# llsurreal919/Reduce-Complexity-for-intra-coding-of-VVC

Hardware: AMD Instinct MI355X
Metric: CTUs/sec (All-Intra, QP32) (higher is better)
Workload: dtype int16/int32 samples+coefficients, fp64 RD cost

## Files before the change

### include/vvcx.h

```cpp
#ifndef VVCX_H
#define VVCX_H
#include <stdint.h>
#ifdef __cplusplus
extern "C" {
#endif

typedef enum {
  VVCX_OK = 0, VVCX_ERR_ARG = -1, VVCX_ERR_UNSUPPORTED = -2, VVCX_ERR_DEVICE = -3, VVCX_ERR_STATE = -4, VVCX_ERR_NO_ENCODING = -5
} vvcx_status;

enum {
  VVCX_TOOL_MRL = 1 << 0, VVCX_TOOL_MIP = 1 << 1, VVCX_TOOL_ISP = 1 << 2, VVCX_TOOL_LFNST = 1 << 3, VVCX_TOOL_MTS = 1 << 4,
  VVCX_TOOL_TS = 1 << 5, VVCX_TOOL_DEPQUANT = 1 << 6, VVCX_TOOL_RDOQ = 1 << 7, VVCX_TOOL_CCLM = 1 << 8,
  VVCX_TOOL_JCCR = 1 << 9, VVCX_TOOL_LMCS = 1 << 10, VVCX_TOOL_CU_REUSE = 1 << 11,
  VVCX_TOOL_FAST = 1 << 12,
  VVCX_TOOL_WPP = 1 << 13
};

typedef struct {
  int32_t pic_w, pic_h;
  int32_t bit_depth;
  int32_t ctu_size;
  int32_t min_qt[2];
  int32_t max_bt_depth[2];
// ... 67 lines not shown
int  vvcx_create(const vvcx_cfg *cfg, vvcx_handle **h);
void vvcx_destroy(vvcx_handle *h);
int  vvcx_set_slice(vvcx_handle *h, const vvcx_slice *s);
typedef struct {
  int32_t qp;
  int32_t bit_depth;
  int32_t n_pts;
  int32_t qp_in[8], qp_out[8];
  int32_t cb_qp_offset, cr_qp_offset;
  int32_t gop_size;
  int32_t dep_quant;
} vvcx_slice_cfg;
int  vvcx_chroma_qp_table(int bit_depth, int n_pts, const int32_t *qp_in, const int32_t *qp_out, int32_t *table);
int  vvcx_derive_slice(const vvcx_slice_cfg *cfg, vvcx_slice *out);

int  vvcx_set_forest(vvcx_handle *h, int n_trees, int n_nodes, int n_classes, const int32_t *root, const int32_t *feature, const double *threshold,
                     const int32_t *left, const int32_t *right, const double *value, const int32_t *classes);
int  vvcx_bind_frames(vvcx_handle *h, const vvcx_frame *frames, int n);
int  vvcx_compress_ctus(vvcx_handle *h, const vvcx_ctu_task *tasks, int n, vvcx_ctu_result *out, void *hip_stream);
int  vvcx_submit_ctus(vvcx_handle *h, const vvcx_ctu_task *tasks, int n, void *hip_stream);
int  vvcx_poll_ctus(vvcx_handle *h);
int  vvcx_wait_ctus(vvcx_handle *h, vvcx_ctu_result *out, int n);
int  vvcx_compress_bound_frames(vvcx_handle *h, vvcx_ctu_result *out , void *hip_stream);
int  vvcx_get_cus(vvcx_handle *h, int frame, vvcx_cu *cus, int max_cus, int *n_cus);
int  vvcx_get_tus(vvcx_handle *h, int frame, vvcx_tu *tus, int max_tus, int *n_tus);
int  vvcx_get_levels(vvcx_handle *h, int frame, int comp, int16_t *plane, int stride);
int  vvcx_lmcs_inverse_reco(vvcx_handle *h, void *hip_stream);
int  vvcx_lmcs_analyze(const void *const org[3], const int stride[3], int pic_w, int pic_h, int bit_depth, int slice_qp, int update_ctrl, vvcx_slice *slice);
int  vvcx_lmcs_analyze_device(const void *const org[3], const int stride[3], int pic_w, int pic_h, int bit_depth, int slice_qp, int update_ctrl, vvcx_slice *slice);
int  vvcx_lmcs_tables(vvcx_handle *h, int16_t *fwd, int16_t *inv, int32_t pivot[17], int32_t chroma_scale[16]);
int  vvcx_deblock_bound_frames(vvcx_handle *h, int beta_offset_div2, int tc_offset_div2, void *hip_stream);
float vvcx_last_deblock_ms(const vvcx_handle *h);
typedef struct vvcx_sao_param { int8_t mode, type, band, offset[4]; } vvcx_sao_param;
int   vvcx_sao_bound_frames(vvcx_handle *h, const vvcx_sao_param *prm, int lf_across_tiles, int log2_offset_scale, void *hip_stream);
float vvcx_last_sao_ms(const vvcx_handle *h);
int   vvcx_sao_statistics_bound_frames(vvcx_handle *h, int lf_across_tiles, int64_t *stats, void *hip_stream);
float vvcx_last_sao_stats_ms(const vvcx_handle *h);
int   vvcx_sao_decide(int pic_w, int pic_h, int bit_depth, int tile_cols, int tile_rows, int slice_qp, const double *lambda, int log2_offset_scale,
                      const int64_t *stats, vvcx_sao_param *prm);
int   vvcx_sao_picture(int pic_w, int pic_h, int bit_depth, int tile_cols, int tile_rows, const vvcx_sao_param *prm, int lf_across_tiles, int log2_offset_scale,
                       uint16_t *y, uint16_t *cb, uint16_t *cr, int device);
typedef struct vvcx_alf_aps {
  int32_t num_luma_filters; uint8_t class_to_filter[25]; uint8_t nonlinear_luma; int16_t luma_coeff[25][12]; uint8_t luma_clip_idx[25][12];
  int32_t num_chroma_alt; uint8_t nonlinear_chroma[8]; int16_t chroma_coeff[8][6]; uint8_t chroma_clip_idx[8][6];
} vvcx_alf_aps;
typedef struct vvcx_alf_slice { int32_t n_luma_aps, luma_aps[8], chroma_aps; } vvcx_alf_slice;
typedef struct vvcx_alf_ctu { uint8_t flag[3]; int8_t set; uint8_t alt[2]; } vvcx_alf_ctu;
int   vvcx_alf_bound_frames(vvcx_handle *h, const vvcx_alf_aps *aps, int n_aps, const vvcx_alf_slice *slices, const vvcx_alf_ctu *ctus, void *hip_stream);
float vvcx_last_alf_ms(const vvcx_handle *h);
int   vvcx_alf_picture(int pic_w, int pic_h, int bit_depth, const vvcx_alf_aps *aps, int n_aps, const vvcx_alf_slice *slice, const vvcx_alf_ctu *ctus,
                       uint16_t *y, uint16_t *cb, uint16_t *cr, uint8_t *classes, int device);
int   vvcx_alf_statistics_picture(int pic_w, int pic_h, int bit_depth, int n_bins, const uint16_t *const org[3], const uint16_t *const rec[3],
                                  int64_t *luma, int64_t *chroma, int device);
int   vvcx_alf_statistics_bound_frames(vvcx_handle *h, int frame_first, int n, int n_bins, int64_t *luma, int64_t *chroma, void *hip_stream);
float vvcx_last_alf_stats_ms(const vvcx_handle *h);
int   vvcx_alf_decide(int pic_w, int pic_h, int bit_depth, int chroma, int n_bins, const int64_t *luma, const int64_t *chroma_stats,
                      const double lambda[3], int max_luma_filters, vvcx_alf_aps *aps, vvcx_alf_slice *slice, vvcx_alf_ctu *ctus);
int  vvcx_deblock_cu_table(int pic_w, int pic_h, int bit_depth, int qp, int qp_cb, int qp_cr, int beta_offset_div2, int tc_offset_div2,
                           const int32_t *rows, int n_rows, uint16_t *y, uint16_t *cb, uint16_t *cr, int device);
int  vvcx_get_payload(vvcx_handle *h, int frame, int tile, uint8_t *buf, int cap, int *nbytes);
int  vvcx_enable_training_dump(vvcx_handle *h, int cap_rows);
int  vvcx_get_training_rows(vvcx_handle *h, int32_t *rows, int max_rows, int *n_rows);
int  vvcx_get_substream_sizes(vvcx_handle *h, int frame, int tile, int *sizes, int max_sizes, int *n_sizes);
float vvcx_last_kernel_ms(const vvcx_handle *h);
int  vvcx_get_counters(vvcx_handle *h, uint64_t out[4]);
int  vvcx_get_profile(vvcx_handle *h, uint64_t out[48]);
const char *vvcx_last_error(void);
int  vvcx_ctus_per_frame(const vvcx_handle *h);
int  vvcx_resident_streams(const vvcx_handle *h);


int  vvcx_distortion_batch(const int16_t *a, const int16_t *b, int w, int h, int n, uint64_t *out, int device);
typedef struct { int32_t comp, x, y, w, h, mode, mrl; } vvcx_pred_case;
int  vvcx_intra_pred_batch(vvcx_handle *h, const void *const reco[3], const uint8_t *const coded[2], const vvcx_pred_case *cases, int n, int16_t *pred);
int  vvcx_ctx_init(int qp, uint16_t s0[386], uint16_t s1[386]);
int  vvcx_cabac_code_bins(uint16_t *s0, uint16_t *s1, int ctx, const uint8_t *bins, int nbins, uint64_t *frac_bits, int device);
int  vvcx_rd_cost_batch(double lambda, const uint64_t *frac_bits, const uint64_t *dist, int n, double *cost, int device);
int  vvcx_transform_quant_batch(const int16_t *org, const int16_t *pred, int w, int h, int bit_depth, int qp, int n,
                                int16_t *lev, int16_t *rec, uint64_t *sse, uint8_t *cbf, int device);
int  vvcx_depquant_batch(const int16_t *org, const int16_t *pred, int w, int h, int bit_depth, int qp, int comp, int mts_idx, int cbf_cb, double lambda,
                         const uint16_t *s0, const uint16_t *s1, int n, int16_t *lev, int16_t *rec, uint64_t *sse, uint8_t *cbf, int device);
int  vvcx_lfnst_depquant_batch(const int16_t *org, const int16_t *pred, int w, int h, int bit_depth, int qp, int comp, int lfnst_idx, int intra_dir, int cbf_cb, double lambda,
                               const uint16_t *s0, const uint16_t *s1, int n, int16_t *lev, int16_t *rec, uint64_t *sse, uint8_t *cbf, int device);
int  vvcx_transform_skip_batch(const int16_t *resi, int w, int h, int bit_depth, int qp, double lambda, const uint16_t *s0, const uint16_t *s1, int n,
                               int16_t *lev, int16_t *resi_out, int32_t *abs_sum, uint8_t *keep, uint64_t *frac_bits, int device);
int  vvcx_isp_tu_batch(const int16_t *org, const int16_t *pred, int tw, int th, int bit_depth, int qp, double lambda, int prev_cbf, int cbf_inferred,
                       const uint16_t *s0, const uint16_t *s1, int n, int16_t *lev, int16_t *rec, uint64_t *sse, uint8_t *cbf, int device);
int  vvcx_scan_order(int w, int h, uint16_t *idx, int device);
int  vvcx_mip_pred_batch(const int32_t *cases, int n, const int16_t *refs, int n_refs, int16_t *pred, int n_pred, int device);
int  vvcx_forest_predict_batch(vvcx_handle *h, const int32_t *rows, int n, int32_t *out);

#ifdef __cplusplus
}
#endif
#endif
```

### reduce-complexity-for-intra-coding-of-vvc_amd/csrc/vvcx_api.hip

```cpp
#include <hip/hip_runtime.h>
#include <stdint.h>
#include <stdio.h>
#include <stdarg.h>
#include <stdlib.h>
#include <string.h>
#include <math.h>
#include <limits>
#include <algorithm>
#include <vector>
#include "vvcx.h"
#include "vvcx_dev.h"
#include "vvcx_host.h"
#include "vvcx_tables.h"

extern "C" __global__ void vvcx_compress_kernel_u8(VxParams p);
extern "C" __global__ void vvcx_compress_kernel_u16(VxParams p);
extern "C" __global__ void vvcx_compress_wpp_kernel_u8(VxParams p);
extern "C" __global__ void vvcx_compress_wpp_kernel_u16(VxParams p);
extern "C" __global__ void vvcx_leaf_dist_kernel(const int16_t *a, const int16_t *b, int w, int h, int16_t *scr, unsigned long long *out);
extern "C" __global__ void vvcx_leaf_pred_kernel_u8(VxParams p, const VxLeafPred *cases, int16_t *out, const int *out_off);
extern "C" __global__ void vvcx_leaf_pred_kernel_u16(VxParams p, const VxLeafPred *cases, int16_t *out, const int *out_off);
extern "C" __global__ void vvcx_leaf_cabac_kernel(uint16_t *io, int ctx, const uint8_t *bins, int nbins, unsigned long long *bits);
extern "C" __global__ void vvcx_leaf_rdcost_kernel(VxParams p, const unsigned long long *bits, const unsigned long long *dist, int n, double *cost);
extern "C" __global__ void vvcx_leaf_scan_kernel(int w, int h, uint16_t *idx);
extern "C" __global__ void vvcx_leaf_forest_kernel(VxParams p, const int32_t *rows, int n, int32_t *out);
struct VxMipCase { int32_t w, h, mode, bit_depth, ref_off, pred_off; };
extern "C" __global__ void vvcx_leaf_mip_kernel(const VxMipCase *cases, const int16_t *refs, int16_t *preds);
extern "C" __global__ void vvcx_sao_copy_kernel_u8(VxSaoParams p);
extern "C" __global__ void vvcx_sao_copy_kernel_u16(VxSaoParams p);
extern "C" __global__ void vvcx_sao_kernel_u8(VxSaoParams p);
extern "C" __global__ void vvcx_sao_kernel_u16(VxSaoParams p);
extern "C" __global__ void vvcx_sao_stats_kernel_u8(VxSaoStatParams p);
extern "C" __global__ void vvcx_sao_stats_kernel_u16(VxSaoStatParams p);
extern "C" __global__ void vvcx_alf_copy_kernel_u8(VxAlfParams p);
extern "C" __global__ void vvcx_alf_copy_kernel_u16(VxAlfParams p);
extern "C" __global__ void vvcx_alf_kernel_u8(VxAlfParams p);
extern "C" __global__ void vvcx_alf_kernel_u16(VxAlfParams p);
extern "C" __global__ void vvcx_alf_stats_b1_kernel_u8(VxAlfStatParams p);
extern "C" __global__ void vvcx_alf_stats_b4_kernel_u8(VxAlfStatParams p);
extern "C" __global__ void vvcx_alf_stats_b1_kernel_u16(VxAlfStatParams p);
extern "C" __global__ void vvcx_alf_stats_b4_kernel_u16(VxAlfStatParams p);
extern "C" __global__ void vvcx_deblock_edges_kernel(VxDeblockParams p);
extern "C" __global__ void vvcx_deblock_kernel_u8(VxDeblockParams p);
extern "C" __global__ void vvcx_deblock_kernel_u16(VxDeblockParams p);
extern "C" __global__ void vvcx_jccr_sign_kernel_u8(VxFrameDev *frames, int wc, int hc);
extern "C" __global__ void vvcx_jccr_sign_kernel_u16(VxFrameDev *frames, int wc, int hc);
extern "C" __global__ void vvcx_leaf_dq_kernel(VxParams p, const uint16_t *ctx, const int16_t *org, int16_t *rec, int16_t *lev, int32_t *tmp, int w, int h, int qp, int comp, int mts, int cbf_cb, unsigned long long *out, int lf, int lfdir);
extern "C" __global__ void vvcx_leaf_ts_kernel(VxParams p, const uint16_t *ctx, const int16_t *resi, int16_t *lev, int16_t *resi_out, int32_t *tmp, int w, int h, int qp, int *out, unsigned long long *bits);
extern "C" __global__ void vvcx_lmcs_map_kernel_u8(const uint8_t *src, uint8_t *dst, int w, int h, int stride, const int16_t *lut);
extern "C" __global__ void vvcx_lmcs_map_kernel_u16(const uint16_t *src, uint16_t *dst, int w, int h, int stride, const int16_t *lut);
extern "C" __global__ void vvcx_leaf_isp_kernel(VxParams p, const uint16_t *ctx, const int16_t *org, int16_t *rec, int16_t *lev, int32_t *tmp, int w, int h, int qp, int cbf_ctx, unsigned long long *out);
extern "C" __global__ void vvcx_ctu_activity_kernel_u8(const VxFrameDev *frames, int pic_w, int pic_h, int ctus_w, unsigned *out);
extern "C" __global__ void vvcx_ctu_activity_kernel_u16(const VxFrameDev *frames, int pic_w, int pic_h, int ctus_w, unsigned *out);
extern "C" __global__ void vvcx_leaf_trq_kernel(const int16_t *org, int16_t *rec, int16_t *lev, int32_t *tmp, int w, int h, int bd, int qp, unsigned long long *out);

static thread_local char g_err[512];
extern "C" const char *vvcx_last_error(void) { return g_err; }
extern "C" int vvcx_fail_msg_(int code, const char *msg) { snprintf(g_err, sizeof g_err, "%s", msg); return code; }
static int fail(int code, const char *fmt, ...)
{
  va_list ap; va_start(ap, fmt); vsnprintf(g_err, sizeof g_err, fmt, ap); va_end(ap);
  return code;
}

struct vvcx_handle {
  vvcx_cfg cfg; vvcx_slice sl; bool have_slice;
  int ctus_w, ctus_h, uw, uh, ntiles;
  std::vector<int> ctu_tile;
  std::vector<std::vector<int>> tile_ctus;
  int n_frames;
  std::vector<VxFrameDev> frames_h;
  int nsub;
  std::vector<int> ctu_sub, sub_tile, sub_above, tile_sub0, tile_nsub;
  std::vector<std::vector<int>> sub_ctus;
  DevBuf<int32_t> train_rows_d; DevBuf<uint32_t> train_n_d; int train_cap;
  DevBuf<int32_t> wpp_sched_d; int wpp_rr;
  DevBuf<int32_t> wpp_progress_d; DevBuf<uint16_t> wpp_sync_d;
  std::vector<int> next_idx;
  DevBuf<VxFrameDev> frames_d; DevBuf<int16_t> lev_d; DevBuf<VxUnit> units_d; DevBuf<uint16_t> stream_ctx_d;
  DevBuf<uint8_t> scratch_d;
  DevBuf<VxStreamDesc> streams_d; DevBuf<int32_t> task_ctu_d; DevBuf<VxCtuRes> results_d;
  DevBuf<unsigned long long> counters_d;
  DevBuf<uint8_t> payload_d; DevBuf<uint64_t> payload_off_d; DevBuf<uint32_t> payload_cap_d; DevBuf<uint8_t> arith_d; std::vector<uint64_t> payload_off; std::vector<uint32_t> payload_cap;
  DevBuf<VxForestNode> f_node_d; DevBuf<double> f_value_d; DevBuf<int32_t> f_root_d; int f_ntrees, f_nclasses; int32_t f_classes[8];
  DevBuf<VxDqConst> dq_d;
  bool lmcs_on, lmcs_inverted; int16_t lmcs_fwd[1024], lmcs_inv[1024]; int32_t lmcs_pivot[17], lmcs_cadj[16];
  DevBuf<int16_t> lmcs_lut_d; DevBuf<uint8_t> lmcs_org_d;
  std::vector<uint32_t> activity;
  hipEvent_t ev0, ev1; float last_ms, last_deblock_ms, last_sao_ms;
  DevBuf<uint8_t> sao_tmp_d; DevBuf<VxSaoEntry> sao_tab_d; DevBuf<uint8_t> sao_tile_d;
  DevBuf<uint8_t> db_edges_d;
  DevBuf<long long> sao_stat_d; float last_sao_stats_ms;
  DevBuf<VxAlfFrame> alf_tab_d; DevBuf<VxAlfCtu> alf_ctu_d; float last_alf_ms;
  DevBuf<long long> alf_stat_luma_d, alf_stat_chroma_d; float last_alf_stats_ms;
  bool pending; hipStream_t pend_stream; int pend_n; VxCtuRes *pend_res; int pend_cap;
  std::vector<VxStreamDesc> pend_sd; std::vector<int32_t> pend_task_ctu; std::vector<int> pend_src, pend_next; VxDqConst pend_dq[17 * 96];
  size_t lev_plane[3], lev_frame, units_plane, units_frame;
};

#define VVCX_PAYLOAD_BYTES_PER_CTU 32768u
static const uint32_t kBuiltTools = VVCX_TOOL_ISP | VVCX_TOOL_MRL | VVCX_TOOL_MIP | VVCX_TOOL_LFNST | VVCX_TOOL_MTS | VVCX_TOOL_JCCR | VVCX_TOOL_DEPQUANT | VVCX_TOOL_CU_REUSE | VVCX_TOOL_CCLM | VVCX_TOOL_FAST |
                                    VVCX_TOOL_TS | VVCX_TOOL_RDOQ | VVCX_TOOL_LMCS | VVCX_TOOL_WPP;

static VxDqConst dq_consts_of(int lsum, int bit_depth, int qp, double lambda)
{
  VxDqConst c; memset(&c, 0, sizeof c);
  const int sq = lsum & 1, qpDQ = qp + 1, per = qpDQ / 6, rem = qpDQ - 6 * per;
  const int nomShift = 15 - bit_depth - (lsum >> 1), trShift = nomShift + (sq ? -1 : 0);
  const int qshift = 14 - 1 + per + trShift;
  const int64_t qscale = VX_QUANT_SCALES[sq * 6 + rem];
  const int invShift = 6 + 1 - per - trShift;
  int qIdxBD = 32 + invShift - 6 - 1; if (qIdxBD > 16) qIdxBD = 16;
  const int nomDShift = 15 - 2 * nomShift + qshift + (sq ? 1 : 0);
  const double qScale2 = (double) (qscale * qscale);
  const double nomDistFactor = nomDShift < 0 ? 1.0 / ((double) ((int64_t) 1 << (-nomDShift)) * qScale2 * lambda) : (double) ((int64_t) 1 << nomDShift) / (qScale2 * lambda);
  const int64_t pow2dfShift = (int64_t) (nomDistFactor * qScale2) + 1;
  int dfShift = (pow2dfShift & (pow2dfShift - 1)) ? 1 : 0;
  for (uint64_t x = (uint64_t) pow2dfShift; x > 1; x >>= 1) dfShift++;
  const int dshift = 62 + qshift - 2 * 15 - dfShift;
  c.qshift = qshift; c.qadd = -(((int64_t) 3 << qshift) >> 1); c.qscale = qscale; c.max_qidx = (1 << (qIdxBD - 1)) - 4;
  c.thres = (int32_t) ((int64_t) 4 << qshift);
  c.dshift = dshift; c.dadd = ((int64_t) 1 << dshift) >> 1;
  c.dstep = (int64_t) (nomDistFactor * (double) ((int64_t) 1 << (dshift + qshift)) + .5);
  c.dorg = (int64_t) (nomDistFactor * (double) ((int64_t) 1 << (dshift + 1)) + .5);
  return c;
}

#define NOT_PENDING(h) do { if ((h) && (h)->pending) return fail(VVCX_ERR_STATE, "a submitted launch is outstanding: call vvcx_wait_ctus first"); } while (0)

// ... 1605 lines not shown
  HIPCHK(hipGetLastError());
  HIPCHK(hipMemcpy(pred, dp.p, (size_t) po * 2, hipMemcpyDeviceToHost));
  return VVCX_OK;
}

extern "C" int vvcx_forest_predict_batch(vvcx_handle *h, const int32_t *rows, int n, int32_t *out)
{
  NOT_PENDING(h);
  if (!h || !rows || !out || n < 0) return fail(VVCX_ERR_ARG, "bad argument");
  if (!h->f_ntrees) return fail(VVCX_ERR_STATE, "vvcx_set_forest first");
  if (n == 0) return VVCX_OK;
  ON_DEVICE(h->cfg.device);
  DevBuf<int32_t> dr, dout; HIPCHK(dr.alloc((size_t) n * 26)); HIPCHK(dout.alloc((size_t) n));
  HIPCHK(hipMemcpy(dr.p, rows, (size_t) n * 26 * 4, hipMemcpyHostToDevice));
  VxParams p; memset(&p, 0, sizeof p);
  p.f_node = h->f_node_d.p; p.f_value = h->f_value_d.p; p.f_root = h->f_root_d.p; p.f_ntrees = h->f_ntrees; p.f_nclasses = h->f_nclasses;
  for (int c = 0; c < 8; c++) p.f_classes[c] = h->f_classes[c];
  hipLaunchKernelGGL(vvcx_leaf_forest_kernel, dim3((unsigned) ((n + VXD_NT - 1) / VXD_NT)), dim3(VXD_NT), 0, 0, p, dr.p, n, dout.p);
  HIPCHK(hipGetLastError());
  HIPCHK(hipMemcpy(out, dout.p, (size_t) n * 4, hipMemcpyDeviceToHost));
  return VVCX_OK;
}

extern "C" int vvcx_transform_quant_batch(const int16_t *org, const int16_t *pred, int w, int h, int bit_depth, int qp, int n,
                                          int16_t *lev, int16_t *rec, uint64_t *sse, uint8_t *cbf, int device)
{
  if (!org || !pred || !lev || !rec || !sse || !cbf || n < 0 || !pow2_block(w, h) || (bit_depth != 8 && bit_depth != 10) || qp < 0 || qp > 75) return fail(VVCX_ERR_ARG, "bad argument");
  if (n == 0) return VVCX_OK;
  ON_DEVICE(device);
  const size_t bytes = (size_t) n * w * h * 2;
  DevBuf<int16_t> dorg, drec, dlev; DevBuf<int32_t> dtmp; DevBuf<unsigned long long> dout;
  HIPCHK(dorg.alloc(bytes / 2)); HIPCHK(drec.alloc(bytes / 2)); HIPCHK(dlev.alloc(bytes / 2)); HIPCHK(dtmp.alloc((size_t) n * 2048)); HIPCHK(dout.alloc((size_t) n * 2));
  HIPCHK(hipMemcpy(dorg.p, org, bytes, hipMemcpyHostToDevice)); HIPCHK(hipMemcpy(drec.p, pred, bytes, hipMemcpyHostToDevice));
  hipLaunchKernelGGL(vvcx_leaf_trq_kernel, dim3((unsigned) n), dim3(VXD_NT), 0, 0, dorg.p, drec.p, dlev.p, dtmp.p, w, h, bit_depth, qp,
                     dout.p);
  HIPCHK(hipGetLastError());
  std::vector<unsigned long long> o((size_t) n * 2);
  HIPCHK(hipMemcpy(lev, dlev.p, bytes, hipMemcpyDeviceToHost)); HIPCHK(hipMemcpy(rec, drec.p, bytes, hipMemcpyDeviceToHost));
  HIPCHK(hipMemcpy(o.data(), dout.p, (size_t) n * 16, hipMemcpyDeviceToHost));
  for (int i = 0; i < n; i++) { sse[i] = o[(size_t) i * 2]; cbf[i] = (uint8_t) o[(size_t) i * 2 + 1]; }
  return VVCX_OK;
}

static int depquant_batch_impl(const int16_t *org, const int16_t *pred, int w, int h, int bit_depth, int qp, int comp, int mts_idx, int cbf_cb, double lambda,
                               const uint16_t *s0, const uint16_t *s1, int n, int16_t *lev, int16_t *rec, uint64_t *sse, uint8_t *cbf, int device, int lfnst_idx, int intra_dir)
{
  if (!org || !pred || !lev || !rec || !sse || !cbf || !s0 || !s1 || n < 0 || !pow2_block(w, h) || (bit_depth != 8 && bit_depth != 10) || qp < 0 || qp > 75 || comp < 0 || comp > 2 ||
      !(lambda > 0.0) || (mts_idx != 0 && (mts_idx < 2 || mts_idx > 5 || comp != 0 || w > 32 || h > 32 || w < 4 || h < 4))) return fail(VVCX_ERR_ARG, "bad argument");
  if (n == 0) return VVCX_OK;
  ON_DEVICE(device);
  const size_t bytes = (size_t) n * w * h * 2;
  DevBuf<int16_t> dorg, drec, dlev; DevBuf<int32_t> dtmp; DevBuf<unsigned long long> dout; DevBuf<uint16_t> dctx; DevBuf<VxDqConst> dtab; DevBuf<uint8_t> dscr;
  HIPCHK(dorg.alloc(bytes / 2)); HIPCHK(drec.alloc(bytes / 2)); HIPCHK(dlev.alloc(bytes / 2)); HIPCHK(dtmp.alloc((size_t) n * 2048)); HIPCHK(dout.alloc((size_t) n * 2));
  HIPCHK(dctx.alloc(2 * VXD_NUM_CTX)); HIPCHK(dtab.alloc(48)); HIPCHK(dscr.alloc((size_t) n * VXD_OFF_CACHE));
  HIPCHK(hipMemcpy(dorg.p, org, bytes, hipMemcpyHostToDevice)); HIPCHK(hipMemcpy(drec.p, pred, bytes, hipMemcpyHostToDevice));
  { uint16_t kept[2 * VXD_NUM_CTX]; ctx_from_reference_order(s0, s1, kept); HIPCHK(hipMemcpy(dctx.p, kept, sizeof kept, hipMemcpyHostToDevice)); }
  VxDqConst tab[48]; memset(tab, 0, sizeof tab);
  for (int lsum = 2; lsum <= 12; lsum++) tab[comp * 16 + lsum] = dq_consts_of(lsum, bit_depth, qp, lambda);
  HIPCHK(hipMemcpy(dtab.p, tab, sizeof tab, hipMemcpyHostToDevice));
  VxParams p; memset(&p, 0, sizeof p);
  p.bit_depth = bit_depth; p.tools = VVCX_TOOL_DEPQUANT | VVCX_TOOL_MTS | (lfnst_idx ? VVCX_TOOL_LFNST : 0); p.dq_consts = dtab.p; p.scratch = dscr.p; p.scratch_per_stream = VXD_OFF_CACHE;
  hipLaunchKernelGGL(vvcx_leaf_dq_kernel, dim3((unsigned) n), dim3(VXD_NT), 0, 0, p, dctx.p, dorg.p, drec.p, dlev.p, dtmp.p,
                     w, h, qp, comp, mts_idx, cbf_cb, dout.p, (w >= 4 && h >= 4) ? lfnst_idx : 0, intra_dir);
  HIPCHK(hipGetLastError());
  std::vector<unsigned long long> o((size_t) n * 2);
  HIPCHK(hipMemcpy(lev, dlev.p, bytes, hipMemcpyDeviceToHost)); HIPCHK(hipMemcpy(rec, drec.p, bytes, hipMemcpyDeviceToHost));
  HIPCHK(hipMemcpy(o.data(), dout.p, (size_t) n * 16, hipMemcpyDeviceToHost));
  for (int i = 0; i < n; i++) { sse[i] = o[(size_t) i * 2]; cbf[i] = (uint8_t) o[(size_t) i * 2 + 1]; }
  return VVCX_OK;
}

extern "C" int vvcx_depquant_batch(const int16_t *org, const int16_t *pred, int w, int h, int bit_depth, int qp, int comp, int mts_idx, int cbf_cb, double lambda,
                                   const uint16_t *s0, const uint16_t *s1, int n, int16_t *lev, int16_t *rec, uint64_t *sse, uint8_t *cbf, int device)
{
  return depquant_batch_impl(org, pred, w, h, bit_depth, qp, comp, mts_idx, cbf_cb, lambda, s0, s1, n, lev, rec, sse, cbf, device, 0, 0);
}
extern "C" int vvcx_lfnst_depquant_batch(const int16_t *org, const int16_t *pred, int w, int h, int bit_depth, int qp, int comp, int lfnst_idx, int intra_dir, int cbf_cb, double lambda,
                                         const uint16_t *s0, const uint16_t *s1, int n, int16_t *lev, int16_t *rec, uint64_t *sse, uint8_t *cbf, int device)
{
  if (lfnst_idx < 0 || lfnst_idx > 2 || intra_dir < 0 || intra_dir > 66) return fail(VVCX_ERR_ARG, "bad argument");
  return depquant_batch_impl(org, pred, w, h, bit_depth, qp, comp, 0, cbf_cb, lambda, s0, s1, n, lev, rec, sse, cbf, device, lfnst_idx, intra_dir);
}

extern "C" int vvcx_isp_tu_batch(const int16_t *org, const int16_t *pred, int tw, int th, int bit_depth, int qp, double lambda, int prev_cbf, int cbf_inferred,
                                 const uint16_t *s0, const uint16_t *s1, int n, int16_t *lev, int16_t *rec, uint64_t *sse, uint8_t *cbf, int device)
{
  const bool shape = tw >= 1 && th >= 1 && tw <= 64 && th <= 64 && !(tw & (tw - 1)) && !(th & (th - 1)) && tw * th >= 16;
  if (!org || !pred || !lev || !rec || !sse || !cbf || !s0 || !s1 || n < 0 || !shape || (bit_depth != 8 && bit_depth != 10) || qp < 0 || qp > 75 || !(lambda > 0.0)) return fail(VVCX_ERR_ARG, "bad argument");
  if (n == 0) return VVCX_OK;
  ON_DEVICE(device);
  const size_t bytes = (size_t) n * tw * th * 2;
  DevBuf<int16_t> dorg, drec, dlev; DevBuf<int32_t> dtmp; DevBuf<unsigned long long> dout; DevBuf<uint16_t> dctx; DevBuf<VxDqConst> dtab; DevBuf<uint8_t> dscr;
  HIPCHK(dorg.alloc(bytes / 2)); HIPCHK(drec.alloc(bytes / 2)); HIPCHK(dlev.alloc(bytes / 2)); HIPCHK(dtmp.alloc((size_t) n * 2048)); HIPCHK(dout.alloc((size_t) n * 2));
  HIPCHK(dctx.alloc(2 * VXD_NUM_CTX)); HIPCHK(dtab.alloc(96)); HIPCHK(dscr.alloc((size_t) n * VXD_OFF_CACHE));
  HIPCHK(hipMemcpy(dorg.p, org, bytes, hipMemcpyHostToDevice)); HIPCHK(hipMemcpy(drec.p, pred, bytes, hipMemcpyHostToDevice));
  { uint16_t kept[2 * VXD_NUM_CTX]; ctx_from_reference_order(s0, s1, kept); HIPCHK(hipMemcpy(dctx.p, kept, sizeof kept, hipMemcpyHostToDevice)); }
  VxDqConst tab[96]; memset(tab, 0, sizeof tab);
  for (int lsum = 2; lsum <= 12; lsum++) tab[lsum] = dq_consts_of(lsum, bit_depth, qp, lambda);
  HIPCHK(hipMemcpy(dtab.p, tab, sizeof tab, hipMemcpyHostToDevice));
  VxParams p; memset(&p, 0, sizeof p);
  p.bit_depth = bit_depth; p.tools = VVCX_TOOL_DEPQUANT | VVCX_TOOL_MTS | VVCX_TOOL_LFNST | VVCX_TOOL_ISP; p.dq_consts = dtab.p; p.scratch = dscr.p; p.scratch_per_stream = VXD_OFF_CACHE;
  p.lambda = lambda;
  hipLaunchKernelGGL(vvcx_leaf_isp_kernel, dim3((unsigned) n), dim3(VXD_NT), 0, 0, p, dctx.p, dorg.p, drec.p, dlev.p, dtmp.p,
                     tw, th, qp, cbf_inferred ? -1 : (int) VX_CTX_QtCbf[0] + 2 + (prev_cbf ? 1 : 0), dout.p);
  HIPCHK(hipGetLastError());
  std::vector<unsigned long long> o((size_t) n * 2);
  HIPCHK(hipMemcpy(lev, dlev.p, bytes, hipMemcpyDeviceToHost)); HIPCHK(hipMemcpy(rec, drec.p, bytes, hipMemcpyDeviceToHost));
  HIPCHK(hipMemcpy(o.data(), dout.p, (size_t) n * 16, hipMemcpyDeviceToHost));
  for (int i = 0; i < n; i++) { sse[i] = o[(size_t) i * 2]; cbf[i] = (uint8_t) o[(size_t) i * 2 + 1]; }
  return VVCX_OK;
}

extern "C" int vvcx_transform_skip_batch(const int16_t *resi, int w, int h, int bit_depth, int qp, double lambda, const uint16_t *s0, const uint16_t *s1, int n,
                                         int16_t *lev, int16_t *resi_out, int32_t *abs_sum, uint8_t *keep, uint64_t *frac_bits, int device)
{
  if (!resi || !lev || !resi_out || !abs_sum || !keep || !frac_bits || !s0 || !s1 || n < 0 || !pow2_block(w, h) || w < 4 || h < 4 || w > 32 || h > 32 || (bit_depth != 8 && bit_depth != 10) ||
      qp < 0 || qp > 75 || !(lambda > 0.0)) return fail(VVCX_ERR_ARG, "bad argument");
  if (n == 0) return VVCX_OK;
  ON_DEVICE(device);
  const size_t bytes = (size_t) n * w * h * 2;
  DevBuf<int16_t> dres, dout, dlev; DevBuf<int32_t> dtmp; DevBuf<int> do2; DevBuf<unsigned long long> dbits; DevBuf<uint16_t> dctx;
  HIPCHK(dres.alloc(bytes / 2)); HIPCHK(dout.alloc(bytes / 2)); HIPCHK(dlev.alloc(bytes / 2)); HIPCHK(dtmp.alloc((size_t) n * 2048)); HIPCHK(do2.alloc((size_t) n * 2)); HIPCHK(dbits.alloc((size_t) n));
  HIPCHK(dctx.alloc(2 * VXD_NUM_CTX));
  HIPCHK(hipMemcpy(dres.p, resi, bytes, hipMemcpyHostToDevice)); HIPCHK(hipMemset(dout.p, 0, bytes));
  { uint16_t kept[2 * VXD_NUM_CTX]; ctx_from_reference_order(s0, s1, kept); HIPCHK(hipMemcpy(dctx.p, kept, sizeof kept, hipMemcpyHostToDevice)); }
  VxParams p; memset(&p, 0, sizeof p);
  p.bit_depth = bit_depth; p.tools = VVCX_TOOL_DEPQUANT | VVCX_TOOL_LFNST | VVCX_TOOL_TS; p.lambda = lambda;
  hipLaunchKernelGGL(vvcx_leaf_ts_kernel, dim3((unsigned) n), dim3(VXD_NT), 0, 0, p, dctx.p, dres.p, dlev.p, dout.p, dtmp.p, w, h, qp,
                     do2.p, dbits.p);
  HIPCHK(hipGetLastError());
  std::vector<int> o((size_t) n * 2);
  HIPCHK(hipMemcpy(lev, dlev.p, bytes, hipMemcpyDeviceToHost)); HIPCHK(hipMemcpy(resi_out, dout.p, bytes, hipMemcpyDeviceToHost));
  HIPCHK(hipMemcpy(o.data(), do2.p, (size_t) n * 8, hipMemcpyDeviceToHost)); HIPCHK(hipMemcpy(frac_bits, dbits.p, (size_t) n * 8, hipMemcpyDeviceToHost));
  for (int i = 0; i < n; i++) { abs_sum[i] = o[(size_t) i * 2]; keep[i] = (uint8_t) o[(size_t) i * 2 + 1]; }
  return VVCX_OK;
}

static int payload_of_tile(vvcx_handle *h, int frame, int tile, uint8_t *buf, int cap, int *nbytes, int *sizes, int max_sizes, int *n_sizes)
{
  if (!h || frame < 0 || frame >= h->n_frames || tile < 0 || tile >= h->ntiles) return fail(VVCX_ERR_ARG, "bad argument");
  if (!h->payload_d.p) return fail(VVCX_ERR_STATE, "handle was created without emit_payload");
  ON_DEVICE(h->cfg.device);
  const int sub0 = h->tile_sub0[(size_t) tile], ns = h->tile_nsub[(size_t) tile];
  if (n_sizes) *n_sizes = ns;
  if (sizes && max_sizes < ns) return fail(VVCX_ERR_ARG, "room for %d sub-stream sizes, the tile has %d", max_sizes, ns);
  size_t total = 0;
  for (int k = 0; k < ns; k++) {
    const size_t s = (size_t) frame * h->nsub + (size_t) (sub0 + k);
    if (h->next_idx[s] != (int) h->sub_ctus[(size_t) (sub0 + k)].size()) return fail(VVCX_ERR_STATE, "tile %d of frame %d is not completely coded yet", tile, frame);
    uint32_t st[8];
    HIPCHK(hipMemcpy(st, (const uint8_t *) h->arith_d.p + s * 32, 32, hipMemcpyDeviceToHost));
    const uint32_t n = st[7];
    if (n > h->payload_cap[s]) return fail(VVCX_ERR_STATE, "payload of tile %d exceeds the %u bytes reserved", tile, h->payload_cap[s]);
    if (sizes) sizes[k] = (int) n;
    if (buf && total + n <= (size_t) cap) HIPCHK(hipMemcpy(buf + total, h->payload_d.p + h->payload_off[s], n, hipMemcpyDeviceToHost));
    total += n;
  }
  if (nbytes) *nbytes = (int) total;
  if (buf && total > (size_t) cap) return fail(VVCX_ERR_ARG, "buffer too small: %zu bytes needed", total);
  return VVCX_OK;
}
extern "C" int vvcx_enable_training_dump(vvcx_handle *h, int cap_rows)
{
  NOT_PENDING(h);
  if (!h || cap_rows < 0) return fail(VVCX_ERR_ARG, "bad argument");
  if (cap_rows > 0 && (h->cfg.tools & VVCX_TOOL_WPP)) return fail(VVCX_ERR_UNSUPPORTED, "the training dump is not available on a WPP handle");
// ... 37 lines not shown
```

### reduce-complexity-for-intra-coding-of-vvc_amd/csrc/vvcx_depquant_dev.h

```cpp
#pragma once
#ifndef VXD_SERIAL_PRIO
#define VXD_SERIAL_PRIO 0
#endif

struct U4 { unsigned a, b, c, d; };
struct U8 { unsigned a, b, c, d, e, f, g, h; };
struct DqS { long long cost; int pk, rem; unsigned long long anc; U4 lev; };
#define DQ_NUMSIG(p) ((p) & 31)
#define DQ_HIST(p) ((((p) >> 5) & 7) - 1)
#define DQ_RPAR(p) (((p) >> 8) & 3)
#define DQ_RZERO(p) (((p) >> 10) & 63)
#define DQ_SBBC(p) ((((p) >> 16) & 3) - 1)
#define DQ_SIGI(p) (((p) >> 18) & 15)
#define DQ_GTXI(p) (((p) >> 22) & 31)
__device__ inline int dq_put(int p, int sh, int nbits, int v) { const int m = ((1 << nbits) - 1) << sh; return (p & ~m) | ((v << sh) & m); }

#ifndef VX_GLOBAL
#ifdef VX_EMU
#define VX_GLOBAL
#else
#define VX_GLOBAL __attribute__((address_space(1)))
#endif
#endif
#ifndef VX_REG_BARRIER
#define VX_REG_BARRIER(x) asm volatile("" : "+v"(x))
#endif
__device__ inline unsigned dq_get_b(const U4 &v, int i)
{
  unsigned a = v.a, b = v.b, c = v.c, d = v.d;
  VX_REG_BARRIER(a); VX_REG_BARRIER(b); VX_REG_BARRIER(c); VX_REG_BARRIER(d);
  const unsigned w = i < 8 ? (i < 4 ? a : b) : (i < 12 ? c : d);
  return (w >> ((i & 3) << 3)) & 255u;
}
__device__ inline void dq_set_b(U4 &v, int i, unsigned x)
{
  const unsigned sh = (unsigned) (i & 3) << 3, m = ~(255u << sh), y = x << sh; const int wi = i >> 2;
  v.a = wi == 0 ? (v.a & m) | y : v.a; v.b = wi == 1 ? (v.b & m) | y : v.b; v.c = wi == 2 ? (v.c & m) | y : v.c; v.d = wi == 3 ? (v.d & m) | y : v.d;
}
__device__ inline unsigned dq_get_h(const U8 &v, int i)
{
  const int wi = i >> 1;
  unsigned a = v.a, b = v.b, c = v.c, d = v.d, e = v.e, f = v.f, g = v.g, h = v.h;
  VX_REG_BARRIER(a); VX_REG_BARRIER(b); VX_REG_BARRIER(c); VX_REG_BARRIER(d); VX_REG_BARRIER(e); VX_REG_BARRIER(f); VX_REG_BARRIER(g); VX_REG_BARRIER(h);
  const unsigned w = wi < 4 ? (wi < 2 ? (wi == 0 ? a : b) : (wi == 2 ? c : d)) : (wi < 6 ? (wi == 4 ? e : f) : (wi == 6 ? g : h));
  return (w >> ((i & 1) << 4)) & 0xffffu;
}
__device__ inline void dq_set_h(U8 &v, int i, unsigned x)
{
  const unsigned sh = (unsigned) (i & 1) << 4, m = ~(0xffffu << sh), y = x << sh; const int wi = i >> 1;
  v.a = wi == 0 ? (v.a & m) | y : v.a; v.b = wi == 1 ? (v.b & m) | y : v.b; v.c = wi == 2 ? (v.c & m) | y : v.c; v.d = wi == 3 ? (v.d & m) | y : v.d;
  v.e = wi == 4 ? (v.e & m) | y : v.e; v.f = wi == 5 ? (v.f & m) | y : v.f; v.g = wi == 6 ? (v.g & m) | y : v.g; v.h = wi == 7 ? (v.h & m) | y : v.h;
}
__device__ inline U4 dq_shfl_u4(const U4 &v, int src) { U4 r; r.a = (unsigned) __shfl((int) v.a, src); r.b = (unsigned) __shfl((int) v.b, src); r.c = (unsigned) __shfl((int) v.c, src); r.d = (unsigned) __shfl((int) v.d, src); return r; }
__device__ inline U8 dq_shfl_u8(const U8 &v, int src)
{
  U8 r; r.a = (unsigned) __shfl((int) v.a, src); r.b = (unsigned) __shfl((int) v.b, src); r.c = (unsigned) __shfl((int) v.c, src); r.d = (unsigned) __shfl((int) v.d, src);
  r.e = (unsigned) __shfl((int) v.e, src); r.f = (unsigned) __shfl((int) v.f, src); r.g = (unsigned) __shfl((int) v.g, src); r.h = (unsigned) __shfl((int) v.h, src);
  return r;
}
template <int CTRL> __device__ inline long long dq_quad_i64(long long v)
{
  const int lo = __builtin_amdgcn_update_dpp(0, (int) v, CTRL, 0xF, 0xF, true), hi = __builtin_amdgcn_update_dpp(0, (int) (v >> 32), CTRL, 0xF, 0xF, true);
  return (long long) (((unsigned long long) (unsigned) hi << 32) | (unsigned) lo);
}
__device__ inline int dq_parent(int v, bool fromA)
{
  const int a = __builtin_amdgcn_update_dpp(0, v, 0xD8, 0xF, 0xF, true), b = __builtin_amdgcn_update_dpp(0, v, 0x8D, 0xF, 0xF, true);
  return fromA ? a : b;
}
__device__ inline long long dq_shfl_i64(long long v, int src)
{
  const int lo = __shfl((int) v, src), hi = __shfl((int) (v >> 32), src);
  return (long long) (((unsigned long long) (unsigned) hi << 32) | (unsigned) lo);
}
__device__ inline long long dq_uni_ll(long long v)
{
  const int lo = __builtin_amdgcn_readfirstlane((int) v), hi = __builtin_amdgcn_readfirstlane((int) (v >> 32));
  return (long long) (((unsigned long long) (unsigned) hi << 32) | (unsigned) lo);
}
__device__ inline int dq_fb(int ci, int ctx, int bin) { const Ctx &c = L.ctxs[ci]; return (int) BIN_FRAC(((unsigned) c.s0[ctx] + (unsigned) c.s1[ctx]) >> 8, bin); }
__device__ inline int dq_rice_bits(int par, unsigned v) { return rem_abs_len(v, (unsigned) par) << 15; }

struct DqRate { int ci, g1Base, g2Base, parBase, sbbBase; };
__device__ inline long long dq_lev_bits(const DqRate &R, int gtx_i, int rice_par, int lev)
{
  if (lev == 0) return 0;
  if (lev == 1) return dq_fb(R.ci, R.g1Base + gtx_i, 0) + (1 << 15);
  long long b = (long long) dq_fb(R.ci, R.g1Base + gtx_i, 1) + (1 << 15) + dq_fb(R.ci, R.parBase + gtx_i, lev & 1) + dq_fb(R.ci, R.g2Base + gtx_i, lev >= 4);
  if (lev >= 4) { const unsigned v = (unsigned) (lev - 4) >> 1; b += dq_rice_bits(rice_par, v < 32 ? v : 31); }
  return b;
}
__device__ inline int dq_qidx0(const VxDqConst &q, long long scaledOrg)
{
  const int v = (int) ((scaledOrg + q.qadd) >> q.qshift);
  return imax(1, imin(q.max_qidx, v));
}
__device__ inline long long dq_dd(const VxDqConst &q, long long scaledOrg, int qIdx0, int step)
{
  const long long scaledAdd = (long long) qIdx0 * q.dstep - scaledOrg * q.dorg + (long long) step * q.dstep;
  return (scaledAdd * (qIdx0 + step) + q.dadd) >> q.dshift;
}
__device__ inline int dq_sig_off(int ch, int diag) { return ch ? (diag < 2 ? 4 : 0) : (diag < 2 ? 8 : diag < 5 ? 4 : 0); }
__device__ inline int dq_gtx_off(int ch, int diag) { return ch ? (diag < 1 ? 6 : 1) : (diag < 1 ? 16 : diag < 3 ? 11 : diag < 10 ? 6 : 1); }

#define DQ_TAB_BYTES (4 * DQ_TAB_INTS)
#ifdef VVCX_STAMP_DQ
#define DQ_T(n_) const long long n_ = clock64()
#define DQ_U(n_) n_ = clock64()
#else
#define DQ_T(n_)
#define DQ_U(n_)
#endif
__device__ inline void dq_fill_tables(int *tab, int ci, int ch, int t, int nt)
{
  const int ngtx = ch ? 11 : 21, nsig = ch ? 8 : 12;
  const int g1Base = VX_CTX_GtxFlag[2 + ch], g2Base = VX_CTX_GtxFlag[ch], parBase = VX_CTX_ParFlag[ch], sbbBase = VX_CTX_SigCoeffGroup[ch];
  int *levTab = tab, *sigTab = tab + 21 * 6, *sbbTab = sigTab + 3 * 12 * 2;
  for (int e = t; e < ngtx * 6; e += nt) {
    const int g = e / 6, j = e - g * 6;
    levTab[e] = j == 0 ? 0 : j == 1 ? dq_fb(ci, g1Base + g, 0) + (1 << 15) : dq_fb(ci, g1Base + g, 1) + (1 << 15) + dq_fb(ci, parBase + g, j & 1) + dq_fb(ci, g2Base + g, j >= 4);
  }
  for (int e = t; e < 3 * nsig * 2; e += nt) { const int st = e / (nsig * 2), r = e - st * nsig * 2; sigTab[st * 24 + r] = dq_fb(ci, VX_CTX_SigFlag[ch + 2 * st] + (r >> 1), r & 1); }
  if (t < 4) sbbTab[t] = dq_fb(ci, sbbBase + (t >> 1), t & 1);
}
__device__ inline void dq_build_tables(int ch) { dq_fill_tables(L.dq_tab, CI_CUR, ch, (int) VTX, NT); __syncthreads(); }
template <int TAB>
__device__ __noinline__ void wave_depquant_batch(int n_items, int16_t *cf_base, int cf_stride, uint8_t *nodes, int node_stride, int wk_wave, int abs0,
                                                 int ci0, int ci_step, int cbf_ctx0, unsigned cbf_mask, int w, int h, int comp, int zo, int lfnst, int lane, int qidx = -1)
{
  n_items = uni(n_items); w = uni(w); h = uni(h); comp = uni(comp); zo = uni(zo); lfnst = uni(lfnst); ci0 = uni(ci0); ci_step = uni(ci_step); cbf_ctx0 = uni(cbf_ctx0);
  cf_base = uni_p(cf_base); nodes = uni_p(nodes); cf_stride = uni(cf_stride); node_stride = uni(node_stride); abs0 = uni(abs0); cbf_mask = (unsigned) uni((int) cbf_mask); qidx = uni(qidx);
  uint8_t *wk = (uint8_t *) &L.wm[uni(wk_wave)];
  const int ch = comp ? 1 : 0, lw = ilog2i(w), lh = ilog2i(h);
  const int qrow = uni(qidx) < 0 ? comp : uni(qidx);
  VxDqConst q;
  { const VxDqConst &qv = L.par.dq_consts[(qrow ? uni(L.lmcs_tab) * 96 : 0) + qrow * 16 + lw + lh];
    q.qshift = uni(qv.qshift); q.max_qidx = uni(qv.max_qidx); q.thres = uni(qv.thres); q.dshift = uni(qv.dshift);
    q.qadd = dq_uni_ll(qv.qadd); q.qscale = dq_uni_ll(qv.qscale); q.dadd = dq_uni_ll(qv.dadd); q.dstep = dq_uni_ll(qv.dstep); q.dorg = dq_uni_ll(qv.dorg); }
  const ScanGeo geo = scan_geo(w, h);
  const int lcw = geo.lcw, lch = geo.lch, lcg = geo.lcg, gs = 1 << lcg, total = geo.nscan;
  const int nzw = imin(32, w), nzh = imin(32, h), wsbb = geo.wg, hsbb = geo.hg;
  const uint8_t *cg_inv = L.t.cg_inv + cg_tab_off(lcw, lch);
  const uint8_t *grp_inv = L.t.grp_inv + 15 * (wsbb - 1) + wsbb * (hsbb - 1);
  int effW = w, effH = h, zeroOut = 0;
  if (zo && comp == 0) { effH = h == 32 ? 16 : h; effW = w == 32 ? 16 : w; zeroOut = effH < h || effW < w; }
  const int item = lane >> 2, k = lane & 3, qbase = lane & ~3;
  const bool valid = item < n_items;
  DQ_T(t0);
  const int it0 = valid ? item : 0;
  int16_t *cf = cf_base + it0 * cf_stride;
  uint8_t *nd = nodes + (size_t) it0 * node_stride;
  int *lastb = (int *) wk + it0 * 20;
  uint16_t *trel = (uint16_t *) (wk + n_items * 80) + it0 * total;
  uint16_t *tmrows = (uint16_t *) (wk + n_items * (80 + 2 * total)) + it0 * 80;
  const int node_room = node_stride ? node_stride : VXD_DQ_WAVE;
  VX_CHECK((total >> lcg) * 64 <= node_room);
  if (valid) for (int e = k; e < 80; e += 4) tmrows[e] = 0;
  const int ci = ci0 + it0 * ci_step;
  const int cbf_ctx = cbf_ctx0 < 0 ? -1 : cbf_ctx0 + (int) ((cbf_mask >> it0) & 1u);
  int start = total - 1;
  if (lfnst > 0 && w >= 4 && h >= 4) start = ((w == 4 && h == 4) || (w == 8 && h == 8)) ? 7 : 15;
  int first = -1, top = -1;
  {
    const int thr = q.thres / (int) (4 * q.qscale);
    for (int i = 0; i < n_items; i++) {
      const int16_t *c = cf_base + i * cf_stride;
      int found = -1;
      for (int t = start | 63; t >= 63 && found < 0; t -= 64) {
        const int sp = t - lane;
        bool hit = false;
        if (sp <= start) {
          const int blk = scan_blk(geo, sp), x = blk & (w - 1), y = blk >> lw;
          hit = !(zeroOut && (x >= effW || y >= effH)) && iabs((int) c[blk]) > thr;
        }
        const unsigned long long m = __ballot(hit);
        if (m) found = t - (__ffsll(m) - 1);
      }
      found = uni(found);
      if (item == i) first = found;
      top = imax(top, found);
    }
  }
  DQ_T(t1);
  if (top < 0) {
    for (int i = 0; i < n_items; i++) { int16_t *c = cf_base + i * cf_stride; for (int sp = lane; sp < total; sp += 64) c[scan_blk(geo, sp)] = 0; }
    if (lane < n_items) L.dq_abs[abs0 + lane] = 0;
    wave_sync();
    return;
  }
  DqRate R; R.ci = ci; R.g1Base = VX_CTX_GtxFlag[2 + ch]; R.g2Base = VX_CTX_GtxFlag[ch]; R.parBase = VX_CTX_ParFlag[ch]; R.sbbBase = VX_CTX_SigCoeffGroup[ch];
  const int sigSet = VX_CTX_SigFlag[ch + 2 * imax(k - 1, 0)];
  int *tabBase = TAB == 2 ? L.dq_tab : (int *) (wk + n_items * (240 + 2 * total));
  if (TAB == 1) dq_fill_tables(tabBase, ci, ch, lane, 64);
  const int *levTab = tabBase, *sigTab = tabBase + 21 * 6, *sbbTab = sigTab + 3 * 12 * 2; const uint8_t *riceTab = L.t.rice_len;
  const int *mySig = sigTab + imax(k - 1, 0) * 24;
  auto levBits = [&](int gtx_i, int rpar, int lev) -> int {
    if (!TAB) return (int) dq_lev_bits(R, gtx_i, rpar, lev);
    const int b = levTab[gtx_i * 6 + (lev < 4 ? lev : 4 + (lev & 1))];
    const int rb = (int) riceTab[rpar * 32 + imin(31, imax(0, lev - 4) >> 1)] << 15;
    return lev >= 4 ? b + rb : b;
  };
  auto riceBits = [&](int rpar, unsigned v) -> int { return TAB ? (int) riceTab[rpar * 32 + (int) v] << 15 : dq_rice_bits(rpar, v); };
  auto sbbBits = [&](int sbbc, int bin) -> int { return TAB ? sbbTab[sbbc * 2 + bin] : dq_fb(ci, R.sbbBase + sbbc, bin); };
  if (valid) {
    const int cbfDelta = cbf_ctx >= 0 ? dq_fb(ci, cbf_ctx, 1) - dq_fb(ci, cbf_ctx, 0) : 0;
    for (int e = k; e < 20; e += 4) {
      const int xy = e >= 10, id = xy ? e - 10 : e;
      const int size = xy ? h : w, l2 = ilog2i(size);
      const int base = (xy ? VX_CTX_LastY : VX_CTX_LastX)[ch];
      const int sh = comp == 0 ? (l2 + 1) >> 2 : imin(2, size >> 3), lo = comp == 0 ? L.t.last_prefix[l2] : 0;
      const int maxId = L.t.group_idx[imin(32, size) - 1];
      if (id <= maxId) {
        unsigned sum = 0;
        for (int j = 0; j < id; j++) sum += (unsigned) dq_fb(ci, base + lo + (j >> sh), 1);
        unsigned b = sum + (id > 3 ? (unsigned) ((id - 2) >> 1) << 15 : 0u) + (unsigned) (xy ? cbfDelta : 0);
        if (id < maxId) b += (unsigned) dq_fb(ci, base + lo + (id >> sh), 0);
        lastb[e] = (int) b;
      }
    }
  }
  wave_sync();
  DQ_T(t2);
  const int regFull = (imin(32, effW) * imin(32, effH) * 28) >> 4;
  struct DqK { long long cost; int pk, rem; unsigned long long anc; };
  DqS cur, prv; DqK skp;
  {
    DqS s0; s0.cost = 0x7fffffffffffffffll >> 1; s0.rem = 4; s0.anc = 0;
    s0.pk = dq_put(0, 5, 3, 0);
    s0.lev = U4{ 0, 0, 0, 0 };
    cur = s0; prv = s0; skp.cost = s0.cost; skp.pk = s0.pk; skp.rem = s0.rem; skp.anc = 0;
  }
  long long decCost = 0x7fffffffffffffffll >> 2;
  if (valid) for (int sp = k; sp <= first; sp += 4) trel[sp] = (uint16_t) cf[scan_blk(geo, sp)];
  wave_sync();
  unsigned eosW = 0;
  if (lane < gs) {
    const int off = cg_tab_off(lcw, lch);
    const int xy = L.t.cg_scan[off + lane], gx = xy & 15, gy = xy >> 4;
#pragma unroll
    for (int n = 0; n < 5; n++) {
      const int xx = gx + (n == 0 ? 1 : n == 1 ? 2 : n == 2 ? 1 : 0), yy = gy + (n == 2 ? 1 : n == 3 ? 1 : n == 4 ? 2 : 0);
      const int ox = (xx >> lcw) != 0, oy = (yy >> lch) != 0;
      if (ox || oy) eosW |= (unsigned) ((ox ? (oy ? 3 : 1) : 2) | ((int) cg_inv[((yy & ((1 << lch) - 1)) << lcw) | (xx & ((1 << lcw) - 1))] << 2)) << (6 * n);
    }
  }
  int cnext = 0;
#ifdef VVCX_STAMP_DQ
  long long sA = 0, sB = 0, sC = 0, sE = 0, u1 = 0, u2 = 0, u3 = 0;
#endif
  __builtin_amdgcn_s_setprio(VXD_SERIAL_PRIO);
  for (int top64 = top; top64 >= 0; top64 -= 64) {
  int pgA = 0, pgB = 0, pgC = 0;
  {
    const int sp = top64 - lane;
    if (sp >= 0) {
      const int blk = scan_blk(geo, sp), x = blk & (w - 1), y = blk >> lw, inside = sp & (gs - 1);
      int spt = 0;
      if (inside == gs - 1 && sp > gs && sp < total - 1) spt = 1; else if (inside == 0 && sp > 0 && sp < total - gs) spt = 2;
      pgA = blk | (inside << 12) | (spt << 16) | ((zeroOut && (x >= effW || y >= effH)) ? 1 << 18 : 0) | ((int) L.t.group_idx[x] << 19) | ((int) L.t.group_idx[y] << 23);
      if (sp > 0) {
        const int nb = scan_blk(geo, sp - 1), xn = nb & (w - 1), yn = nb >> lw, diag = xn + yn;
        int cnt = 0;
#pragma unroll
        for (int n = 0; n < 5; n++) {
          const int xx = xn + (n == 0 ? 1 : n == 1 ? 2 : n == 2 ? 1 : 0), yy = yn + (n == 2 ? 1 : n == 3 ? 1 : n == 4 ? 2 : 0);
          if (xx < nzw && yy < nzh && (xx >> lcw) == (xn >> lcw) && (yy >> lch) == (yn >> lch)) { pgC |= (int) cg_inv[((yy & ((1 << lch) - 1)) << lcw) | (xx & ((1 << lcw) - 1))] << (4 * cnt); cnt++; }
        }
        pgB = ((sp - 1) & (gs - 1)) | (dq_sig_off(ch, diag) << 4) | (dq_gtx_off(ch, diag) << 8) | (cnt << 13) | (nb << 16);
      }
    }
  }
  if (top64 == top) cnext = (valid && top <= first) ? (int) (int16_t) trel[top] : 0;
  const int nchunk = imin(64, top64 + 1);
  for (int it = 0; it < nchunk; it++) {
    const int sp = top64 - it;
    DQ_T(u0); DQ_U(u1);
    const int gA = __builtin_amdgcn_readlane(pgA, it), gB = __builtin_amdgcn_readlane(pgB, it), nbl = __builtin_amdgcn_readlane(pgC, it);
    const int inside = (gA >> 12) & 15, eos = inside == 0, spt = (gA >> 16) & 3, zeroed = (gA >> 18) & 1;
    const int nin = gB & 15, sigOffN = (gB >> 4) & 15, gtxOffN = (gB >> 8) & 31, nbCnt = (gB >> 13) & 7;
    const bool act = valid && sp <= first;
    const int absC = iabs(cnext);
    if (valid && sp > 0 && sp - 1 <= first) cnext = (int) (int16_t) trel[sp - 1];
    { const DqS t = prv; prv = cur; cur = t; }
    long long dc = 0x7fffffffffffffffll >> 2; int dsrc = 0, dnz = 0, dlev = -1;
    if (zeroed) {
      if (spt == 2) { dc = skp.cost + (DQ_SBBC(skp.pk) >= 0 ? sbbBits(DQ_SBBC(skp.pk), 0) : 0); dsrc = 4; dlev = 0; }
    } else {
      const long long scaledOrg = (long long) absC * q.qscale;
      const int qIdx0 = dq_qidx0(q, scaledOrg);
#define DQ_STEP(i_) (((i_) - qIdx0) & 3)
#define DQ_LEV(st_) ((qIdx0 + (st_) + 1) >> 1)
      const int stA = DQ_STEP(k < 2 ? 0 : 3), stB = DQ_STEP(k < 2 ? 2 : 1);
      const int levA = DQ_LEV(stA), levB = DQ_LEV(stB);
      const long long ddMine = dq_dd(q, scaledOrg, qIdx0, DQ_STEP(k));
      const long long ddA = dq_quad_i64<0xF0>(ddMine), ddB = dq_quad_i64<0x5A>(ddMine);
      long long cA = prv.cost + ddA, cB = prv.cost + ddB, cZ = prv.cost;
      {
        const int ppk = prv.pk, rpar = DQ_RPAR(ppk);
        if (prv.rem >= 4) {
          cA += levBits(DQ_GTXI(ppk), rpar, levA); cB += levBits(DQ_GTXI(ppk), rpar, levB);
          int s0b, s1b;
          if (TAB) { const long long sb2 = *(const long long *) (mySig + 2 * DQ_SIGI(ppk)); s0b = (int) sb2; s1b = (int) (sb2 >> 32); }
          else { s0b = dq_fb(ci, sigSet + DQ_SIGI(ppk), 0); s1b = dq_fb(ci, sigSet + DQ_SIGI(ppk), 1); }
          if (spt == 0) { cA += s1b; cB += s1b; cZ += s0b; }
          else if (spt == 1) { const int sb = DQ_SBBC(ppk) >= 0 ? sbbBits(DQ_SBBC(ppk), 1) : 0; cA += sb + s1b; cB += sb + s1b; cZ += sb + s0b; }
          else if (DQ_NUMSIG(ppk)) { cA += s1b; cB += s1b; cZ += s0b; }
          else cZ = 0x7fffffffffffffffll;
        } else {
          const int rz = DQ_RZERO(ppk);
          cA += (1 << 15) + riceBits(rpar, (unsigned) (levA <= rz ? levA - 1 : (levA < 32 ? levA : 31)));
          cB += (1 << 15) + riceBits(rpar, (unsigned) (levB <= rz ? levB - 1 : (levB < 32 ? levB : 31)));
          cZ += riceBits(rpar, (unsigned) imin(31, rz));
        }
      }
      DQ_U(u1);
      const long long azA = dq_quad_i64<0xD8>(cA), azZ = dq_quad_i64<0xD8>(cZ), bB = dq_quad_i64<0x8D>(cB);
      const int tLevA = DQ_LEV(DQ_STEP((k & 1) ? 3 : 0)), tLevB = DQ_LEV(DQ_STEP((k & 1) ? 1 : 2));
      {
        long long m = azA; int msrc = 2, mnz = 1, mlev = tLevA;
        if (azZ < m) { m = azZ; mnz = 0; mlev = 0; }
        const bool bWins = k < 2 ? bB < m : bB <= m;
// ... 6 lines not shown
      }
      if (!(k & 1)) {
        const int stS = DQ_STEP(k), levS = DQ_LEV(stS);
        const long long c = ddMine + (long long) (lastb[(gA >> 19) & 15] + lastb[10 + ((gA >> 23) & 15)]) + levBits(0, 0, levS);
        if (c < dc) { dc = c; dsrc = 1; dnz = 1; dlev = levS; }
      }
#undef DQ_STEP
#undef DQ_LEV
    }
    {
      int e = ((dsrc << 1) | dnz) << (4 * k);
      e = seg_sum<4>(e);
      VX_CHECK(sp >= 0 && sp < total);
      if (k == 0 && act) trel[sp] = (uint16_t) e;
    }
    if (act) decCost = dc;
    DQ_U(u2);
    if (sp == 0) break;
    if (eos || !zeroed) {
      struct { int pk, rem; unsigned long long anc; U4 lev; } P;
      {
        const bool fromA = dsrc == 2;
#define DQ_PARENT(x_) dq_parent((int) (x_), fromA)
        P.pk = DQ_PARENT(prv.pk); P.rem = DQ_PARENT(prv.rem);
        P.anc = (unsigned long long) (unsigned) DQ_PARENT((unsigned) prv.anc) | ((unsigned long long) (unsigned) DQ_PARENT((unsigned) (prv.anc >> 32)) << 32);
        P.lev.a = (unsigned) DQ_PARENT(prv.lev.a); P.lev.b = (unsigned) DQ_PARENT(prv.lev.b); P.lev.c = (unsigned) DQ_PARENT(prv.lev.c); P.lev.d = (unsigned) DQ_PARENT(prv.lev.d);
#undef DQ_PARENT
      }
      const bool alive = act && dsrc != 0, fromPrev = dsrc == 2 || dsrc == 3;
      if (act) cur.cost = dc;
      if (!eos) {
        if (alive) {
          int pk = cur.pk;
          {
            const int lowNew = fromPrev ? ((P.pk & ((7 << 5) | (3 << 16))) | ((P.pk + (dlev != 0)) & 31)) : 1;
            pk = (pk & (fromPrev ? ~(0xFF | (3 << 16)) : ~0xFF)) | lowNew;
            int rem = fromPrev ? P.rem - 1 : regFull;
            rem -= rem >= 4 ? (dlev < 2 ? dlev : 3) : 0;
            cur.rem = rem; cur.anc = fromPrev ? P.anc : 0ull;
            cur.lev.a = fromPrev ? P.lev.a : 0u; cur.lev.b = fromPrev ? P.lev.b : 0u; cur.lev.c = fromPrev ? P.lev.c : 0u; cur.lev.d = fromPrev ? P.lev.d : 0u;
          }
          dq_set_b(cur.lev, inside, (unsigned) imin(255, dlev));
          const int trow = fromPrev ? ((P.pk >> 27) & 7) : 4;
          VX_CHECK(trow <= 4 && nin < 16);
          pk = (pk & ~(7 << 27)) | (trow << 27);
          const int t = (int) tmrows[trow * 16 + nin];
          int sumAbs = t >> 8, sumAbs1 = (t >> 3) & 31, sumNum = t & 7;
          {
            typedef unsigned dq_v4u __attribute__((vector_size(16)));
            const dq_v4u cl = { cur.lev.a, cur.lev.b, cur.lev.c, cur.lev.d };
#pragma unroll
            for (int n = 0; n < 5; n++) if (n < nbCnt) {
              const int bi = (nbl >> (4 * n)) & 15;
              const int a = (int) ((cl[bi >> 2] >> ((bi & 3) << 3)) & 255u);
              sumAbs += a; sumAbs1 += imin(4 + (a & 1), a); sumNum += a != 0;
            }
          }
          if (cur.rem >= 4) {
            pk = (pk & ~((3 << 8) | (0x1FF << 18))) | (((sumAbs >= 27) + (sumAbs >= 34) + (sumAbs >= 48)) << 8) | ((sigOffN + imin((sumAbs1 + 1) >> 1, 3)) << 18)
                 | ((gtxOffN + imin(sumAbs1 - sumNum, 4)) << 22);
          } else {
            sumAbs = imin(31, sumAbs);
            pk = dq_put(pk, 8, 2, L.t.gorice_pars[sumAbs]); pk = dq_put(pk, 10, 6, L.t.gorice_pos0[imax(0, k - 1) * 32 + sumAbs]);
          }
          cur.pk = pk;
        }
      } else {
        const int g = sp >> lcg;
        int pk = cur.pk; int numSig, pRem; unsigned long long pAnc; U4 lv = { 0, 0, 0, 0 };
        if (dsrc == 4) { numSig = 0; pRem = skp.rem; pAnc = skp.anc; }
        else if (fromPrev) { numSig = DQ_NUMSIG(P.pk) + (dlev != 0); pRem = P.rem; pAnc = P.anc; lv = P.lev; }
        else { numSig = 1; pRem = regFull; pAnc = 0; }
        dq_set_b(lv, 0, (unsigned) imin(255, imax(dlev, 0)));
        const unsigned long long anc = (pAnc << 4) | (unsigned long long) (unsigned) (k + 1) | ((numSig != 0) ? 8ull : 0ull);
        VX_CHECK(g >= 1 && (g * 4 + k) * 16 + 16 <= node_room);
        if (alive) { VX_GLOBAL uint32_t *hl = (VX_GLOBAL uint32_t *) (nd + (size_t) (g * 4 + k) * 16); hl[0] = lv.a; hl[1] = lv.b; hl[2] = lv.c; hl[3] = lv.d; }
        wave_sync();
        const unsigned ng = geo.grp[g - 1]; const int nsx = (int) (ng & 15), nsy = (int) (ng >> 4);
        const int gR = nsx < wsbb - 1 ? grp_inv[nsy * wsbb + nsx + 1] : -1, gB = nsy < hsbb - 1 ? grp_inv[(nsy + 1) * wsbb + nsx] : -1;
        const int gD = (gR >= 0 && gB >= 0) ? grp_inv[(nsy + 1) * wsbb + nsx + 1] : -1;
        const unsigned fR = gR >= 0 ? (unsigned) (anc >> (4 * (gR - g))) & 15u : 0u, fB = gB >= 0 ? (unsigned) (anc >> (4 * (gB - g))) & 15u : 0u;
        const unsigned fD = gD >= 0 ? (unsigned) (anc >> (4 * (gD - g))) & 15u : 0u;
        const int sigN = ((fR & 8u) || (fB & 8u)) ? 1 : 0;
        typedef unsigned dq_v16u __attribute__((vector_size(64)));
        dq_v16u nv = { 0, 0, 0, 0, 0, 0, 0, 0, 0, 0, 0, 0, 0, 0, 0, 0 };
        if (alive) {
          VX_CHECK(!(fR & 7u) || (gR >= g && gR - g < 16 && (gR * 4 + (int) (fR & 7u) - 1) * 16 + 16 <= node_room));
          VX_CHECK(!(fB & 7u) || (gB >= g && gB - g < 16 && (gB * 4 + (int) (fB & 7u) - 1) * 16 + 16 <= node_room));
          VX_CHECK(!(fD & 7u) || (gD >= g && gD - g < 16 && (gD * 4 + (int) (fD & 7u) - 1) * 16 + 16 <= node_room));
          if (fR & 7u) { const VX_GLOBAL uint32_t *p_ = (const VX_GLOBAL uint32_t *) (nd + (size_t) (gR * 4 + (int) (fR & 7u) - 1) * 16); nv[4] = p_[0]; nv[5] = p_[1]; nv[6] = p_[2]; nv[7] = p_[3]; }
          if (fB & 7u) { const VX_GLOBAL uint32_t *p_ = (const VX_GLOBAL uint32_t *) (nd + (size_t) (gB * 4 + (int) (fB & 7u) - 1) * 16); nv[8] = p_[0]; nv[9] = p_[1]; nv[10] = p_[2]; nv[11] = p_[3]; }
          if (fD & 7u) { const VX_GLOBAL uint32_t *p_ = (const VX_GLOBAL uint32_t *) (nd + (size_t) (gD * 4 + (int) (fD & 7u) - 1) * 16); nv[12] = p_[0]; nv[13] = p_[1]; nv[14] = p_[2]; nv[15] = p_[3]; }
        }
        for (int id = 0; id < gs; id++) {
          const unsigned wrd = (unsigned) __builtin_amdgcn_readlane((int) eosW, id);
          int sumAbs = 0, sumAbs1 = 0, sumNum = 0;
#pragma unroll
          for (int n = 0; n < 5; n++) {
            const unsigned f = (wrd >> (6 * n)) & 63u;
            if (f & 3u) {
              const int a = (int) ((nv[(f & 3u) * 4 + (f >> 4)] >> (((f >> 2) & 3u) << 3)) & 255u);
              sumAbs += a; sumAbs1 += imin(4 + (a & 1), a); sumNum += a != 0;
            }
          }
          if (alive) tmrows[k * 16 + id] = (uint16_t) (sumNum + (sumAbs1 << 3) + (imin(127, sumAbs) << 8));
        }
        if (alive) {
          pk = dq_put(pk, 0, 5, 0); pk = dq_put(pk, 8, 2, 0); pk = dq_put(pk, 5, 3, k + 1); pk = dq_put(pk, 16, 2, sigN + 1);
          cur.rem = pRem; cur.anc = anc;
          cur.lev = U4{ 0, 0, 0, 0 };
          pk = dq_put(pk, 27, 3, k);
          const int t = (int) tmrows[k * 16 + nin];
          const int sumAbs1 = (t >> 3) & 31, sumNum = t & 7;
          pk = dq_put(pk, 18, 4, sigOffN + imin((sumAbs1 + 1) >> 1, 3)); pk = dq_put(pk, 22, 5, gtxOffN + imin(sumAbs1 - sumNum, 4));
          cur.pk = pk;
        }
      }
    }
    DQ_U(u3);
#ifdef VVCX_STAMP_DQ
    sA += u1 - u0; sB += u2 - u1; sC += u3 - u2; if (eos) sE += u3 - u2;
#endif
    if (spt == 1) { const DqK t = skp; skp.cost = prv.cost; skp.pk = prv.pk; skp.rem = prv.rem; skp.anc = prv.anc; prv.cost = t.cost; prv.pk = t.pk; prv.rem = t.rem; prv.anc = t.anc; }
  }
  }
  __builtin_amdgcn_s_setprio(0);
  DQ_T(t3);
  int prev = -2; long long minCost = 0;
#pragma unroll
  for (int s = 0; s < 4; s++) { const long long c = dq_shfl_i64(decCost, qbase + s); if (c < minCost) { prev = s; minCost = c; } }
  int nPath = 0;
  if (k == 0 && valid) {
    int sp = 0, absSum = 0;
    if (first < 0) prev = -2;
    while (prev >= 0) {
      VX_CHECK(sp >= 0 && sp <= first && prev < 4);
      const int e = (trel[sp] >> (4 * prev)) & 15, src = e >> 1;
      int lev = 0;
      if (e & 1) {
        const long long scaledOrg = (long long) iabs((int) cf[scan_blk(geo, sp)]) * q.qscale;
        const int i = src == 1 ? prev : src == 2 ? ((prev & 1) ? 3 : 0) : ((prev & 1) ? 1 : 2);
        const int qIdx0 = dq_qidx0(q, scaledOrg);
        lev = (qIdx0 + ((i - qIdx0) & 3) + 1) >> 1;
      }
      trel[sp] = (uint16_t) lev; absSum += lev;
      if (src == 4) { for (int j = 1; j < gs; j++) trel[sp + j] = 0; sp += gs; }
      else { prev = src == 1 ? -1 : src == 2 ? ((prev & 1) ? (prev == 1 ? 2 : 3) : (prev == 0 ? 0 : 1)) : src == 3 ? ((prev & 1) ? (prev == 1 ? 3 : 2) : (prev == 0 ? 1 : 0)) : -2; sp++; }
    }
    nPath = sp;
    L.dq_abs[abs0 + item] = absSum;
  }
  nPath = __shfl(nPath, qbase);
  wave_sync();
  DQ_T(t4);
  for (int i = 0; i < n_items; i++) {
    const int np = __builtin_amdgcn_readlane(nPath, i * 4);
    int16_t *c_ = cf_base + i * cf_stride; const uint16_t *tr = (const uint16_t *) (wk + n_items * 80) + i * total;
    for (int sp = lane; sp < total; sp += 64) {
      const int blk = scan_blk(geo, sp), c = c_[blk];
      const int lv = sp < np ? (int) tr[sp] : 0;
      c_[blk] = (int16_t) (c < 0 ? -lv : lv);
    }
  }
  wave_sync();
#ifdef VVCX_STAMP_DQ
  { const long long t5 = clock64(); int fs = valid && k == 0 ? first + 1 : 0; for (int o = 32; o; o >>= 1) fs += __shfl_xor(fs, o);
    if (lane == 0) { const long long v[14] = { t1 - t0, t2 - t1, t3 - t2, t4 - t3, t5 - t4, 1, top + 1, n_items, fs, total, sA, sB, sC, sE };
      for (int i = 0; i < 14; i++) atomicAdd(&L.prof[16 + i], (unsigned long long) v[i]); } }
#endif
}

#ifndef VXD_DQ_TAB_MIN
#define VXD_DQ_TAB_MIN 16
#endif
template <bool SMALL>
__device__ inline int wave_depquant(int16_t *cf_g, int buf_off, uint8_t *scratch, int ci, int w, int h, int comp, int cbf_ctx, int zo, int lfnst, int lane, int qidx = -1)
{
  const int wave_ = uni(VTX >> 6);
  int16_t *cf = SMALL ? L.wm[wave_].slot + BUF + uni(buf_off) : cf_g;
  if (imin(32, w) * imin(32, h) >= VXD_DQ_TAB_MIN && 240 + 2 * imin(32, w) * imin(32, h) + DQ_TAB_BYTES <= (int) (sizeof(WaveScratch) + sizeof(int32_t) * BUF))
    wave_depquant_batch<1>(1, cf, 0, scratch + VXD_OFF_DQ + (size_t) wave_ * VXD_DQ_WAVE, 0, wave_, DQ_ABS_SINGLE + wave_, ci, 0, cbf_ctx, 0u, w, h, comp, zo, lfnst, lane, qidx);
  else
    wave_depquant_batch<0>(1, cf, 0, scratch + VXD_OFF_DQ + (size_t) wave_ * VXD_DQ_WAVE, 0, wave_, DQ_ABS_SINGLE + wave_, ci, 0, cbf_ctx, 0u, w, h, comp, zo, lfnst, lane, qidx);
  return uni(L.dq_abs[DQ_ABS_SINGLE + wave_]);
}

__device__ inline void wave_dequant_dq(const int16_t *lev, int16_t *deq, int w, int h, int zw, int zh, int bd, int qp, int lane)
{
  const ScanGeo geo = scan_geo(w, h);
  const int lw = ilog2i(w), lh = ilog2i(h), lzw = ilog2i(zw), total = geo.nscan;
  int last = -1;
  for (int top = (total - 1) | 63; top >= 63 && last < 0; top -= 64) {
    const int sp = top - lane;
    const unsigned long long m = __ballot(sp < total && lev[scan_blk(geo, sp)] != 0);
    if (m) last = top - (__ffsll(m) - 1);
  }
  last = uni(last);
  for (int i = lane; i < zw * zh; i += 64) deq[i] = 0;
  wave_sync();
  if (last < 0) return;
  const int sq = (lw + lh) & 1, qpDQ = qp + 1, per = qpDQ / 6, rem = qpDQ - 6 * per;
  const int trShift = 15 - bd - ((lw + lh) >> 1) - sq;
  const int shift = 6 + 1 - per - trShift;
  int invQ = L.t.iqscale[sq * 6 + rem];
  if (shift < 0) invQ <<= -shift;
  const int sh = shift < 0 ? 0 : shift, add = shift < 0 ? 0 : ((1 << shift) >> 1);
  int x0 = 0, y0 = 0;
  const unsigned long long below = lane == 0 ? 0ull : (~0ull >> (64 - lane));
  const unsigned long long EVEN = 0x5555555555555555ull, ODD = 0xAAAAAAAAAAAAAAAAull;
  for (int t0 = 0; t0 <= last; t0 += 64) {
    const int sp = last - t0 - lane;
    int lv = 0, blk = 0;
    if (sp >= 0) { blk = scan_blk(geo, sp); lv = lev[blk]; }
    const unsigned long long P = __ballot(lv & 1);
    const int odd = lane & 1;
    const int xs = (odd ? y0 : x0) ^ (__popcll(P & below & (odd ? EVEN : ODD)) & 1);
    if (lv) {
      const int qIdx = (lv << 1) + (lv > 0 ? -xs : xs);
      const long long v = ((long long) qIdx * (long long) invQ + add) >> sh;
      deq[((blk >> lw) << lzw) + (blk & (w - 1))] = (int16_t) (v < -32768 ? -32768 : v > 32767 ? 32767 : v);
    }
    x0 ^= __popcll(P & ODD) & 1; y0 ^= __popcll(P & EVEN) & 1;
  }
  wave_sync();
}
```

### reduce-complexity-for-intra-coding-of-vvc_amd/csrc/vvcx_dev.h

```cpp
#pragma once
#include <stdint.h>

#ifndef VXD_NW
#define VXD_NW 4
#endif
#define VXD_NT (VXD_NW * 64)
#ifndef VXD_BUF
#define VXD_BUF 256
#endif
#ifndef VXD_WPE
#define VXD_WPE 5
#endif
#define VXD_MAXD 12
#define VXD_NUM_CTX 291

struct VxUnit {
  uint64_t ss;
  int16_t  x, y;
  uint8_t  lw, lh;
  uint8_t  qt, mt, bt, depth;
  uint8_t  dir, mrl, cbf, mts;
  uint16_t tag;
};

// ... 39 lines not shown
  int32_t             ntiles, nsub;
  uint8_t            *payload;
  const uint64_t     *payload_off;
  const uint32_t     *payload_cap;
  void               *arith_state;
  const VxForestNode *f_node;
  const double       *f_value;
  const int32_t      *f_root;
  int32_t             f_ntrees, f_nclasses;
  int32_t             f_classes[8];
  const VxDqConst    *dq_consts;
  int32_t             lmcs_on, lmcs_cadj_on, lmcs_min_bin, lmcs_max_bin;
  int32_t             lmcs_pivot[17], lmcs_cadj[16];
  int32_t             n_streams;
  int32_t             train_cap;
  int32_t            *train_rows;
  uint32_t           *train_n;
  int32_t            *wpp_progress;
  uint16_t           *wpp_sync;
  int32_t            *wpp_sched;
  int32_t             wpp_rr, pad_wpp;
};

struct VxDeblockParams {
  const VxFrameDev *frames;
  int32_t uw, uh, bit_depth, chroma;
  int32_t qp, qp_c[2];
  int32_t beta_off2, tc_off2, dir;
  uint8_t *edges;
};

struct VxSaoEntry { int8_t type, band; int16_t off[4]; int16_t pad_; };
struct VxSaoParams {
  const VxFrameDev *frames;
  const VxSaoEntry *table;
  const uint8_t *tile_of_ctu;
  void *tmp;
  uint64_t tmp_frame, tmp_comp[3];
  int32_t pic_w, pic_h, ctus_w, ctus_h, bit_depth, chroma, lf_across_tiles, pad_;
};

struct VxSaoStatParams {
  const VxFrameDev *frames;
  const uint8_t *tile_of_ctu;
  long long *out;
  int32_t pic_w, pic_h, ctus_w, ctus_h, bit_depth, chroma, lf_across_tiles, pad_;
};

struct VxAlfCtu { uint8_t flag[3]; int8_t set; uint8_t alt[2]; };
struct VxAlfFrame { int16_t luma_coeff[8][25][12], luma_clip[8][25][12], chroma_coeff[8][6], chroma_clip[8][6]; int32_t n_sets, n_alt; };
struct VxAlfParams {
  const VxFrameDev *frames;
  const VxAlfFrame *tabs;
  const VxAlfCtu *ctus;
  void *tmp;
  uint64_t tmp_frame, tmp_comp[3];
  uint8_t *classes;
  int32_t pic_w, pic_h, ctus_w, ctus_h, bit_depth, chroma;
};

struct VxAlfStatParams {
  const VxFrameDev *frames;
  long long *luma;
  long long *chroma;
  int32_t frame_first, pic_w, pic_h, ctus_w, ctus_h, bit_depth;
  int32_t clip[2][4];
};

#define VXD_STORE_REC   (128 * 128 * 2)
#define VXD_STORE_UNITS (32 * 32 * (int) sizeof(VxUnit))
#define VXD_STORE_LEVEL (2 * VXD_STORE_REC + VXD_STORE_UNITS)
#define VXD_CTXSNAP     (2 * VXD_NUM_CTX * 2)
#define VXD_OFF_STORE   0
#define VXD_OFF_CTX     (VXD_OFF_STORE + VXD_MAXD * VXD_STORE_LEVEL)
#define VXD_OFF_SLOTS   ((VXD_OFF_CTX + (VXD_MAXD + VXD_NW + 1) * 2 * VXD_CTXSNAP + 255) & ~255)
#define VXD_SLOT_ELEMS  (2 * 4096)
#define VXD_OFF_TMP     (VXD_OFF_SLOTS + VXD_NW * 2 * VXD_SLOT_ELEMS * 2)
struct VxCacheEnt { uint64_t ss; uint8_t kind , dir, mrl, cbf, depth, mts; uint16_t gen ; };
#define VXD_CACHE_ENTRIES (32 * 32 * 5 * 5)
#define VXD_CACHE_DIM   1152
#define VXD_OFF_ORG     (VXD_OFF_TMP + VXD_NW * 2048 * 4)
#define VXD_OFF_LM      (VXD_OFF_ORG + 4096 * 2)
#define VXD_DQ_WAVE     8192
#define VXD_OFF_DQ      ((VXD_OFF_LM + (1024 + 128) * 2 + 255) & ~255)
#define VXD_POOL_ELEMS      32768
#define VXD_POOL_NODE_BYTES (128 * 1024)
#define VXD_POOL_ITEMS      64
struct VxRbItem { double cost; uint64_t dist, bits; int32_t cbf, sum0, test, wave; };
#define VXD_OFF_POOL    ((VXD_OFF_DQ + VXD_NW * VXD_DQ_WAVE + 255) & ~255)
#define VXD_OFF_POOL_COEF  (VXD_OFF_POOL + VXD_POOL_ELEMS * 2)
#define VXD_OFF_POOL_NODES (VXD_OFF_POOL_COEF + VXD_POOL_ELEMS * 2)
#define VXD_OFF_POOL_REC   (VXD_OFF_POOL_NODES + VXD_POOL_NODE_BYTES)
#define VXD_ISP_WAVE    14336
#define VXD_OFF_ISP     ((VXD_OFF_POOL_REC + 2 * VXD_POOL_ITEMS * (int) sizeof(VxRbItem) + 255) & ~255)
#define VXD_OFF_ISP_BEST (VXD_OFF_ISP + VXD_NW * VXD_ISP_WAVE * 2)
#define VXD_OFF_JCCR    ((VXD_OFF_ISP_BEST + 2 * 4096 * 2 + 255) & ~255)
#define VXD_JCCR_WAVE   (6 * 1024 * 2)
#define VXD_OFF_CACHE   ((VXD_OFF_JCCR + VXD_NW * VXD_JCCR_WAVE + 255) & ~255)
#define VXD_OFF_CACHE_LEV (VXD_OFF_CACHE + VXD_CACHE_ENTRIES * (int) sizeof(VxCacheEnt))
#define VXD_OFF_META    (VXD_OFF_CACHE_LEV + VXD_CACHE_DIM * VXD_CACHE_DIM * 2)
#define VXD_SCRATCH_BYTES (VXD_OFF_META + 256)
```

### reduce-complexity-for-intra-coding-of-vvc_amd/csrc/vvcx_kernel.hip

```cpp
#include <hip/hip_runtime.h>
#include <stdint.h>
#define VX_QUAL static __device__ const
#include "vvcx_tables.h"
#include "vvcx_dev.h"
#include "vvcx_mip_dev.h"

#define NT VXD_NT
#if (VXD_NW & (VXD_NW - 1)) == 0
#define VTX ((threadIdx.x + ((((unsigned) blockIdx.x * 0x9E3779B1u) >> 30) << 6)) & (unsigned) (VXD_NT - 1))
#else
__device__ inline unsigned vtx_rotated()
{
  const unsigned t = threadIdx.x + ((((unsigned) blockIdx.x * 0x9E3779B1u) >> 24) % VXD_NW << 6);
  return t >= VXD_NT ? t - VXD_NT : t;
}
#define VTX (vtx_rotated())
#endif
#define NW VXD_NW
#define MAXD VXD_MAXD
#define BUF VXD_BUF
#define NCTX VXD_NUM_CTX
static_assert(VXD_NUM_CTX == VX_NUM_CTX, "vvcx_dev.h and the generated tables disagree on the number of context models");
#define MAX_DOUBLE 1.7e+308
#ifndef VVCX_STAMP
// ... 15 lines not shown
#define TOOL_LFNST (1u << 3)
#define MIPF 0x80
#define TOOL_MTS (1u << 4)
#define TOOL_TS (1u << 5)
#define TOOL_DEPQUANT (1u << 6)
#define TOOL_CCLM (1u << 8)
#define TOOL_JCCR (1u << 9)
#define TOOL_FAST (1u << 12)
#define TOOL_WPP (1u << 13)
enum { LM_CHROMA = 67, MDLM_L = 68, MDLM_T = 69 };
enum { PLANAR = 0, DC = 1, HOR = 18, DIA = 34, VER = 50, VDIA = 66, DM_CHROMA = 70 };
enum { OP_NONE, OP_DONE, OP_LUMA_PREP, OP_STAGE_A, OP_STAGE_B, OP_CHROMA_RD, OP_SAVE_INTRA, OP_SAVE_PIC, OP_RESTORE_PIC,
       OP_CLEAR_UNITS, OP_CTX_COPY, OP_REUSE, OP_FAST, OP_ISP, OP_ISP_END, OP_ISP_PARK };
enum { PH_ENTER, PH_FAST_DONE, PH_RUN, PH_A1_DONE, PH_A2_DONE, PH_B_DONE, PH_INTRA_SAVED, PH_CHILD, PH_CHILD_RET, PH_SPLIT_SAVED, PH_ADVANCE, PH_EXIT, PH_EXIT2, PH_A3_DONE, PH_PASS, PH_NEXT_PASS, PH_ISP };
enum { CTX_CUR = 0, CTX_START = 1, CTX_BEST = 2, CTX_WAVE = 3 };

struct Ctx { uint16_t s0[NCTX], s1[NCTX]; };
struct Cab { int ci; uint64_t bits; };

struct Sum {
  double cost; uint64_t dist, bits;
  int16_t n_cu, f_bt, f_cbf, f_w, f_h, l_bt, l_w, l_h, max_qt, valid;
};

struct Frame {
  int16_t x, y, w, h;
  uint8_t depth, qt, bt, mt, impl_bt, last_split, part_idx, phase;
  uint8_t impl_checked, impl_split, nmodes, did_h, did_v, did_q, do_th, do_tv;
  uint8_t qt_before_bt, max_qt_sub, has_best, cur_mode, cur_split, child, nparts, first;
  uint8_t modes[8];
  uint8_t nb_ok, nbL_lh, nbL_qt, nbA_lw, nbA_qt;
  uint8_t can_mask, ctx_spl, ctx_qt, ctx_hv;
  uint8_t reusing, r_dir, r_mrl, r_cbf, r_mts;
  uint8_t ctx_dirty;
  int16_t px[4], py[4], pw[4], ph[4];
  uint64_t ss;
  double max_cost;
  Sum best, temp;
};

struct Cand { uint8_t mode, mrl; };
struct IspRes { unsigned long long d[4], fb[4]; uint8_t cbf, nrun, mode, split, used, pad_[3]; };
struct Arith { uint32_t low, range, buffered_byte; int32_t bits_left, num_buffered; uint32_t bit_acc; int32_t bit_n; uint32_t n; };

struct CtlState {
  Cand rdList[24]; double rdCost[24]; int rdSize, numRd;
  uint8_t checked[67];
  int n_a2;
  int8_t lfOn, grp, lf, mts, startLf, endLf, skipOther, bestMts, bestLf, considerMts, mtsUsage, testMip, lfSaved, bestValid0;
  uint8_t grpCheck[4], bestSel[4], idxOf[16];
  double dct2Cost, grpBest[4], modeCost[16], bestCost0;
  int lfNum, lfSize, mtsNum; Cand lfList[16], mtsList[16];
  int8_t ispHave, ispPark, ispReqMode, ispReqSplit;
  int8_t testIsp, ispSlot, ispPrev, ispNT, ispBestMode, ispBestSplit, ispNOrig, ispNList, ispRegN, ispHadN, skipMts2, ispBreak, ispStop[2], ispNumTotal[2], ispCandIdx[2], ispNTested[2];
  uint8_t ispTMode[16], ispTInfo[16], ispList[28], ispReg[16], ispHad[24], ispWinMode, ispWinSplit, ispWinTucbf;
  double ispTCost[16], ispBestRd, ispCurBest, noIspCost;
  unsigned long long ispWinDist, ispWinBits;
  alignas(4) int8_t ispPartsOf[2][68]; int8_t ispFirst[2][2];
  uint8_t inv0[16], rdSrc[24];
};

#define BIN_FRAC(st_, bin_) L.t.bin_frac[(unsigned) (st_) ^ ((0u - (unsigned) (bin_)) & 255u)]
struct Tables {
  uint32_t bin_frac[256];
  int32_t  qscale[12], iqscale[12];
  int16_t  ang[32], inv_ang[32];
  int8_t   gauss[128], cubic[128];
  uint8_t  last_prefix[8], mode_shift[8];
  uint8_t  ctx_rate[NCTX + 2], gorice_pars[32], gorice_pos0[96], rice_len[128], group_idx[64], mode_num[36], intra_thr[8];
  uint8_t  cg_scan[84], grp_scan[228];
  uint8_t  cg_inv[84], grp_inv[228];
};

#define DQ_ABS_SINGLE 64
#define RC_LIST 320
#define DQ_TAB_INTS (21 * 6 + 3 * 12 * 2 + 4)
struct WaveRc { uint16_t binbuf[RC_LIST]; uint8_t binsort[RC_LIST + 8]; };
struct alignas(16) WaveScratch { WaveRc rc; };
struct WaveMem {
  WaveScratch ws;
  alignas(16) int32_t tmp[BUF];
  alignas(16) int16_t slot[2 * BUF];
};
#define CI_CUR 0
#define CI_W(w) (1 + (w))
struct Lds {
  Tables t;
  Ctx ctxs[1 + NW];
  alignas(16) int16_t org[BUF];
  alignas(16) WaveMem wm[NW];
  int acc[NW][4][2];
  int16_t refs[4][2][140];
  uint8_t flags[72]; int8_t src_unit[72];
  int cache_gen, cur_stream;
  int dq_abs[DQ_ABS_SINGLE + NW];
  Frame fr[MAXD];
  int op, op_a, op_b, op_c, op_d, op_ch;
  int pre_copy_d;
  int nx, ny, nw, nh, nd;
  Cand cand[64]; union { double cand_cost[64]; IspRes isp_res[NW]; }; int n_cand;
  union { uint2 cand_ipa[64]; int dq_tab[DQ_TAB_INTS]; };
  Cand rd[16]; double rd_cost[16]; uint64_t rd_dist[16]; uint64_t rd_bits[16]; uint8_t rd_cbf[16]; uint8_t rd_mts[16]; int mts_evals[NW]; int n_rd;
  int do_save;
  int wave_best[NW], wave_slot[NW];
  uint8_t rd_wave[16];
  uint8_t rb_pairs[VXD_POOL_ITEMS]; int rb_nb;
  CtlState S; VxUnit cu;
  unsigned mpm[6], mpm_sorted[6]; int mpm_n;
  int16_t mip_n, mip_ctx;
  int16_t isp_ok, isp_pad_;
  int8_t ps_lfnst, ps_mts, ps_grp, isp_wait; int rc_last[NW]; uint8_t rd_lfl[16];
  int8_t spec_n, spec_kind; uint8_t rd_src[16]; int spec_abs[16];
  double isp_limit;
  unsigned long long isp_dist;
  uint8_t isp_nb, isp_park, isp_split, isp_tucbf, isp_win, isp_pad2_[3];
  int lmcs_cadj, lmcs_tab;
  int dc_val[4];
  int cur_tile, frame, ctu_x, ctu_y, tree_ch;
  int d;
  int win_idx, win_wave;
  unsigned long long cu_bits;
  unsigned long long cnt[4];
  VxParams par; VxFrameDev fdv;
  alignas(16) int16_t lm_in[BUF / 2]; union { struct { int16_t lm_top[64], lm_left[64]; }; int ts_tab[36]; }; int lm_info[4], lm_ok, lm_nsatd; int lm_par[2][3][3]; int64_t lm_cost[8];
  int16_t fa_nb[5][4]; int fa_n, fa_res, fa_row, fa_feat[27];
  int wpp_ok, wpp_pos;
  int train_row[MAXD];
  Arith aw; uint8_t *aw_out; uint32_t aw_cap; int colm;
  unsigned long long prof[VVCX_STAMP ? 48 : 1];
};

__shared__ Lds L;
#define PROF(i) L.prof[VVCX_STAMP ? (i) : 0]
#ifdef VVCX_STAMP_ISP
#define ISP_T(n_) long long n_ = clock64()
#define ISP_ADD(slot_, a_, b_) do { if (VTX == 0) PROF(slot_) += (unsigned long long) ((b_) - (a_)); } while (0)
#define ISP_ADD0(slot_, a_, b_) do { PROF(slot_) += (unsigned long long) ((b_) - (a_)); } while (0)
#else
#define ISP_T(n_)
#define ISP_ADD(slot_, a_, b_)
#define ISP_ADD0(slot_, a_, b_)
#endif
#ifndef VX_POISON_LDS
#define VX_POISON_LDS(obj) ((void) 0)
#endif
#ifndef VX_CHECK
#define VX_CHECK(c) ((void) 0)
#endif

__device__ inline int ilog2i(int v) { return 31 - __clz(v); }
__device__ inline int imin(int a, int b) { return a < b ? a : b; }
__device__ inline int imax(int a, int b) { return a > b ? a : b; }
__device__ inline int iabs(int a) { return a < 0 ? -a : a; }
__device__ inline int pow2_log(int d) { return (d & (d - 1)) == 0 ? 31 - __clz(d) : -1; }
__device__ inline int fast_div(int i, int d, int ld) { return ld >= 0 ? i >> ld : i / d; }
__device__ inline int uni(int v) { return __builtin_amdgcn_readfirstlane(v); }
template <typename T> __device__ inline T *uni_p(T *p)
{
  union { T *p; int i[2]; } u; u.p = p;
  u.i[0] = __builtin_amdgcn_readfirstlane(u.i[0]); u.i[1] = __builtin_amdgcn_readfirstlane(u.i[1]);
  return u.p;
}
template <typename T> __device__ inline T *as_lds(T *p) { return (T *) ((char *) &L + (int) ((const char *) p - (const char *) &L)); }
__device__ inline double uni_d(double v)
{
  union { double d; int i[2]; } u; u.d = v;
// ... 1874 lines not shown
  for (int c = wave; c < n_rd; c += NW) {
    const int mode = uni(L.rd[c].mode), mrl = uni(L.rd[c].mrl);
    int16_t *rec = SMALL ? L.wm[wave].slot : slot_rec(scratch, P, wave, cur), *lev = SMALL ? L.wm[wave].slot + BUF : slot_lev(scratch, P, wave, cur);
    if (lane == 0) L.rd_cost[c] = MAX_DOUBLE;
    const int mip = mrl & MIPF;
    Ipa ip; init_pred_params(w, h, 1, mip ? 0 : mode, mip ? 0 : mrl, ip);
    const int set = luma_set(mip ? 0 : mrl, ip.ref_filter);
    const int16_t *top = L.refs[set][0], *left = L.refs[set][1];
    const int dcv = L.dc_val[luma_set(mip ? 0 : mrl, 0)];
    const long long tb0 = STAMP();
    if (mip) wave_pred_mip(rec, w, h, mode, bd, wave, lane);
    else for (int i = lane; i < P; i += 64) { const int py = i >> ilog2i(w), px = i & (w - 1); rec[i] = (int16_t) pred_sample(top, left, w, h, px, py, ip, mode, 1, bd, dcv); }
    wave_sync();
    const long long tb1 = STAMP();
    const int mtsOk = MTS && mts_allowed(p, w, h);
    unsigned test = 1; int sum0 = 0;
    double mbest = MAX_DOUBLE; int cbfDCT2 = 1;
    for (int k = 0; k < (MTS && mtsOk ? 5 : 1); k++) {
    if (!cbfDCT2) break;
    if (!((test >> k) & 1)) continue;
    const int mts = k ? k + 1 : 0;
    if (k) {
      rec = SMALL ? L.wm[wave].slot : slot_rec(scratch, P, wave, cur); lev = SMALL ? L.wm[wave].slot + BUF : slot_lev(scratch, P, wave, cur);
      if (mip) wave_pred_mip(rec, w, h, mode, bd, wave, lane);
      else for (int i = lane; i < P; i += 64) { const int py = i >> ilog2i(w), px = i & (w - 1); rec[i] = (int16_t) pred_sample(top, left, w, h, px, py, ip, mode, 1, bd, dcv); }
      wave_sync();
    }
    if (MTS && k == 1) {
      int sums[5]; sums[0] = sum0;
      for (int q = 1; q < 5; q++) sums[q] = wave_fwd_sumabs<SMALL>(org_tile(scratch, P), rec, wave_tmp(scratch, imin(w, 32) * h, wave), w, h, bd, q + 1, lane);
      const int ls = imax(ilog2i(w), ilog2i(h)) - 2;
      const double fac = ls == 0 ? 1.2 : ls <= 2 ? 1.3 : ls == 3 ? 1.4 : 1.5;
      const double thr = fac * (double) sums[0], thrTS = (double) sums[0];
      int numTests = 0; test = 0;
      for (int q = 0; q < 5; q++) { const int t = (double) sums[q] <= (q == 1 ? thrTS : thr) && numTests <= 3; test |= (unsigned) t << q; numTests += t; }
      test = uni((int) test);
      if (!((test >> 1) & 1)) continue;
    }
    unsigned long long sse; int cbf;
    if (k == 0 && !(MTS && mtsOk)) wave_code_block<SMALL>(org_tile(scratch, P), 0, 0, rec, lev, wave_tmp(scratch, imin(w, 32) * h, wave), w, h, bd, p.qp_tr, lane, sse, cbf);
    else if (k == 0) wave_code_block<SMALL, true>(org_tile(scratch, P), 0, 0, rec, lev, wave_tmp(scratch, imin(w, 32) * h, wave), w, h, bd, p.qp_tr, lane, sse, cbf, -1, &sum0);
    else wave_code_block_mts<SMALL>(org_tile(scratch, P), rec, lev, wave_tmp(scratch, imin(w, 32) * h, wave), w, h, bd, p.qp_tr, mts, lane, sse, cbf);
    if (k) nmts++;
    if (k == 0) { cbfDCT2 = uni(cbf); if (MTS && mtsOk) test = 0x1f; }
    if (k && !uni(cbf)) continue;
    const long long tb2 = STAMP();
    { uint32_t *d = (uint32_t *) &L.ctxs[CI_W(wave)]; const uint32_t *s = (const uint32_t *) &L.ctxs[CI_CUR]; for (int i = lane; i < NCTX; i += 64) d[i] = s[i]; }
    wave_sync();
    double cost = 0;
    Cab cb; cb.ci = CI_W(wave); cb.bits = 0;
    if (lane == 0) {
      enc_intra_luma_pred_mode(cb, L.ny, mode, mrl);
      enc_bin(cb, (unsigned) cbf, VX_CTX_QtCbf[0]);
      if (cbf && mtsOk) enc_mts_idx(cb, mts);
    }
    if (uni(cbf)) residual_coding_wave<SMALL>(cb, 0, lev, w, h, 0, lane, mts > 1);
    if (lane == 0) cost = rd_cost(p, cb.bits, sse);
    if (VVCX_STAMP && VTX == 0) { const long long tb3 = STAMP(); PROF(28) += (unsigned long long) (tb1 - tb0); PROF(29) += (unsigned long long) (tb2 - tb1); PROF(31) += (unsigned long long) (tb3 - tb2); }
    cost = lane0_d(cost);
    if (cost < mbest) {
      mbest = cost;
      if (lane == 0) { L.rd_cost[c] = cost; L.rd_dist[c] = sse; L.rd_bits[c] = cb.bits; L.rd_cbf[c] = (uint8_t) cbf; L.rd_mts[c] = (uint8_t) mts; L.rd_wave[c] = (uint8_t) wave; }
    }
    if (cost < wbest) {
      wbest = cost;
      if (lane == 0) { L.wave_best[wave] = c; L.wave_slot[wave] = SMALL ? 1 : cur; }
      if (SMALL) { int16_t *pr = slot_rec(scratch, P, wave, 1), *pl = slot_lev(scratch, P, wave, 1); for (int i = lane; i < P; i += 64) { pr[i] = rec[i]; pl[i] = lev[i]; } }
      else cur ^= 1;
      { uint32_t *d = (uint32_t *) ctx_ptr(scratch, CTX_START, MAXD + wave, 0); const uint32_t *s = (const uint32_t *) &L.ctxs[CI_W(wave)]; for (int i = lane; i < NCTX; i += 64) d[i] = s[i]; }
    }
    wave_sync();
    }
  }
  if (lane == 0) L.mts_evals[wave] = nmts;
}
template <bool SMALL> __device__ __noinline__ void stage_b_loop_dct2(uint8_t *scratch, int wave, int lane, int w, int h) { stage_b_loop<SMALL, false>(L.par, scratch, wave, lane, w, h); }
template <bool SMALL> __device__ __noinline__ void stage_b_loop_mts(const VxParams &p_, uint8_t *scratch, int wave, int lane, int w, int h) { stage_b_loop<SMALL, true>(L.par, scratch, wave, lane, w, h); (void) p_; }
template <bool SMALL>
__device__ void dq_trellis_phase(uint8_t *scratch, int n, int P, int total, int w, int h, int zo, int wave, int lane, int lfnst = 0, int item0 = 0, int abs0 = 0, int wave_shift = 0)
{
  int16_t *poolCoef = (int16_t *) (scratch + VXD_OFF_POOL_COEF) + (size_t) item0 * P; uint8_t *poolNodes = scratch + VXD_OFF_POOL_NODES + (size_t) item0 * 4 * total;
  const int ipw = imin(16, (int) sizeof(WaveMem) / (240 + 2 * total));
  for (int i0 = ((wave + NW - wave_shift) % NW) * ipw; i0 < n; i0 += NW * ipw)
    wave_depquant_batch<2>(imin(ipw, n - i0), poolCoef + (size_t) i0 * P, P, poolNodes + (size_t) i0 * 4 * total, 4 * total, wave, abs0 + i0,
                        CI_CUR, 0, VX_CTX_QtCbf[0], 0u, w, h, 0, zo, lfnst, lane);
}
template <bool SMALL>
__device__ __noinline__ void stage_b_rounds(uint8_t *scratch, int wave, int lane, int w, int h)
{
  scratch = uni_p(scratch); wave = uni(wave); w = uni(w); h = uni(h);
  const VxParams &p = L.par;
  const int P = w * h, bd = uni(p.bit_depth), total = imin(32, w) * imin(32, h);
  const int mtsOk = mts_allowed(p, w, h);
  const int lfOn = uni((int) (p.tools & TOOL_LFNST)) != 0, psLf = lfOn ? uni((int) L.ps_lfnst) : 0, psMts = lfOn ? uni((int) L.ps_mts) : 0, psGrp = uni((int) L.ps_grp);
  const int pruneOk = mtsOk && !lfOn;
  const int tsOn = lfOn && !psLf && !psMts && ts_allowed(p, w, h);
  int16_t *poolPred = (int16_t *) (scratch + VXD_OFF_POOL), *poolCoef = (int16_t *) (scratch + VXD_OFF_POOL_COEF);
  VxRbItem *recA = (VxRbItem *) (scratch + VXD_OFF_POOL_REC), *recB = recA + VXD_POOL_ITEMS;
  const int capItems = imin(VXD_POOL_ITEMS, imin(VXD_POOL_ELEMS / P, VXD_POOL_NODE_BYTES / (4 * total)));
  const int capCand = imin(16, pruneOk ? imax(1, capItems / 3) : capItems);
  const int n_rd = uni(L.n_rd);
  const int specGen = lfOn && !psLf && !psMts && mtsOk && 2 * n_rd <= capItems && n_rd <= 16;
  const int specGen2 = lfOn && psLf == 1 && !psMts && uni((int) L.S.endLf) >= 2 && 2 * n_rd <= capItems && n_rd <= 16;
  const int specKind = uni((int) L.spec_kind);
  const int specUse = lfOn && uni((int) L.spec_n) > 0 && ((psMts && psGrp == 0 && specKind == 1) || (psLf == 2 && !psMts && specKind == 2 && uni((int) L.spec_n) == n_rd));
  const int specN = uni((int) L.spec_n);
  const int tsEarly = tsOn && NW >= 4 && n_rd <= 16 && (48 + 16) * P <= VXD_POOL_ELEMS, tsAt = tsEarly ? 48 : 0;
  if (lane == 0) L.wave_best[wave] = -1;
  if (tsOn) ts_build_tables();
  dq_build_tables(0);
  double wbest = MAX_DOUBLE; int wkey = 1 << 30;
  int cur = 0, nmts = 0;
  const int16_t *org = org_tile(scratch, P);
  for (int c0 = 0; c0 < n_rd; c0 += capCand) {
    const int nA = imin(capCand, n_rd - c0);
    const long long q0 = STAMP();
    if (!specUse) for (int i = wave; i < nA; i += NW) {
      const int c = c0 + i, mode = uni(L.rd[c].mode), mrl = uni(L.rd[c].mrl), mip = mrl & MIPF;
      int16_t *rec = SMALL ? L.wm[wave].slot : slot_rec(scratch, P, wave, cur), *lev = SMALL ? L.wm[wave].slot + BUF : slot_lev(scratch, P, wave, cur);
      if (mip) wave_pred_mip(rec, w, h, mode, bd, wave, lane);
      else {
        Ipa ip; init_pred_params(w, h, 1, mode, mrl, ip);
        const int set = luma_set(mrl, ip.ref_filter), dcv = L.dc_val[luma_set(mrl, 0)];
        const int16_t *top = L.refs[set][0], *left = L.refs[set][1];
        for (int e = lane; e < P; e += 64) { const int py = e >> ilog2i(w), px = e & (w - 1); rec[e] = (int16_t) pred_sample(top, left, w, h, px, py, ip, mode, 1, bd, dcv); }
      }
      wave_sync();
      for (int e = lane; e < P; e += 64) poolPred[(size_t) i * P + e] = rec[e];
      unsigned long long sse; int cbf, sum0 = 0;
      const int mtsC = psMts ? pass_mts_idx(psGrp, mode) : 0;
      if (mtsC) wave_code_block_mts<SMALL>(org, rec, lev, wave_tmp(scratch, imin(w, 32) * h, wave), w, h, bd, p.qp_tr, mtsC, lane, sse, cbf, -2);
      else wave_code_block<SMALL, true>(org, 0, 0, rec, lev, wave_tmp(scratch, imin(w, 32) * h, wave), w, h, bd, p.qp_tr, lane, sse, cbf, -2, &sum0, 0, 0, 0, psLf, psLf ? lfnst_mode(mip ? PLANAR : mode, w, h) : 0);
      for (int e = lane; e < P; e += 64) poolCoef[(size_t) i * P + e] = lev[e];
      if (lane == 0) { recA[i].sum0 = sum0; recA[i].test = 0; recB[i].sum0 = sum0; }
      if (specGen) {
        wave_code_block_mts<SMALL>(org, rec, lev, wave_tmp(scratch, imin(w, 32) * h, wave), w, h, bd, p.qp_tr, 2, lane, sse, cbf, -2);
        for (int e = lane; e < P; e += 64) poolCoef[(size_t) (nA + i) * P + e] = lev[e];
      }
      if (specGen2) {
        wave_code_block<SMALL>(org, 0, 0, rec, lev, wave_tmp(scratch, imin(w, 32) * h, wave), w, h, bd, p.qp_tr, lane, sse, cbf, -2, nullptr, 0, 0, 0, 2, lfnst_mode(mip ? PLANAR : mode, w, h));
        for (int e = lane; e < P; e += 64) poolCoef[(size_t) (nA + i) * P + e] = lev[e];
      }
    }
    __threadfence_block();
    __syncthreads();
    const long long q1 = STAMP();
    if (!specUse) dq_trellis_phase<SMALL>(scratch, nA, P, total, w, h, psMts, wave, lane, psLf);
    if (specGen) dq_trellis_phase<SMALL>(scratch, nA, P, total, w, h, 1, wave, lane, 0, nA, 32, 1);
    if (specGen2) dq_trellis_phase<SMALL>(scratch, nA, P, total, w, h, 0, wave, lane, 2, nA, 32, 1);
    if (tsEarly && wave >= 2) {
      for (int i = wave - 2; i < nA; i += 2) {
        const int sa = wave_ts_fwd(org, poolPred + (size_t) i * P, poolCoef + (size_t) (48 + i) * P, w, h, bd, lane);
        if (lane == 0) L.rb_pairs[i] = (uint8_t) ((double) sa <= (double) recB[i].sum0);
      }
      __threadfence_block();
      wave_sync();
      int cnt = 0, mine = -1;
      for (int i = wave - 2; i < nA; i += 2) if (L.rb_pairs[i]) { if (cnt == lane) mine = i; cnt++; }
      if (mine >= 0) L.dq_abs[48 + mine] = ts_rdoq_lane(poolCoef + (size_t) (48 + mine) * P, w, h, bd, p.qp_tr);
    }
    __threadfence_block();
    __syncthreads();
    const long long q2 = STAMP();
    if (specGen || specGen2) { if ((int) VTX < nA) L.spec_abs[VTX] = L.dq_abs[32 + VTX]; if (VTX == 0) { L.spec_n = (int8_t) nA; L.spec_kind = (int8_t) (specGen ? 1 : 2); } }
    else if (VTX == 0) L.spec_n = 0;
    for (int i = wave; i < nA; i += NW) {
      const int c = c0 + i, mode = uni(L.rd[c].mode), mrl = uni(L.rd[c].mrl);
// ... 269 lines not shown
      if (lane == 0) {
        enc_intra_chroma_pred_mode(cb, cm, L.colm, L.lm_ok);
        enc_bin(cb, (unsigned) cbfs[0], VX_CTX_QtCbf[1]);
        enc_bin(cb, (unsigned) cbfs[1], VX_CTX_QtCbf[2] + cbfs[0]);
      }
      if (uni(cbfs[0])) residual_coding_wave<SMALL>(cb, 0, levb, w, h, 1, lane);
      if (uni(cbfs[1])) residual_coding_wave<SMALL>(cb, P, levb + P, w, h, 1, lane);
      if (lane == 0) {
        cost = rd_cost(p, cb.bits, dist);
        L.rd_cost[c] = cost; L.rd_dist[c] = dist; L.rd_cbf[c] = (uint8_t) ((cbfs[0] ? 2 : 0) | (cbfs[1] ? 4 : 0));
      }
    }
    cost = lane0_d(cost);
    if (cost < wbest) {
      wbest = cost;
      if (lane == 0) { L.wave_best[wave] = c; L.wave_slot[wave] = SMALL ? 1 : cur; }
      if (SMALL) { int16_t *pr = slot_rec(scratch, 2 * P, wave, 1), *pl = slot_lev(scratch, 2 * P, wave, 1); for (int i = lane; i < 2 * P; i += 64) { pr[i] = recb[i]; pl[i] = levb[i]; } }
      else cur ^= 1;
    }
    wave_sync();
  }
}
__device__ inline int ict_mode(int sign, int mask) { const int m = mask == 1 ? 3 : mask == 2 ? 1 : 2; return sign ? -m : m; }
__device__ inline int ict_fwd(int b, int r, int mode, long long &err)
{
  int v, eb, er;
  switch (mode) {
    case  1: v = (4 * b + 2 * r) / 5; eb = b - v; er = r - (v >> 1); break;
    case -1: v = (4 * b - 2 * r) / 5; eb = b - v; er = r - (-v >> 1); break;
    case  2: v = (b + r) / 2; eb = b - v; er = r - v; break;
    case -2: v = (b - r) / 2; eb = b - v; er = r + v; break;
    case  3: v = (4 * r + 2 * b) / 5; eb = b - (v >> 1); er = r - v; break;
    default: v = (4 * r - 2 * b) / 5; eb = b - (-v >> 1); er = r - v; break;
  }
  err += (long long) eb * eb + (long long) er * er;
  return v;
}
__device__ inline int ict_inv(int c, int mode, int k)
{
  const int am = mode < 0 ? -mode : mode, sc = mode < 0 ? -c : c;
  if (am == 3) return k == 1 ? c : (sc >> 1);
  return k == 0 ? c : (am == 1 ? (sc >> 1) : sc);
}
__device__ inline long long wave_sum_i64(long long v) { return (long long) wave_sum_u64((unsigned long long) v); }

template <bool SMALL>
__device__ __noinline__ void chroma_rd_rounds(uint8_t *scratch, int wave, int lane, int w, int h)
{
  scratch = uni_p(scratch); wave = uni(wave); w = uni(w); h = uni(h);
  const VxParams &p = L.par;
  const int P = w * h, bd = uni(p.bit_depth), total = imin(32, w) * imin(32, h);
  const int16_t *lmin = lm_in_buf(scratch, 2 * P);
  const int16_t *org = org_tile(scratch, 2 * P);
  int16_t *poolPred = (int16_t *) (scratch + VXD_OFF_POOL), *poolCoef = (int16_t *) (scratch + VXD_OFF_POOL_COEF); uint8_t *poolNodes = scratch + VXD_OFF_POOL_NODES;
  if (lane == 0) L.wave_best[wave] = -1;
  dq_build_tables(1);
  double wbest = MAX_DOUBLE;
  int cur = 0;
  const int n_rd = uni(L.n_rd);
  const int psLf = (uni((int) (p.tools & TOOL_LFNST)) && w >= 4 && h >= 4) ? uni((int) L.ps_lfnst) : 0;
  const int jccrOn = uni((int) (p.tools & TOOL_JCCR)) != 0;
  const int cadj = P > 4 ? uni(L.lmcs_cadj) : 0;
  int njoint = 0;
#define CHROMA_LFMODE(c_) (psLf ? lfnst_mode((uni((int) L.rd[c_].mode) >= LM_CHROMA && uni((int) L.rd[c_].mode) <= MDLM_T) ? uni(L.colm) : uni((int) L.rd[c_].mrl), w, h) : 0)
  for (int c = wave; c < n_rd; c += NW) {
    const int fm = uni(L.rd[c].mrl), lfm = CHROMA_LFMODE(c);
    int16_t *recb = SMALL ? L.wm[wave].slot : slot_rec(scratch, 2 * P, wave, cur), *levb = SMALL ? L.wm[wave].slot + BUF : slot_lev(scratch, 2 * P, wave, cur);
    for (int k = 0; k < 2; k++) {
      int16_t *rec = recb + k * P, *lev = levb + k * P;
      chroma_pred_wave(rec, lmin, k, fm, w, h, bd, lane);
      wave_sync();
      for (int e = lane; e < P; e += 64) poolPred[(size_t) (2 * c + k) * P + e] = rec[e];
      unsigned long long sse; int cbf;
      wave_code_block<SMALL>(org, k * P, k * P, rec, lev, wave_tmp(scratch, imin(w, 32) * h, wave), w, h, bd, p.qp_tr_c[k], lane, sse, cbf, -2, nullptr, k + 1, CI_CUR, 0, psLf, lfm, 0, -1, cadj);
      for (int e = lane; e < P; e += 64) poolCoef[(size_t) (2 * c + k) * P + e] = lev[e];
      wave_sync();
    }
  }
  __threadfence_block();
  __syncthreads();
  {
    const int ipw = imin(16, (int) sizeof(WaveMem) / (240 + 2 * total));
    for (int i0 = wave * ipw; i0 < n_rd; i0 += NW * ipw)
      wave_depquant_batch<2>(imin(ipw, n_rd - i0), poolCoef + (size_t) (2 * i0) * P, 2 * P, poolNodes + (size_t) (2 * i0) * 4 * total, 8 * total, wave, i0,
                          CI_CUR, 0, VX_CTX_QtCbf[1], 0u, w, h, 1, 0, psLf, lane);
  }
  __threadfence_block();
  __syncthreads();
  const bool crBatch = 4 * (240 + 2 * total) <= (int) (sizeof(WaveScratch) + sizeof(int32_t) * BUF);
  for (int c0 = 0; c0 < n_rd; c0 += NW) {
    const int c = c0 + wave; const bool have = c < n_rd;
    const int cm = have ? uni(L.rd[c].mode) : 0;
    const int lfm = have ? CHROMA_LFMODE(c) : 0;
    int16_t *recb = SMALL ? L.wm[wave].slot : slot_rec(scratch, 2 * P, wave, cur), *levb = SMALL ? L.wm[wave].slot + BUF : slot_lev(scratch, 2 * P, wave, cur);
    unsigned long long dist = 0; int cbfs[2] = { 0, 0 };
    double compCost = 0; int jccr = 0;
    if (have) {
      { uint32_t *d = (uint32_t *) &L.ctxs[CI_W(wave)]; const uint32_t *s_ = (const uint32_t *) &L.ctxs[CI_CUR]; for (int e = lane; e < NCTX; e += 64) d[e] = s_[e]; }
      for (int e = lane; e < P; e += 64) { recb[e] = poolPred[(size_t) (2 * c) * P + e]; levb[e] = poolCoef[(size_t) (2 * c) * P + e]; }
      wave_sync();
      cbfs[0] = uni(L.dq_abs[c]) > 0;
      unsigned long long sse; int cbf2;
      wave_code_block<SMALL>(org, 0, 0, recb, levb, wave_tmp(scratch, imin(w, 32) * h, wave), w, h, bd, p.qp_tr_c[0], lane, sse, cbf2, cbfs[0], nullptr, 1, CI_W(wave), 0, psLf, lfm, 0, -1, cadj);
      dist += (unsigned long long) (p.dist_weight[0] * (double) sse);
      { Cab cb; cb.ci = CI_W(wave); cb.bits = 0; if (lane == 0) enc_bin(cb, (unsigned) cbfs[0], VX_CTX_QtCbf[1]); if (cbfs[0]) residual_coding_wave<SMALL>(cb, 0, levb, w, h, 1, lane);
        double c0 = 0; if (lane == 0) c0 = rd_cost(p, cb.bits, dist); compCost = lane0_d(c0); }
      wave_sync();
      if (lane == 0) L.rb_pairs[wave] = (uint8_t) cbfs[0];
    }
    __threadfence_block();
    __syncthreads();
    {
      const int n4 = imin(NW, n_rd - c0);
      unsigned mask = 0; for (int i = 0; i < n4; i++) mask |= (unsigned) L.rb_pairs[i] << i;
      if (crBatch) { if (wave == 0) wave_depquant_batch<0>(n4, poolCoef + (size_t) (2 * c0 + 1) * P, 2 * P, poolNodes + (size_t) (2 * c0 + 1) * 4 * total, 8 * total, 0, c0,
                                                        CI_W(0), 1, VX_CTX_QtCbf[2], mask, w, h, 2, 0, psLf, lane); }
      else if (have) wave_depquant_batch<0>(1, poolCoef + (size_t) (2 * c + 1) * P, 0, poolNodes + (size_t) (2 * c + 1) * 4 * total, 0, wave, c,
                                         CI_W(wave), 0, VX_CTX_QtCbf[2], (unsigned) cbfs[0], w, h, 2, 0, psLf, lane);
    }
    __threadfence_block();
    __syncthreads();
    if (have) {
      int16_t *rec = recb + P, *lev = levb + P;
      for (int e = lane; e < P; e += 64) { rec[e] = poolPred[(size_t) (2 * c + 1) * P + e]; lev[e] = poolCoef[(size_t) (2 * c + 1) * P + e]; }
      wave_sync();
      cbfs[1] = uni(L.dq_abs[c]) > 0;
      unsigned long long sse; int cbf2;
      wave_code_block<SMALL>(org, P, P, rec, lev, wave_tmp(scratch, imin(w, 32) * h, wave), w, h, bd, p.qp_tr_c[1], lane, sse, cbf2, cbfs[1], nullptr, 2, CI_W(wave), cbfs[0], psLf, lfm, 0, -1, cadj);
      const unsigned long long distCr = (unsigned long long) (p.dist_weight[1] * (double) sse);
      dist += distCr;
      { Cab cb; cb.ci = CI_W(wave); cb.bits = 0;
        if (lane == 0) { enc_bin(cb, (unsigned) cbfs[1], VX_CTX_QtCbf[2] + cbfs[0]); if (jccrOn && (cbfs[0] | cbfs[1])) enc_bin(cb, 0u, VX_CTX_JointCbCrFlag + ((cbfs[0] ? 2 : 0) | (cbfs[1] ? 1 : 0)) - 1); }
        if (cbfs[1]) residual_coding_wave<SMALL>(cb, P, lev, w, h, 1, lane);
        double c1 = 0; if (lane == 0) c1 = compCost + rd_cost(p, cb.bits, distCr); compCost = lane0_d(c1); }
      wave_sync();
      if (jccrOn && (cbfs[0] | cbfs[1])) {
        int16_t *jb = (int16_t *) (scratch + VXD_OFF_JCCR + (size_t) wave * VXD_JCCR_WAVE);
        int16_t *jres = jb, *jout = jb + 1024, *jlev = jb + 2048, *brec = jb + 3072, *blev = jb + 5120;
        const int16_t *pCb = poolPred + (size_t) (2 * c) * P, *pCr = poolPred + (size_t) (2 * c + 1) * P;
        const int sign = uni(L.fdv.jccr_sign);
        long long d0 = 0, d1 = 0, e1 = 0, e2 = 0, e3 = 0;
        for (int e = lane; e < P; e += 64) {
          int b = org[e] - pCb[e], r = org[P + e] - pCr[e];
          if (cadj) { b = lmcs_scale_fwd(b, cadj, bd); r = lmcs_scale_fwd(r, cadj, bd); }
          d0 += (long long) b * b; d1 += (long long) r * r;
          ict_fwd(b, r, ict_mode(sign, 1), e1); ict_fwd(b, r, ict_mode(sign, 2), e2); ict_fwd(b, r, ict_mode(sign, 3), e3);
        }
        d0 = wave_sum_i64(d0); d1 = wave_sum_i64(d1); e1 = wave_sum_i64(e1); e2 = wave_sum_i64(e2); e3 = wave_sum_i64(e3);
        long long min1 = d0 < d1 ? d0 : d1, min2 = 0x7fffffffffffffffll; int m1 = 0, m2 = 0;
        for (int m = 1; m < 4; m++) {
          const long long pd = m == 1 ? e1 : m == 2 ? e2 : e3;
          if (pd < min1) { m2 = m1; min2 = min1; m1 = m; min1 = pd; } else if (pd < min2) { m2 = m; min2 = pd; }
        }
        int masks[2], nm = 0;
        if (m1) masks[nm++] = m1;
        if (m2 && ((min2 < (9 * min1) / 8) || (!m1 && min2 < (3 * min1) / 2))) masks[nm++] = m2;
        nm = uni(nm);
        unsigned long long bestJDist = 0;
        for (int q = 0; q < nm; q++) {
          const int mask = uni(masks[q]), mode = ict_mode(sign, mask), comp = (mask >> 1) ? 1 : 2;
          for (int e = lane; e < P; e += 64) {
            long long dm = 0; int b = org[e] - pCb[e], r = org[P + e] - pCr[e];
            if (cadj) { b = lmcs_scale_fwd(b, cadj, bd); r = lmcs_scale_fwd(r, cadj, bd); }
            jres[e] = (int16_t) ict_fwd(b, r, mode, dm); jout[e] = 0;
          }
          wave_sync();
          njoint++;
          unsigned long long sseJ; int cbfJ;
          wave_code_block<false>(jres, 0, 0, jout, jlev, wave_tmp(scratch, imin(w, 32) * h, wave), w, h, bd, mask == 3 ? p.qp_tr_j : p.qp_tr_c[comp - 1], lane, sseJ, cbfJ, -1, nullptr, comp, CI_CUR, 0, psLf, lfm, 1, 2 + mask);
          if (!cbfJ) continue;
          unsigned long long sCb = 0, sCr = 0;
          const int mx = (1 << bd) - 1;
          for (int e = lane; e < P; e += 64) {
            const int cj = jout[e];
            int rb = ict_inv(cj, mode, 0), rr = ict_inv(cj, mode, 1);
            if (cadj) { rb = lmcs_scale_inv((int) (int16_t) rb, cadj, bd); rr = lmcs_scale_inv((int) (int16_t) rr, cadj, bd); }
            int vb = pCb[e] + rb, vr = pCr[e] + rr;
            vb = vb < 0 ? 0 : vb > mx ? mx : vb; vr = vr < 0 ? 0 : vr > mx ? mx : vr;
            jres[e] = (int16_t) vb; jout[e] = (int16_t) vr;
            const int db = org[e] - vb, dr = org[P + e] - vr;
            sCb += (unsigned long long) (db * db); sCr += (unsigned long long) (dr * dr);
          }
          sCb = wave_sum_u64(sCb); sCr = wave_sum_u64(sCr);
          const unsigned long long dJ = (unsigned long long) (p.dist_weight[0] * (double) sCb) + (unsigned long long) (p.dist_weight[1] * (double) sCr);
          { uint32_t *d = (uint32_t *) &L.ctxs[CI_W(wave)]; const uint32_t *s_ = (const uint32_t *) &L.ctxs[CI_CUR]; for (int e = lane; e < NCTX; e += 64) d[e] = s_[e]; }
          wave_sync();
          Cab cb; cb.ci = CI_W(wave); cb.bits = 0;
          if (lane == 0) { enc_bin(cb, (unsigned) (mask >> 1), VX_CTX_QtCbf[1]); enc_bin(cb, (unsigned) (mask & 1), VX_CTX_QtCbf[2] + (mask >> 1)); enc_bin(cb, 1u, VX_CTX_JointCbCrFlag + mask - 1); }
          residual_coding_wave<false>(cb, 0, jlev, w, h, 1, lane);
          double cj = 0; if (lane == 0) cj = rd_cost(p, cb.bits, dJ);
          cj = lane0_d(cj);
          if (cj < compCost) {
            compCost = cj; jccr = mask; bestJDist = dJ;
            for (int e = lane; e < P; e += 64) { brec[e] = jres[e]; brec[P + e] = jout[e]; blev[e] = jlev[e]; }
          }
          wave_sync();
        }
        if (jccr) {
          dist = bestJDist; cbfs[0] = jccr >> 1; cbfs[1] = jccr & 1;
          for (int e = lane; e < P; e += 64) { recb[e] = brec[e]; recb[P + e] = brec[P + e]; levb[e] = (jccr >> 1) ? blev[e] : 0; levb[P + e] = (jccr >> 1) ? 0 : blev[e]; }
// ... 1488 lines not shown
        Frame &f = L.fr[0];
        f.x = (int16_t) ctu_x; f.y = (int16_t) ctu_y; f.w = 128; f.h = 128; f.depth = 0; f.qt = 0; f.bt = 0; f.mt = 0; f.impl_bt = 0;
        f.last_split = 0; f.part_idx = 0; f.impl_checked = 0; f.ss = 0; f.max_cost = MAX_DOUBLE; f.phase = PH_ENTER;
      }
      if (ch == 1) ctx_copy_all(&L.ctxs[CI_CUR], ctx_ptr(scratch, CTX_START, MAXD + NW, 0));
      __syncthreads();
      run_tree<T>(p, fd, scratch);
      if (tid == 0) { const Sum &b = L.fr[0].best; res.dist += b.dist; res.bits += b.bits; res.cost += b.cost; res.n_cu += b.n_cu; }
      __syncthreads();
    }
    ctx_copy_all(&L.ctxs[CI_CUR], ctx_ptr(scratch, CTX_START, MAXD + NW, 0));
    __syncthreads();
    if (tid == 0) {
      const long long t0 = STAMP();
      advance_ctx_ctu<T>(p, fd, sd.tile, ctu_x, ctu_y);
      if (p.payload) writer_end_of_ctu(sd.done_before + t + 1 == sd.tile_ctus, sd.sub == p.nsub - 1);
      if (VVCX_STAMP) PROF(12) += (unsigned long long) (STAMP() - t0);
      p.results[sd.first_task + t] = res;
    }
    __syncthreads();
    if (p.tools & TOOL_WPP) {
      if (sd.done_before + t == 0) ctx_copy_all((Ctx *) (p.wpp_sync + (size_t) sidx * 2 * NCTX), &L.ctxs[CI_CUR]);
      __threadfence();
      __syncthreads();
      if (tid == 0) { wpp_publish(p.wpp_progress + sidx, sd.done_before + t + 1); atomicAdd(p.wpp_sched + 2, 1); }
    }
  }
  ctx_copy_all(carry, &L.ctxs[CI_CUR]);
  if (tid == 0 && (p.tools & TOOL_CU_REUSE)) *(uint32_t *) (scratch + VXD_OFF_META) = (uint32_t) L.cache_gen;
  if (tid == 0 && p.payload) writer_suspend(p, sidx);
#ifdef VX_DBG_STREAM
  if (tid == 0) fprintf(stderr, "stream %d sub %d done_before %d tasks %d slot %d cnt %llu %llu %llu %llu gen %d\n", stream_idx, sd.sub, sd.done_before, sd.n_tasks, (int) blockIdx.x, L.cnt[0], L.cnt[1], L.cnt[2], L.cnt[3], L.cache_gen);
#endif
  if (tid == 0) { for (int i = 0; i < 4; i++) atomicAdd(&p.counters[i], L.cnt[i]); if (VVCX_STAMP) for (int i = 0; i < 48; i++) atomicAdd(&p.counters[4 + i], PROF(i)); }
  return pos0 + t;
}

extern "C" __global__ void __launch_bounds__(NT, VXD_WPE) vvcx_leaf_dist_kernel(const int16_t *a, const int16_t *b, int w, int h, int16_t *scr, unsigned long long *out)
{
  const int wave = uni(VTX >> 6), lane = VTX & 63, P = w * h;
  if (wave != 0) return;
  const int16_t *pa = a + (size_t) blockIdx.x * P, *pb = b + (size_t) blockIdx.x * P;
  unsigned long long sad, satd;
  wave_sad_satd<false>(pa, pb, scr + (size_t) blockIdx.x * P, w, h, lane, sad, satd);
  unsigned long long sse = 0;
  for (int i = lane; i < P; i += 64) { const int d = pa[i] - pb[i]; sse += (unsigned long long) (d * d); }
  sse = wave_sum_u64(sse);
  if (lane == 0) { out[blockIdx.x * 3 + 0] = sad; out[blockIdx.x * 3 + 1] = satd; out[blockIdx.x * 3 + 2] = sse; }
}
extern "C" __global__ void __launch_bounds__(NT, VXD_WPE) vvcx_leaf_trq_kernel(const int16_t *org, int16_t *rec, int16_t *lev, int32_t *tmp, int w, int h, int bd, int qp,
                                                                               unsigned long long *out)
{
  if (VTX == 0) L.par.tools = 0;
  load_tables();
  __syncthreads();
  const int wave = uni(VTX >> 6), lane = VTX & 63, P = w * h;
  if (wave != 0) return;
  unsigned long long sse; int cbf;
  wave_code_block<false>(org + (size_t) blockIdx.x * P, 0, 0, rec + (size_t) blockIdx.x * P, lev + (size_t) blockIdx.x * P, tmp + (size_t) blockIdx.x * 2048, w, h, bd, qp, lane, sse, cbf);
  if (lane == 0) { out[blockIdx.x * 2] = sse; out[blockIdx.x * 2 + 1] = (unsigned long long) cbf; }
}
extern "C" __global__ void __launch_bounds__(NT, VXD_WPE) vvcx_leaf_dq_kernel(VxParams p, const uint16_t *ctx, const int16_t *org, int16_t *rec, int16_t *lev, int32_t *tmp,
                                                                              int w, int h, int qp, int comp, int mts, int cbf_cb, unsigned long long *out, int lf, int lfdir)
{
  if (VTX == 0) { L.par = p; L.lmcs_tab = 0; }
  load_tables();
  for (int i = VTX; i < NCTX; i += NT) { L.ctxs[CI_CUR].s0[i] = ctx[i]; L.ctxs[CI_CUR].s1[i] = ctx[NCTX + i]; }
  __syncthreads();
  const int wave = uni(VTX >> 6), lane = VTX & 63, P = w * h, bd = uni(p.bit_depth);
  if (wave != 0) return;
  const size_t b = (size_t) blockIdx.x * P;
  unsigned long long sse; int cbf;
  if (P <= BUF) {
    for (int i = lane; i < P; i += 64) { L.org[i] = org[b + i]; L.wm[0].slot[i] = rec[b + i]; }
    wave_sync();
    if (mts > 1) wave_code_block_mts<true>(nullptr, nullptr, nullptr, nullptr, w, h, bd, qp, mts, lane, sse, cbf);
    else wave_code_block<true>(nullptr, 0, 0, nullptr, nullptr, nullptr, w, h, bd, qp, lane, sse, cbf, -1, nullptr, comp, CI_CUR, cbf_cb, lf, lf ? lfnst_mode(lfdir, w, h) : 0);
    wave_sync();
    for (int i = lane; i < P; i += 64) { rec[b + i] = L.wm[0].slot[i]; lev[b + i] = L.wm[0].slot[BUF + i]; }
  } else if (mts > 1) wave_code_block_mts<false>(org + b, rec + b, lev + b, tmp + (size_t) blockIdx.x * 2048, w, h, bd, qp, mts, lane, sse, cbf);
  else wave_code_block<false>(org + b, 0, 0, rec + b, lev + b, tmp + (size_t) blockIdx.x * 2048, w, h, bd, qp, lane, sse, cbf, -1, nullptr, comp, CI_CUR, cbf_cb, lf, lf ? lfnst_mode(lfdir, w, h) : 0);
  if (lane == 0) { out[blockIdx.x * 2] = sse; out[blockIdx.x * 2 + 1] = (unsigned long long) cbf; }
}
extern "C" __global__ void __launch_bounds__(NT, VXD_WPE) vvcx_leaf_ts_kernel(VxParams p, const uint16_t *ctx, const int16_t *resi, int16_t *lev, int16_t *resi_out, int32_t *tmp,
                                                                              int w, int h, int qp, int *out, unsigned long long *bits)
{
  if (VTX == 0) L.par = p;
  load_tables();
  for (int i = VTX; i < NCTX; i += NT) { L.ctxs[CI_CUR].s0[i] = ctx[i]; L.ctxs[CI_CUR].s1[i] = ctx[NCTX + i]; }
  __syncthreads();
  ts_build_tables();
  __syncthreads();
  const int wave = uni(VTX >> 6), lane = VTX & 63, P = w * h, bd = uni(p.bit_depth);
  if (wave != 0) return;
  const size_t b = (size_t) blockIdx.x * P;
  unsigned long long sse; int cbf, sum0 = 0;
  wave_code_block<false, true>(resi + b, 0, 0, resi_out + b, lev + b, tmp + (size_t) blockIdx.x * 2048, w, h, bd, qp, lane, sse, cbf, -2, &sum0);
  wave_sync();
  const int sa = wave_ts_fwd(resi + b, resi_out + b, lev + b, w, h, bd, lane);
  wave_sync();
  int a = 0;
  if (lane == 0) a = ts_rdoq_lane(lev + b, w, h, bd, qp);
  a = __builtin_amdgcn_readlane(a, 0);
  wave_sync();
  wave_ts_recon(resi + b, resi_out + b, lev + b, w, h, bd, qp, a > 0, lane, sse, 1);
  if (lane == 0) {
    Cab cb; cb.ci = CI_CUR; cb.bits = 0;
    if (a > 0) rc_ts_serial(cb, lev + b, w, h);
    out[blockIdx.x * 2] = a; out[blockIdx.x * 2 + 1] = sa <= sum0; bits[blockIdx.x] = cb.bits;
  }
}
extern "C" __global__ void __launch_bounds__(NT, VXD_WPE) vvcx_leaf_isp_kernel(VxParams p, const uint16_t *ctx, const int16_t *org, int16_t *rec, int16_t *lev, int32_t *tmp,
                                                                               int w, int h, int qp, int cbf_ctx, unsigned long long *out)
{
  if (VTX == 0) { L.par = p; L.lmcs_tab = 0; }
  load_tables();
  for (int i = VTX; i < NCTX; i += NT) { L.ctxs[CI_CUR].s0[i] = ctx[i]; L.ctxs[CI_CUR].s1[i] = ctx[NCTX + i]; }
  __syncthreads();
  const int wave = uni(VTX >> 6), lane = VTX & 63, P = w * h;
  if (wave != 0) return;
  const size_t b = (size_t) blockIdx.x * P;
  unsigned long long sse; int cbf;
  wave_code_block_isp<false>(org + b, rec + b, lev + b, w, tmp + (size_t) blockIdx.x * 2048, lev + b, p.scratch + (size_t) blockIdx.x * p.scratch_per_stream, w, h, p.bit_depth, qp, lane, sse, cbf, -1, CI_CUR, cbf_ctx);
  if (lane == 0) { out[blockIdx.x * 2] = sse; out[blockIdx.x * 2 + 1] = (unsigned long long) cbf; }
}
template <typename T>
__device__ void leaf_pred(const VxParams &p, const VxLeafPred *cases, int16_t *out, const int *out_off)
{
  const VxFrameDev &fd = p.frames[0];
  const VxLeafPred c = cases[blockIdx.x];
  if (VTX == 0) { L.par = p; L.fdv = p.frames[0]; }
  load_tables();
  if (VTX == 0) { L.cur_tile = 0; L.nx = c.x; L.ny = c.y; L.nw = c.w; L.nh = c.h; }
  __syncthreads();
  const int luma = c.comp == 0;
  int16_t *o = out + out_off[blockIdx.x];
  if (c.mode >= LM_CHROMA) {
    uint8_t *scratch = p.scratch + (size_t) blockIdx.x * p.scratch_per_stream;
    for (int k = 1; k <= 2; k++) build_refs<T>(p, fd, k, c.x, c.y, c.w, c.h, 0, 1);
    cclm_prepare<T>(p, fd, scratch, c.x, c.y, c.w, c.h);
    if ((VTX >> 6) == 0) chroma_pred_wave(o, lm_in_buf(scratch, 2 * c.w * c.h), c.comp - 1, c.mode, c.w, c.h, p.bit_depth, VTX & 63);
    return;
  }
  build_refs<T>(p, fd, c.comp, c.x, c.y, c.w, c.h, 0, luma ? 3 : 1);
  __syncthreads();
  if (VTX < 4) {
    const int s = VTX;
    if (luma ? s != 1 : s == c.comp - 1) L.dc_val[s] = dc_value(L.refs[s][0], L.refs[s][1], c.w, c.h, luma ? (s == 0 ? 0 : s == 2 ? 1 : 3) : 0);
  }
  __syncthreads();
  Ipa ip; init_pred_params(c.w, c.h, luma, c.mode, c.mrl, ip);
  const int set = luma ? luma_set(c.mrl, ip.ref_filter) : c.comp - 1;
  const int dcv = L.dc_val[luma ? luma_set(c.mrl, 0) : c.comp - 1];
  for (int i = VTX; i < c.w * c.h; i += NT) { const int py = i >> ilog2i(c.w), px = i & (c.w - 1); o[i] = (int16_t) pred_sample(L.refs[set][0], L.refs[set][1], c.w, c.h, px, py, ip, c.mode, luma, p.bit_depth, dcv); }
}
extern "C" __global__ void __launch_bounds__(NT, VXD_WPE) vvcx_leaf_pred_kernel_u8(VxParams p, const VxLeafPred *cases, int16_t *out, const int *out_off) { leaf_pred<uint8_t>(p, cases, out, out_off); }
extern "C" __global__ void __launch_bounds__(NT, VXD_WPE) vvcx_leaf_pred_kernel_u16(VxParams p, const VxLeafPred *cases, int16_t *out, const int *out_off) { leaf_pred<uint16_t>(p, cases, out, out_off); }
extern "C" __global__ void __launch_bounds__(NT, VXD_WPE) vvcx_leaf_cabac_kernel(uint16_t *io, int rate, const uint8_t *bins, int nbins, unsigned long long *bits)
{
  load_tables();
  __syncthreads();
  if (VTX == 0) {
    const int ctx = 0; L.t.ctx_rate[0] = (uint8_t) rate;
    L.ctxs[CI_CUR].s0[ctx] = io[0]; L.ctxs[CI_CUR].s1[ctx] = io[1];
    Cab cb; cb.ci = CI_CUR; cb.bits = 0;
    for (int i = 0; i < nbins; i++) enc_bin(cb, bins[i], ctx);
// ... 174 lines not shown
```

### reduce-complexity-for-intra-coding-of-vvc_amd/vvcx.py

```python
import ctypes as C
import os
import numpy as np

HERE = os.path.dirname(os.path.abspath(__file__))
DEFAULT_LIB = os.path.join(HERE, "libvvcx.so")
TOOL_MRL = 1
TOOL_LFNST = 1 << 3
TOOL_JCCR = 1 << 9
TOOL_MIP = 1 << 1
TOOL_MTS = 1 << 4
TOOL_DEPQUANT = 1 << 6
TOOL_CU_REUSE = 1 << 11
TOOL_CCLM = 1 << 8
TOOL_FAST = 1 << 12
TOOL_TS = 1 << 5
TOOL_RDOQ = 1 << 7
TOOL_ISP = 1 << 2
TOOL_LMCS = 1 << 10
TOOL_WPP = 1 << 13
TOOLS_DEFAULT = TOOL_MRL | TOOL_CU_REUSE


class VvcxError(RuntimeError):
    pass
# ... 465 lines not shown
        self._chk(self.L.vvcx_get_tus(self.h, frame, tus.ctypes.data, len(tus), C.byref(n)))
        return tus[:n.value].copy()

    def last_kernel_ms(self):
        return float(self.L.vvcx_last_kernel_ms(self.h))

    def profile(self):
        c = np.zeros(48, np.uint64)
        self._chk(self.L.vvcx_get_profile(self.h, c.ctypes.data))
        return c

    def counters(self):
        c = np.zeros(4, np.uint64)
        self._chk(self.L.vvcx_get_counters(self.h, c.ctypes.data))
        return c


PRED_CASE_DTYPE = np.dtype([("comp", "<i4"), ("x", "<i4"), ("y", "<i4"), ("w", "<i4"), ("h", "<i4"), ("mode", "<i4"), ("mrl", "<i4")])


def _chk(L, rc):
    if rc != 0:
        raise VvcxError("vvcx error %d: %s" % (rc, L.vvcx_last_error().decode()))


def distortion_batch(a, b, w, h, device=0, lib_path=None):
    L = load_library(lib_path)
    a = np.ascontiguousarray(a, np.int16).ravel(); b = np.ascontiguousarray(b, np.int16).ravel()
    n = a.size // (w * h)
    out = np.zeros((n, 3), np.uint64)
    _chk(L, L.vvcx_distortion_batch(a.ctypes.data, b.ctypes.data, w, h, n, out.ctypes.data, device))
    return out


def ctx_init(qp, lib_path=None):
    L = load_library(lib_path)
    s0 = np.zeros(386, np.uint16); s1 = np.zeros(386, np.uint16)
    _chk(L, L.vvcx_ctx_init(int(qp), s0.ctypes.data, s1.ctypes.data))
    return s0, s1


def cabac_code_bins(s0, s1, ctx, bins, device=0, lib_path=None):
    L = load_library(lib_path)
    a = np.array([s0], np.uint16); b = np.array([s1], np.uint16); bins = np.ascontiguousarray(bins, np.uint8); bits = np.zeros(1, np.uint64)
    _chk(L, L.vvcx_cabac_code_bins(a.ctypes.data, b.ctypes.data, int(ctx), bins.ctypes.data, len(bins), bits.ctypes.data, device))
    return int(bits[0]), int(a[0]), int(b[0])


def rd_cost_batch(lam, frac_bits, dist, device=0, lib_path=None):
    L = load_library(lib_path)
    fb = np.ascontiguousarray(frac_bits, np.uint64); d = np.ascontiguousarray(dist, np.uint64); out = np.zeros(len(fb), np.float64)
    _chk(L, L.vvcx_rd_cost_batch(float(lam), fb.ctypes.data, d.ctypes.data, len(fb), out.ctypes.data, device))
    return out


def scan_order(w, h, device=0, lib_path=None):
    L = load_library(lib_path)
    idx = np.zeros(min(w, 32) * min(h, 32), np.uint16)
    _chk(L, L.vvcx_scan_order(w, h, idx.ctypes.data, device))
    return idx


def transform_quant_batch(org, pred, w, h, bit_depth, qp, device=0, lib_path=None):
    L = load_library(lib_path)
    org = np.ascontiguousarray(org, np.int16).ravel(); pred = np.ascontiguousarray(pred, np.int16).ravel()
    n = org.size // (w * h)
    lev = np.zeros(org.size, np.int16); rec = np.zeros(org.size, np.int16); sse = np.zeros(n, np.uint64); cbf = np.zeros(n, np.uint8)
    _chk(L, L.vvcx_transform_quant_batch(org.ctypes.data, pred.ctypes.data, w, h, bit_depth, qp, n, lev.ctypes.data, rec.ctypes.data, sse.ctypes.data, cbf.ctypes.data, device))
    return lev.reshape(n, h, w), rec.reshape(n, h, w), sse, cbf


def depquant_batch(org, pred, w, h, bit_depth, qp, comp, mts_idx, cbf_cb, lam, s0, s1, device=0, lib_path=None):
    L = load_library(lib_path)
    org = np.ascontiguousarray(org, np.int16).ravel(); pred = np.ascontiguousarray(pred, np.int16).ravel()
    s0 = np.ascontiguousarray(s0, np.uint16); s1 = np.ascontiguousarray(s1, np.uint16)
    n = org.size // (w * h)
    lev = np.zeros(org.size, np.int16); rec = np.zeros(org.size, np.int16); sse = np.zeros(n, np.uint64); cbf = np.zeros(n, np.uint8)
    L.vvcx_depquant_batch.argtypes = [C.c_void_p, C.c_void_p] + [C.c_int] * 7 + [C.c_double, C.c_void_p, C.c_void_p, C.c_int] + [C.c_void_p] * 4 + [C.c_int]
    _chk(L, L.vvcx_depquant_batch(org.ctypes.data, pred.ctypes.data, w, h, bit_depth, qp, comp, mts_idx, cbf_cb, lam, s0.ctypes.data, s1.ctypes.data, n,
                                  lev.ctypes.data, rec.ctypes.data, sse.ctypes.data, cbf.ctypes.data, device))
    return lev.reshape(n, h, w), rec.reshape(n, h, w), sse, cbf


def transform_skip_batch(resi, w, h, bit_depth, qp, lam, s0, s1, device=0, lib_path=None):
    L = load_library(lib_path)
    resi = np.ascontiguousarray(resi, np.int16).ravel()
    s0 = np.ascontiguousarray(s0, np.uint16); s1 = np.ascontiguousarray(s1, np.uint16)
    n = resi.size // (w * h)
    lev = np.zeros(resi.size, np.int16); out = np.zeros(resi.size, np.int16); a = np.zeros(n, np.int32); keep = np.zeros(n, np.uint8); bits = np.zeros(n, np.uint64)
    L.vvcx_transform_skip_batch.argtypes = [C.c_void_p] + [C.c_int] * 4 + [C.c_double, C.c_void_p, C.c_void_p, C.c_int] + [C.c_void_p] * 5 + [C.c_int]
    _chk(L, L.vvcx_transform_skip_batch(resi.ctypes.data, w, h, bit_depth, qp, lam, s0.ctypes.data, s1.ctypes.data, n, lev.ctypes.data, out.ctypes.data, a.ctypes.data,
                                        keep.ctypes.data, bits.ctypes.data, device))
    return lev.reshape(n, h, w), out.reshape(n, h, w), a, keep, bits


def deblock_cu_table(planes, rows, bit_depth, qp, qp_c, beta_offset_div2=0, tc_offset_div2=0, device=0, lib_path=None):
    L = load_library(lib_path)
    out = [np.ascontiguousarray(p).astype(np.uint16) for p in planes]
    rows = np.ascontiguousarray(rows, np.int32)
    h, w = out[0].shape
    L.vvcx_deblock_cu_table.argtypes = [C.c_int] * 8 + [C.c_void_p, C.c_int] + [C.c_void_p] * 3 + [C.c_int]
    _chk(L, L.vvcx_deblock_cu_table(w, h, bit_depth, qp, int(qp_c[0]), int(qp_c[1]), beta_offset_div2, tc_offset_div2, rows.ctypes.data, len(rows),
                                    out[0].ctypes.data, out[1].ctypes.data, out[2].ctypes.data, device))
    return out


def isp_tu_batch(org, pred, tw, th, bit_depth, qp, lam, prev_cbf, cbf_inferred, s0, s1, device=0, lib_path=None):
    L = load_library(lib_path)
    org = np.ascontiguousarray(org, np.int16).ravel(); pred = np.ascontiguousarray(pred, np.int16).ravel()
    s0 = np.ascontiguousarray(s0, np.uint16); s1 = np.ascontiguousarray(s1, np.uint16)
    n = org.size // (tw * th)
    lev = np.zeros(org.size, np.int16); rec = np.zeros(org.size, np.int16); sse = np.zeros(n, np.uint64); cbf = np.zeros(n, np.uint8)
    L.vvcx_isp_tu_batch.argtypes = [C.c_void_p, C.c_void_p] + [C.c_int] * 4 + [C.c_double, C.c_int, C.c_int, C.c_void_p, C.c_void_p, C.c_int] + [C.c_void_p] * 4 + [C.c_int]
    _chk(L, L.vvcx_isp_tu_batch(org.ctypes.data, pred.ctypes.data, tw, th, bit_depth, qp, lam, int(prev_cbf), int(cbf_inferred), s0.ctypes.data, s1.ctypes.data, n,
                                lev.ctypes.data, rec.ctypes.data, sse.ctypes.data, cbf.ctypes.data, device))
    return lev.reshape(n, th, tw), rec.reshape(n, th, tw), sse, cbf


def lfnst_depquant_batch(org, pred, w, h, bit_depth, qp, comp, lfnst_idx, intra_dir, cbf_cb, lam, s0, s1, device=0, lib_path=None):
    L = load_library(lib_path)
    org = np.ascontiguousarray(org, np.int16).ravel(); pred = np.ascontiguousarray(pred, np.int16).ravel()
    s0 = np.ascontiguousarray(s0, np.uint16); s1 = np.ascontiguousarray(s1, np.uint16)
    n = org.size // (w * h)
    lev = np.zeros(org.size, np.int16); rec = np.zeros(org.size, np.int16); sse = np.zeros(n, np.uint64); cbf = np.zeros(n, np.uint8)
    L.vvcx_lfnst_depquant_batch.argtypes = [C.c_void_p, C.c_void_p] + [C.c_int] * 8 + [C.c_double, C.c_void_p, C.c_void_p, C.c_int] + [C.c_void_p] * 4 + [C.c_int]
    _chk(L, L.vvcx_lfnst_depquant_batch(org.ctypes.data, pred.ctypes.data, w, h, bit_depth, qp, comp, lfnst_idx, intra_dir, cbf_cb, lam, s0.ctypes.data, s1.ctypes.data, n,
                                        lev.ctypes.data, rec.ctypes.data, sse.ctypes.data, cbf.ctypes.data, device))
    return lev.reshape(n, h, w), rec.reshape(n, h, w), sse, cbf
```

Before: 181.7.

## Widen batched depquant trellis to 16 lanes per item and parallelize setup scans

New measurement: 182.0, median of 5. No clear change (+0.2%).

```diff
diff --git a/include/vvcx.h b/include/vvcx.h
--- a/include/vvcx.h
+++ b/include/vvcx.h
@@ -173,6 +173,8 @@
                          const uint16_t *s0, const uint16_t *s1, int n, int16_t *lev, int16_t *rec, uint64_t *sse, uint8_t *cbf, int device);
 int  vvcx_lfnst_depquant_batch(const int16_t *org, const int16_t *pred, int w, int h, int bit_depth, int qp, int comp, int lfnst_idx, int intra_dir, int cbf_cb, double lambda,
                                const uint16_t *s0, const uint16_t *s1, int n, int16_t *lev, int16_t *rec, uint64_t *sse, uint8_t *cbf, int device);
+int  vvcx_leaf_dq_batch(const int16_t *coef, int w, int h, int bit_depth, int qp, int comp, int cbf_cb, double lambda, const uint16_t *s0, const uint16_t *s1, int n,
+                        int zero_out, int lfnst, int tab, int16_t *lev, int32_t *abs_sum, int device);
 int  vvcx_transform_skip_batch(const int16_t *resi, int w, int h, int bit_depth, int qp, double lambda, const uint16_t *s0, const uint16_t *s1, int n,
                                int16_t *lev, int16_t *resi_out, int32_t *abs_sum, uint8_t *keep, uint64_t *frac_bits, int device);
 int  vvcx_isp_tu_batch(const int16_t *org, const int16_t *pred, int tw, int th, int bit_depth, int qp, double lambda, int prev_cbf, int cbf_inferred,
diff --git a/reduce-complexity-for-intra-coding-of-vvc_amd/csrc/vvcx_api.hip b/reduce-complexity-for-intra-coding-of-vvc_amd/csrc/vvcx_api.hip
--- a/reduce-complexity-for-intra-coding-of-vvc_amd/csrc/vvcx_api.hip
+++ b/reduce-complexity-for-intra-coding-of-vvc_amd/csrc/vvcx_api.hip
@@ -45,6 +45,7 @@
 extern "C" __global__ void vvcx_deblock_kernel_u16(VxDeblockParams p);
 extern "C" __global__ void vvcx_jccr_sign_kernel_u8(VxFrameDev *frames, int wc, int hc);
 extern "C" __global__ void vvcx_jccr_sign_kernel_u16(VxFrameDev *frames, int wc, int hc);
+extern "C" __global__ void vvcx_leaf_dq_batch_kernel(VxParams p, const uint16_t *ctx, int16_t *coef, uint8_t *nodes, int n, int w, int h, int comp, int cbf_cb, int zo, int lfnst, int tab, int *abs_out);
 extern "C" __global__ void vvcx_leaf_dq_kernel(VxParams p, const uint16_t *ctx, const int16_t *org, int16_t *rec, int16_t *lev, int32_t *tmp, int w, int h, int qp, int comp, int mts, int cbf_cb, unsigned long long *out, int lf, int lfdir);
 extern "C" __global__ void vvcx_leaf_ts_kernel(VxParams p, const uint16_t *ctx, const int16_t *resi, int16_t *lev, int16_t *resi_out, int32_t *tmp, int w, int h, int qp, int *out, unsigned long long *bits);
 extern "C" __global__ void vvcx_lmcs_map_kernel_u8(const uint8_t *src, uint8_t *dst, int w, int h, int stride, const int16_t *lut);
@@ -1816,6 +1817,32 @@
   return depquant_batch_impl(org, pred, w, h, bit_depth, qp, comp, 0, cbf_cb, lambda, s0, s1, n, lev, rec, sse, cbf, device, lfnst_idx, intra_dir);
 }
 
+extern "C" int vvcx_leaf_dq_batch(const int16_t *coef, int w, int h, int bit_depth, int qp, int comp, int cbf_cb, double lambda, const uint16_t *s0, const uint16_t *s1, int n,
+                                  int zero_out, int lfnst, int tab, int16_t *lev, int32_t *abs_sum, int device)
+{
+  if (!coef || !lev || !abs_sum || !s0 || !s1 || n < 0 || n > 16 || !pow2_block(w, h) || (bit_depth != 8 && bit_depth != 10) || qp < 0 || qp > 75 || comp < 0 || comp > 2 ||
+      !(lambda > 0.0) || tab < 0 || tab > 2 || (zero_out && comp != 0)) return fail(VVCX_ERR_ARG, "bad argument");
+  const int total = (w < 32 ? w : 32) * (h < 32 ? h : 32);
+  if ((tab == 2 ? VXD_DQ_LEAF_ROOM2 : VXD_DQ_LEAF_ROOM01 - (tab == 1 ? VXD_DQ_LEAF_TAB : 0)) < 240 + 2 * total) return fail(VVCX_ERR_ARG, "block too big for this table mode");
+  if (n == 0) return VVCX_OK;
+  ON_DEVICE(device);
+  const size_t elems = (size_t) n * w * h;
+  DevBuf<int16_t> dcoef; DevBuf<uint16_t> dctx; DevBuf<VxDqConst> dtab; DevBuf<uint8_t> dnodes; DevBuf<int32_t> dabs;
+  HIPCHK(dcoef.alloc(elems)); HIPCHK(dctx.alloc(2 * VXD_NUM_CTX)); HIPCHK(dtab.alloc(48)); HIPCHK(dnodes.alloc((size_t) n * 4 * total)); HIPCHK(dabs.alloc(16));
+  HIPCHK(hipMemcpy(dcoef.p, coef, elems * 2, hipMemcpyHostToDevice));
+  { uint16_t kept[2 * VXD_NUM_CTX]; ctx_from_reference_order(s0, s1, kept); HIPCHK(hipMemcpy(dctx.p, kept, sizeof kept, hipMemcpyHostToDevice)); }
+  VxDqConst tabq[48]; memset(tabq, 0, sizeof tabq);
+  for (int lsum = 2; lsum <= 12; lsum++) tabq[comp * 16 + lsum] = dq_consts_of(lsum, bit_depth, qp, lambda);
+  HIPCHK(hipMemcpy(dtab.p, tabq, sizeof tabq, hipMemcpyHostToDevice));
+  VxParams p; memset(&p, 0, sizeof p);
+  p.bit_depth = bit_depth; p.tools = VVCX_TOOL_DEPQUANT; p.dq_consts = dtab.p;
+  hipLaunchKernelGGL(vvcx_leaf_dq_batch_kernel, dim3(1), dim3(VXD_NT), 0, 0, p, dctx.p, dcoef.p, dnodes.p, n, w, h, comp, cbf_cb, zero_out, (w >= 4 && h >= 4) ? lfnst : 0, tab, dabs.p);
+  HIPCHK(hipGetLastError());
+  HIPCHK(hipMemcpy(lev, dcoef.p, elems * 2, hipMemcpyDeviceToHost));
+  HIPCHK(hipMemcpy(abs_sum, dabs.p, (size_t) n * 4, hipMemcpyDeviceToHost));
+  return VVCX_OK;
+}
+
 extern "C" int vvcx_isp_tu_batch(const int16_t *org, const int16_t *pred, int tw, int th, int bit_depth, int qp, double lambda, int prev_cbf, int cbf_inferred,
                                  const uint16_t *s0, const uint16_t *s1, int n, int16_t *lev, int16_t *rec, uint64_t *sse, uint8_t *cbf, int device)
 {
diff --git a/reduce-complexity-for-intra-coding-of-vvc_amd/csrc/vvcx_depquant_dev.h b/reduce-complexity-for-intra-coding-of-vvc_amd/csrc/vvcx_depquant_dev.h
--- a/reduce-complexity-for-intra-coding-of-vvc_amd/csrc/vvcx_depquant_dev.h
+++ b/reduce-complexity-for-intra-coding-of-vvc_amd/csrc/vvcx_depquant_dev.h
@@ -104,6 +104,8 @@
 __device__ inline int dq_gtx_off(int ch, int diag) { return ch ? (diag < 1 ? 6 : 1) : (diag < 1 ? 16 : diag < 3 ? 11 : diag < 10 ? 6 : 1); }
 
 #define DQ_TAB_BYTES (4 * DQ_TAB_INTS)
+#define DQ_ITEM_BYTES(wide_) ((wide_) ? 432 : 240)
+__device__ inline bool dq_wide_fits(int n_items, int total, int tab, int room) { return n_items <= 4 && n_items * (DQ_ITEM_BYTES(true) + 2 * total) + (tab == 1 ? DQ_TAB_BYTES : 0) <= room; }
 #ifdef VVCX_STAMP_DQ
 #define DQ_T(n_) const long long n_ = clock64()
 #define DQ_U(n_) n_ = clock64()
@@ -125,10 +127,10 @@
 }
 __device__ inline void dq_build_tables(int ch) { dq_fill_tables(L.dq_tab, CI_CUR, ch, (int) VTX, NT); __syncthreads(); }
 template <int TAB>
-__device__ __noinline__ void wave_depquant_batch(int n_items, int16_t *cf_base, int cf_stride, uint8_t *nodes, int node_stride, int wk_wave, int abs0,
+__device__ __noinline__ void wave_depquant_batch(int room, int n_items, int16_t *cf_base, int cf_stride, uint8_t *nodes, int node_stride, int wk_wave, int abs0,
                                                  int ci0, int ci_step, int cbf_ctx0, unsigned cbf_mask, int w, int h, int comp, int zo, int lfnst, int lane, int qidx = -1)
 {
-  n_items = uni(n_items); w = uni(w); h = uni(h); comp = uni(comp); zo = uni(zo); lfnst = uni(lfnst); ci0 = uni(ci0); ci_step = uni(ci_step); cbf_ctx0 = uni(cbf_ctx0);
+  room = uni(room); n_items = uni(n_items); w = uni(w); h = uni(h); comp = uni(comp); zo = uni(zo); lfnst = uni(lfnst); ci0 = uni(ci0); ci_step = uni(ci_step); cbf_ctx0 = uni(cbf_ctx0);
   cf_base = uni_p(cf_base); nodes = uni_p(nodes); cf_stride = uni(cf_stride); node_stride = uni(node_stride); abs0 = uni(abs0); cbf_mask = (unsigned) uni((int) cbf_mask); qidx = uni(qidx);
   uint8_t *wk = (uint8_t *) &L.wm[uni(wk_wave)];
   const int ch = comp ? 1 : 0, lw = ilog2i(w), lh = ilog2i(h);
@@ -144,41 +146,49 @@
   const uint8_t *grp_inv = L.t.grp_inv + 15 * (wsbb - 1) + wsbb * (hsbb - 1);
   int effW = w, effH = h, zeroOut = 0;
   if (zo && comp == 0) { effH = h == 32 ? 16 : h; effW = w == 32 ? 16 : w; zeroOut = effH < h || effW < w; }
-  const int item = lane >> 2, k = lane & 3, qbase = lane & ~3;
-  const bool valid = item < n_items;
+  const bool wide = dq_wide_fits(n_items, total, TAB, room);
+  const int lsh = wide ? 4 : 2, LPI = 1 << lsh;
+  const int item = lane >> lsh, sub = lane & (LPI - 1), k = lane & 3, qbase = lane & ~(LPI - 1);
+  const bool ivalid = item < n_items, valid = ivalid && sub < 4;
+  VX_CHECK(n_items >= 1 && n_items * LPI <= 64);
   DQ_T(t0);
-  const int it0 = valid ? item : 0;
+  const int it0 = ivalid ? item : 0;
   int16_t *cf = cf_base + it0 * cf_stride;
   uint8_t *nd = nodes + (size_t) it0 * node_stride;
   int *lastb = (int *) wk + it0 * 20;
   uint16_t *trel = (uint16_t *) (wk + n_items * 80) + it0 * total;
   uint16_t *tmrows = (uint16_t *) (wk + n_items * (80 + 2 * total)) + it0 * 80;
+  uint32_t *stage = (uint32_t *) (wk + n_items * (240 + 2 * total)) + (wide ? it0 * 48 : 0);
   const int node_room = node_stride ? node_stride : VXD_DQ_WAVE;
   VX_CHECK((total >> lcg) * 64 <= node_room);
   if (valid) for (int e = k; e < 80; e += 4) tmrows[e] = 0;
   const int ci = ci0 + it0 * ci_step;
-  const int cbf_ctx = cbf_ctx0 < 0 ? -1 : cbf_ctx0 + (int) ((cbf_mask >> it0) & 1u);
   int start = total - 1;
   if (lfnst > 0 && w >= 4 && h >= 4) start = ((w == 4 && h == 4) || (w == 8 && h == 8)) ? 7 : 15;
   int first = -1, top = -1;
   {
     const int thr = q.thres / (int) (4 * q.qscale);
-    for (int i = 0; i < n_items; i++) {
-      const int16_t *c = cf_base + i * cf_stride;
-      int found = -1;
-      for (int t = start | 63; t >= 63 && found < 0; t -= 64) {
-        const int sp = t - lane;
-        bool hit = false;
-        if (sp <= start) {
-          const int blk = scan_blk(geo, sp), x = blk & (w - 1), y = blk >> lw;
-          hit = !(zeroOut && (x >= effW || y >= effH)) && iabs((int) c[blk]) > thr;
+    unsigned pend = (unsigned) uni((int) ((1u << n_items) - 1u));
+    for (int t = start | 63; t >= 63 && pend; t -= 64) {
+      const int sp = t - lane;
+      int blk = 0; bool in = false;
+      if (sp <= start) { blk = scan_blk(geo, sp); const int x = blk & (w - 1), y = blk >> lw; in = !(zeroOut && (x >= effW || y >= effH)); }
+      for (int i0 = 0; i0 < n_items; i0 += 4) {
+        if (!((pend >> i0) & 15u)) continue;
+        int v[4];
+#pragma unroll
+        for (int j = 0; j < 4; j++) v[j] = (in && i0 + j < n_items) ? (int) cf_base[(i0 + j) * cf_stride + blk] : 0;
+#pragma unroll
+        for (int j = 0; j < 4; j++) {
+          const unsigned long long m = __ballot(in && iabs(v[j]) > thr);
+          if (((pend >> (i0 + j)) & 1u) && m) {
+            const int found = uni(t - (__ffsll(m) - 1));
+            if (item == i0 + j) first = found;
+            top = imax(top, found);
+            pend &= ~(1u << (i0 + j));
+          }
         }
-        const unsigned long long m = __ballot(hit);
-        if (m) found = t - (__ffsll(m) - 1);
-      }
-      found = uni(found);
-      if (item == i) first = found;
-      top = imax(top, found);
+      }
     }
   }
   DQ_T(t1);
@@ -190,7 +200,7 @@
   }
   DqRate R; R.ci = ci; R.g1Base = VX_CTX_GtxFlag[2 + ch]; R.g2Base = VX_CTX_GtxFlag[ch]; R.parBase = VX_CTX_ParFlag[ch]; R.sbbBase = VX_CTX_SigCoeffGroup[ch];
   const int sigSet = VX_CTX_SigFlag[ch + 2 * imax(k - 1, 0)];
-  int *tabBase = TAB == 2 ? L.dq_tab : (int *) (wk + n_items * (240 + 2 * total));
+  int *tabBase = TAB == 2 ? L.dq_tab : (int *) (wk + n_items * (DQ_ITEM_BYTES(wide) + 2 * total));
   if (TAB == 1) dq_fill_tables(tabBase, ci, ch, lane, 64);
   const int *levTab = tabBase, *sigTab = tabBase + 21 * 6, *sbbTab = sigTab + 3 * 12 * 2; const uint8_t *riceTab = L.t.rice_len;
   const int *mySig = sigTab + imax(k - 1, 0) * 24;
@@ -202,22 +212,24 @@
   };
   auto riceBits = [&](int rpar, unsigned v) -> int { return TAB ? (int) riceTab[rpar * 32 + (int) v] << 15 : dq_rice_bits(rpar, v); };
   auto sbbBits = [&](int sbbc, int bin) -> int { return TAB ? sbbTab[sbbc * 2 + bin] : dq_fb(ci, R.sbbBase + sbbc, bin); };
-  if (valid) {
-    const int cbfDelta = cbf_ctx >= 0 ? dq_fb(ci, cbf_ctx, 1) - dq_fb(ci, cbf_ctx, 0) : 0;
-    for (int e = k; e < 20; e += 4) {
-      const int xy = e >= 10, id = xy ? e - 10 : e;
-      const int size = xy ? h : w, l2 = ilog2i(size);
-      const int base = (xy ? VX_CTX_LastY : VX_CTX_LastX)[ch];
-      const int sh = comp == 0 ? (l2 + 1) >> 2 : imin(2, size >> 3), lo = comp == 0 ? L.t.last_prefix[l2] : 0;
-      const int maxId = L.t.group_idx[imin(32, size) - 1];
-      if (id <= maxId) {
-        unsigned sum = 0;
-        for (int j = 0; j < id; j++) sum += (unsigned) dq_fb(ci, base + lo + (j >> sh), 1);
-        unsigned b = sum + (id > 3 ? (unsigned) ((id - 2) >> 1) << 15 : 0u) + (unsigned) (xy ? cbfDelta : 0);
-        if (id < maxId) b += (unsigned) dq_fb(ci, base + lo + (id >> sh), 0);
-        lastb[e] = (int) b;
-      }
-    }
+  for (int i0 = 0; i0 < n_items; i0 += 3) {
+    const int li = lane / 20, e = lane - li * 20, it = i0 + li;
+    const bool on = lane < 60 && it < n_items;
+    const int xy = e >= 10, id = xy ? e - 10 : e;
+    const int size = xy ? h : w, l2 = ilog2i(size);
+    const int base = (xy ? VX_CTX_LastY : VX_CTX_LastX)[ch];
+    const int sh = comp == 0 ? (l2 + 1) >> 2 : imin(2, size >> 3), lo = comp == 0 ? L.t.last_prefix[l2] : 0;
+    const int maxId = L.t.group_idx[imin(32, size) - 1];
+    const int cie = ci0 + (on ? it : 0) * ci_step;
+    unsigned more = 0, stop = 0, tail = 0;
+    if (on && id < maxId) { more = (unsigned) dq_fb(cie, base + lo + (id >> sh), 1); stop = (unsigned) dq_fb(cie, base + lo + (id >> sh), 0); }
+    if (on && xy && cbf_ctx0 >= 0) { const int cc = cbf_ctx0 + (int) ((cbf_mask >> it) & 1u); tail = (unsigned) (dq_fb(cie, cc, 1) - dq_fb(cie, cc, 0)); }
+    unsigned sum = more;
+#pragma unroll
+    for (int d = 1; d < 16; d <<= 1) { const unsigned u = (unsigned) __shfl((int) sum, lane - d); if (id >= d) sum += u; }
+    const unsigned b = (sum - more) + (id > 3 ? (unsigned) ((id - 2) >> 1) << 15 : 0u) + tail + stop;
+    VX_CHECK(maxId < 10);
+    if (on && id <= maxId) ((int *) wk)[it * 20 + e] = (int) b;
   }
   wave_sync();
   DQ_T(t2);
@@ -231,12 +243,12 @@
     cur = s0; prv = s0; skp.cost = s0.cost; skp.pk = s0.pk; skp.rem = s0.rem; skp.anc = 0;
   }
   long long decCost = 0x7fffffffffffffffll >> 2;
-  if (valid) for (int sp = k; sp <= first; sp += 4) trel[sp] = (uint16_t) cf[scan_blk(geo, sp)];
+  if (ivalid) for (int sp = sub; sp <= first; sp += LPI) trel[sp] = (uint16_t) cf[scan_blk(geo, sp)];
   wave_sync();
   unsigned eosW = 0;
-  if (lane < gs) {
+  if ((wide ? sub : lane) < gs) {
     const int off = cg_tab_off(lcw, lch);
-    const int xy = L.t.cg_scan[off + lane], gx = xy & 15, gy = xy >> 4;
+    const int xy = L.t.cg_scan[off + (wide ? sub : lane)], gx = xy & 15, gy = xy >> 4;
 #pragma unroll
     for (int n = 0; n < 5; n++) {
       const int xx = gx + (n == 0 ? 1 : n == 1 ? 2 : n == 2 ? 1 : 0), yy = gy + (n == 2 ? 1 : n == 3 ? 1 : n == 4 ? 2 : 0);
@@ -409,28 +421,61 @@
         const unsigned fR = gR >= 0 ? (unsigned) (anc >> (4 * (gR - g))) & 15u : 0u, fB = gB >= 0 ? (unsigned) (anc >> (4 * (gB - g))) & 15u : 0u;
         const unsigned fD = gD >= 0 ? (unsigned) (anc >> (4 * (gD - g))) & 15u : 0u;
         const int sigN = ((fR & 8u) || (fB & 8u)) ? 1 : 0;
-        typedef unsigned dq_v16u __attribute__((vector_size(64)));
-        dq_v16u nv = { 0, 0, 0, 0, 0, 0, 0, 0, 0, 0, 0, 0, 0, 0, 0, 0 };
-        if (alive) {
-          VX_CHECK(!(fR & 7u) || (gR >= g && gR - g < 16 && (gR * 4 + (int) (fR & 7u) - 1) * 16 + 16 <= node_room));
-          VX_CHECK(!(fB & 7u) || (gB >= g && gB - g < 16 && (gB * 4 + (int) (fB & 7u) - 1) * 16 + 16 <= node_room));
-          VX_CHECK(!(fD & 7u) || (gD >= g && gD - g < 16 && (gD * 4 + (int) (fD & 7u) - 1) * 16 + 16 <= node_room));
-          if (fR & 7u) { const VX_GLOBAL uint32_t *p_ = (const VX_GLOBAL uint32_t *) (nd + (size_t) (gR * 4 + (int) (fR & 7u) - 1) * 16); nv[4] = p_[0]; nv[5] = p_[1]; nv[6] = p_[2]; nv[7] = p_[3]; }
-          if (fB & 7u) { const VX_GLOBAL uint32_t *p_ = (const VX_GLOBAL uint32_t *) (nd + (size_t) (gB * 4 + (int) (fB & 7u) - 1) * 16); nv[8] = p_[0]; nv[9] = p_[1]; nv[10] = p_[2]; nv[11] = p_[3]; }
-          if (fD & 7u) { const VX_GLOBAL uint32_t *p_ = (const VX_GLOBAL uint32_t *) (nd + (size_t) (gD * 4 + (int) (fD & 7u) - 1) * 16); nv[12] = p_[0]; nv[13] = p_[1]; nv[14] = p_[2]; nv[15] = p_[3]; }
-        }
-        for (int id = 0; id < gs; id++) {
-          const unsigned wrd = (unsigned) __builtin_amdgcn_readlane((int) eosW, id);
-          int sumAbs = 0, sumAbs1 = 0, sumNum = 0;
-#pragma unroll
-          for (int n = 0; n < 5; n++) {
-            const unsigned f = (wrd >> (6 * n)) & 63u;
-            if (f & 3u) {
-              const int a = (int) ((nv[(f & 3u) * 4 + (f >> 4)] >> (((f >> 2) & 3u) << 3)) & 255u);
-              sumAbs += a; sumAbs1 += imin(4 + (a & 1), a); sumNum += a != 0;
+        if (wide) {
+          if (alive) {
+            VX_CHECK(!(fR & 7u) || (gR >= g && gR - g < 16 && (gR * 4 + (int) (fR & 7u) - 1) * 16 + 16 <= node_room));
+            VX_CHECK(!(fB & 7u) || (gB >= g && gB - g < 16 && (gB * 4 + (int) (fB & 7u) - 1) * 16 + 16 <= node_room));
+            VX_CHECK(!(fD & 7u) || (gD >= g && gD - g < 16 && (gD * 4 + (int) (fD & 7u) - 1) * 16 + 16 <= node_room));
+            U4 nR = { 0, 0, 0, 0 }, nB = nR, nD = nR;
+            if (fR & 7u) { const VX_GLOBAL uint32_t *p_ = (const VX_GLOBAL uint32_t *) (nd + (size_t) (gR * 4 + (int) (fR & 7u) - 1) * 16); nR.a = p_[0]; nR.b = p_[1]; nR.c = p_[2]; nR.d = p_[3]; }
+            if (fB & 7u) { const VX_GLOBAL uint32_t *p_ = (const VX_GLOBAL uint32_t *) (nd + (size_t) (gB * 4 + (int) (fB & 7u) - 1) * 16); nB.a = p_[0]; nB.b = p_[1]; nB.c = p_[2]; nB.d = p_[3]; }
+            if (fD & 7u) { const VX_GLOBAL uint32_t *p_ = (const VX_GLOBAL uint32_t *) (nd + (size_t) (gD * 4 + (int) (fD & 7u) - 1) * 16); nD.a = p_[0]; nD.b = p_[1]; nD.c = p_[2]; nD.d = p_[3]; }
+            uint32_t *st = stage + k * 12;
+            st[0] = nR.a; st[1] = nR.b; st[2] = nR.c; st[3] = nR.d; st[4] = nB.a; st[5] = nB.b; st[6] = nB.c; st[7] = nB.d; st[8] = nD.a; st[9] = nD.b; st[10] = nD.c; st[11] = nD.d;
+          }
+          const unsigned live = (unsigned) (__ballot(alive) >> qbase) & 15u;
+          wave_sync();
+          if (ivalid && sub < gs) {
+            const uint8_t *sb = (const uint8_t *) stage;
+#pragma unroll
+            for (int s = 0; s < 4; s++) if ((live >> s) & 1u) {
+              int sumAbs = 0, sumAbs1 = 0, sumNum = 0;
+#pragma unroll
+              for (int n = 0; n < 5; n++) {
+                const unsigned f = (eosW >> (6 * n)) & 63u;
+                if (f & 3u) {
+                  const int a = (int) sb[s * 48 + ((int) (f & 3u) - 1) * 16 + (int) (f >> 2)];
+                  sumAbs += a; sumAbs1 += imin(4 + (a & 1), a); sumNum += a != 0;
+                }
+              }
+              tmrows[s * 16 + sub] = (uint16_t) (sumNum + (sumAbs1 << 3) + (imin(127, sumAbs) << 8));
             }
           }
-          if (alive) tmrows[k * 16 + id] = (uint16_t) (sumNum + (sumAbs1 << 3) + (imin(127, sumAbs) << 8));
+          wave_sync();
+        } else {
+          typedef unsigned dq_v16u __attribute__((vector_size(64)));
+          dq_v16u nv = { 0, 0, 0, 0, 0, 0, 0, 0, 0, 0, 0, 0, 0, 0, 0, 0 };
+          if (alive) {
+            VX_CHECK(!(fR & 7u) || (gR >= g && gR - g < 16 && (gR * 4 + (int) (fR & 7u) - 1) * 16 + 16 <= node_room));
+            VX_CHECK(!(fB & 7u) || (gB >= g && gB - g < 16 && (gB * 4 + (int) (fB & 7u) - 1) * 16 + 16 <= node_room));
+            VX_CHECK(!(fD & 7u) || (gD >= g && gD - g < 16 && (gD * 4 + (int) (fD & 7u) - 1) * 16 + 16 <= node_room));
+            if (fR & 7u) { const VX_GLOBAL uint32_t *p_ = (const VX_GLOBAL uint32_t *) (nd + (size_t) (gR * 4 + (int) (fR & 7u) - 1) * 16); nv[4] = p_[0]; nv[5] = p_[1]; nv[6] = p_[2]; nv[7] = p_[3]; }
+            if (fB & 7u) { const VX_GLOBAL uint32_t *p_ = (const VX_GLOBAL uint32_t *) (nd + (size_t) (gB * 4 + (int) (fB & 7u) - 1) * 16); nv[8] = p_[0]; nv[9] = p_[1]; nv[10] = p_[2]; nv[11] = p_[3]; }
+            if (fD & 7u) { const VX_GLOBAL uint32_t *p_ = (const VX_GLOBAL uint32_t *) (nd + (size_t) (gD * 4 + (int) (fD & 7u) - 1) * 16); nv[12] = p_[0]; nv[13] = p_[1]; nv[14] = p_[2]; nv[15] = p_[3]; }
+          }
+          for (int id = 0; id < gs; id++) {
+            const unsigned wrd = (unsigned) __builtin_amdgcn_readlane((int) eosW, id);
+            int sumAbs = 0, sumAbs1 = 0, sumNum = 0;
+  #pragma unroll
+            for (int n = 0; n < 5; n++) {
+              const unsigned f = (wrd >> (6 * n)) & 63u;
+              if (f & 3u) {
+                const int a = (int) ((nv[(f & 3u) * 4 + (f >> 4)] >> (((f >> 2) & 3u) << 3)) & 255u);
+                sumAbs += a; sumAbs1 += imin(4 + (a & 1), a); sumNum += a != 0;
+              }
+            }
+            if (alive) tmrows[k * 16 + id] = (uint16_t) (sumNum + (sumAbs1 << 3) + (imin(127, sumAbs) << 8));
+          }
         }
         if (alive) {
           pk = dq_put(pk, 0, 5, 0); pk = dq_put(pk, 8, 2, 0); pk = dq_put(pk, 5, 3, k + 1); pk = dq_put(pk, 16, 2, sigN + 1);
@@ -458,40 +503,39 @@
   for (int s = 0; s < 4; s++) { const long long c = dq_shfl_i64(decCost, qbase + s); if (c < minCost) { prev = s; minCost = c; } }
   int nPath = 0;
   if (k == 0 && valid) {
-    int sp = 0, absSum = 0;
+    int sp = 0;
     if (first < 0) prev = -2;
     while (prev >= 0) {
       VX_CHECK(sp >= 0 && sp <= first && prev < 4);
       const int e = (trel[sp] >> (4 * prev)) & 15, src = e >> 1;
-      int lev = 0;
-      if (e & 1) {
-        const long long scaledOrg = (long long) iabs((int) cf[scan_blk(geo, sp)]) * q.qscale;
-        const int i = src == 1 ? prev : src == 2 ? ((prev & 1) ? 3 : 0) : ((prev & 1) ? 1 : 2);
-        const int qIdx0 = dq_qidx0(q, scaledOrg);
-        lev = (qIdx0 + ((i - qIdx0) & 3) + 1) >> 1;
-      }
-      trel[sp] = (uint16_t) lev; absSum += lev;
+      const int i = src == 1 ? prev : src == 2 ? ((prev & 1) ? 3 : 0) : ((prev & 1) ? 1 : 2);
+      trel[sp] = (uint16_t) ((e & 1) ? i + 1 : 0);
       if (src == 4) { for (int j = 1; j < gs; j++) trel[sp + j] = 0; sp += gs; }
       else { prev = src == 1 ? -1 : src == 2 ? ((prev & 1) ? (prev == 1 ? 2 : 3) : (prev == 0 ? 0 : 1)) : src == 3 ? ((prev & 1) ? (prev == 1 ? 3 : 2) : (prev == 0 ? 1 : 0)) : -2; sp++; }
     }
     nPath = sp;
-    L.dq_abs[abs0 + item] = absSum;
   }
   nPath = __shfl(nPath, qbase);
   wave_sync();
   DQ_T(t4);
   for (int i = 0; i < n_items; i++) {
-    const int np = __builtin_amdgcn_readlane(nPath, i * 4);
+    const int np = __builtin_amdgcn_readlane(nPath, i * LPI);
     int16_t *c_ = cf_base + i * cf_stride; const uint16_t *tr = (const uint16_t *) (wk + n_items * 80) + i * total;
+    int absSum = 0;
     for (int sp = lane; sp < total; sp += 64) {
       const int blk = scan_blk(geo, sp), c = c_[blk];
-      const int lv = sp < np ? (int) tr[sp] : 0;
+      const int cand = sp < np ? (int) tr[sp] : 0;
+      int lv = 0;
+      if (cand) { const int qIdx0 = dq_qidx0(q, (long long) iabs(c) * q.qscale); lv = (qIdx0 + ((cand - 1 - qIdx0) & 3) + 1) >> 1; }
+      absSum += lv;
       c_[blk] = (int16_t) (c < 0 ? -lv : lv);
     }
+    absSum = wave_sum_i32(absSum);
+    if (lane == 0) L.dq_abs[abs0 + i] = absSum;
   }
   wave_sync();
 #ifdef VVCX_STAMP_DQ
-  { const long long t5 = clock64(); int fs = valid && k == 0 ? first + 1 : 0; for (int o = 32; o; o >>= 1) fs += __shfl_xor(fs, o);
+  { const long long t5 = clock64(); int fs = valid && sub == 0 ? first + 1 : 0; for (int o = 32; o; o >>= 1) fs += __shfl_xor(fs, o);
     if (lane == 0) { const long long v[14] = { t1 - t0, t2 - t1, t3 - t2, t4 - t3, t5 - t4, 1, top + 1, n_items, fs, total, sA, sB, sC, sE };
       for (int i = 0; i < 14; i++) atomicAdd(&L.prof[16 + i], (unsigned long long) v[i]); } }
 #endif
@@ -506,9 +550,9 @@
   const int wave_ = uni(VTX >> 6);
   int16_t *cf = SMALL ? L.wm[wave_].slot + BUF + uni(buf_off) : cf_g;
   if (imin(32, w) * imin(32, h) >= VXD_DQ_TAB_MIN && 240 + 2 * imin(32, w) * imin(32, h) + DQ_TAB_BYTES <= (int) (sizeof(WaveScratch) + sizeof(int32_t) * BUF))
-    wave_depquant_batch<1>(1, cf, 0, scratch + VXD_OFF_DQ + (size_t) wave_ * VXD_DQ_WAVE, 0, wave_, DQ_ABS_SINGLE + wave_, ci, 0, cbf_ctx, 0u, w, h, comp, zo, lfnst, lane, qidx);
+    wave_depquant_batch<1>(0, 1, cf, 0, scratch + VXD_OFF_DQ + (size_t) wave_ * VXD_DQ_WAVE, 0, wave_, DQ_ABS_SINGLE + wave_, ci, 0, cbf_ctx, 0u, w, h, comp, zo, lfnst, lane, qidx);
   else
-    wave_depquant_batch<0>(1, cf, 0, scratch + VXD_OFF_DQ + (size_t) wave_ * VXD_DQ_WAVE, 0, wave_, DQ_ABS_SINGLE + wave_, ci, 0, cbf_ctx, 0u, w, h, comp, zo, lfnst, lane, qidx);
+    wave_depquant_batch<0>(0, 1, cf, 0, scratch + VXD_OFF_DQ + (size_t) wave_ * VXD_DQ_WAVE, 0, wave_, DQ_ABS_SINGLE + wave_, ci, 0, cbf_ctx, 0u, w, h, comp, zo, lfnst, lane, qidx);
   return uni(L.dq_abs[DQ_ABS_SINGLE + wave_]);
 }
 
diff --git a/reduce-complexity-for-intra-coding-of-vvc_amd/csrc/vvcx_dev.h b/reduce-complexity-for-intra-coding-of-vvc_amd/csrc/vvcx_dev.h
--- a/reduce-complexity-for-intra-coding-of-vvc_amd/csrc/vvcx_dev.h
+++ b/reduce-complexity-for-intra-coding-of-vvc_amd/csrc/vvcx_dev.h
@@ -145,6 +145,9 @@
 #define VXD_OFF_ORG     (VXD_OFF_TMP + VXD_NW * 2048 * 4)
 #define VXD_OFF_LM      (VXD_OFF_ORG + 4096 * 2)
 #define VXD_DQ_WAVE     8192
+#define VXD_DQ_LEAF_ROOM2  (976 + 8 * VXD_BUF)
+#define VXD_DQ_LEAF_ROOM01 (976 + 4 * VXD_BUF)
+#define VXD_DQ_LEAF_TAB    808
 #define VXD_OFF_DQ      ((VXD_OFF_LM + (1024 + 128) * 2 + 255) & ~255)
 #define VXD_POOL_ELEMS      32768
 #define VXD_POOL_NODE_BYTES (128 * 1024)
diff --git a/reduce-complexity-for-intra-coding-of-vvc_amd/csrc/vvcx_kernel.hip b/reduce-complexity-for-intra-coding-of-vvc_amd/csrc/vvcx_kernel.hip
--- a/reduce-complexity-for-intra-coding-of-vvc_amd/csrc/vvcx_kernel.hip
+++ b/reduce-complexity-for-intra-coding-of-vvc_amd/csrc/vvcx_kernel.hip
@@ -121,6 +121,7 @@
   alignas(16) int32_t tmp[BUF];
   alignas(16) int16_t slot[2 * BUF];
 };
+static_assert(sizeof(WaveMem) == VXD_DQ_LEAF_ROOM2 && sizeof(WaveScratch) + sizeof(int32_t) * BUF == VXD_DQ_LEAF_ROOM01 && 4 * DQ_TAB_INTS == VXD_DQ_LEAF_TAB, "vvcx_dev.h: sizes of the trellis work area");
 #define CI_CUR 0
 #define CI_W(w) (1 + (w))
 struct Lds {
@@ -2161,7 +2162,7 @@
   int16_t *poolCoef = (int16_t *) (scratch + VXD_OFF_POOL_COEF) + (size_t) item0 * P; uint8_t *poolNodes = scratch + VXD_OFF_POOL_NODES + (size_t) item0 * 4 * total;
   const int ipw = imin(16, (int) sizeof(WaveMem) / (240 + 2 * total));
   for (int i0 = ((wave + NW - wave_shift) % NW) * ipw; i0 < n; i0 += NW * ipw)
-    wave_depquant_batch<2>(imin(ipw, n - i0), poolCoef + (size_t) i0 * P, P, poolNodes + (size_t) i0 * 4 * total, 4 * total, wave, abs0 + i0,
+    wave_depquant_batch<2>((int) sizeof(WaveMem), imin(ipw, n - i0), poolCoef + (size_t) i0 * P, P, poolNodes + (size_t) i0 * 4 * total, 4 * total, wave, abs0 + i0,
                         CI_CUR, 0, VX_CTX_QtCbf[0], 0u, w, h, 0, zo, lfnst, lane);
 }
 template <bool SMALL>
@@ -2597,7 +2598,7 @@
   {
     const int ipw = imin(16, (int) sizeof(WaveMem) / (240 + 2 * total));
     for (int i0 = wave * ipw; i0 < n_rd; i0 += NW * ipw)
-      wave_depquant_batch<2>(imin(ipw, n_rd - i0), poolCoef + (size_t) (2 * i0) * P, 2 * P, poolNodes + (size_t) (2 * i0) * 4 * total, 8 * total, wave, i0,
+      wave_depquant_batch<2>((int) sizeof(WaveMem), imin(ipw, n_rd - i0), poolCoef + (size_t) (2 * i0) * P, 2 * P, poolNodes + (size_t) (2 * i0) * 4 * total, 8 * total, wave, i0,
                           CI_CUR, 0, VX_CTX_QtCbf[1], 0u, w, h, 1, 0, psLf, lane);
   }
   __threadfence_block();
@@ -2628,9 +2629,9 @@
     {
       const int n4 = imin(NW, n_rd - c0);
       unsigned mask = 0; for (int i = 0; i < n4; i++) mask |= (unsigned) L.rb_pairs[i] << i;
-      if (crBatch) { if (wave == 0) wave_depquant_batch<0>(n4, poolCoef + (size_t) (2 * c0 + 1) * P, 2 * P, poolNodes + (size_t) (2 * c0 + 1) * 4 * total, 8 * total, 0, c0,
+      if (crBatch) { if (wave == 0) wave_depquant_batch<0>((int) (sizeof(WaveScratch) + sizeof(int32_t) * BUF), n4, poolCoef + (size_t) (2 * c0 + 1) * P, 2 * P, poolNodes + (size_t) (2 * c0 + 1) * 4 * total, 8 * total, 0, c0,
                                                         CI_W(0), 1, VX_CTX_QtCbf[2], mask, w, h, 2, 0, psLf, lane); }
-      else if (have) wave_depquant_batch<0>(1, poolCoef + (size_t) (2 * c + 1) * P, 0, poolNodes + (size_t) (2 * c + 1) * 4 * total, 0, wave, c,
+      else if (have) wave_depquant_batch<0>((int) (sizeof(WaveScratch) + sizeof(int32_t) * BUF), 1, poolCoef + (size_t) (2 * c + 1) * P, 0, poolNodes + (size_t) (2 * c + 1) * 4 * total, 0, wave, c,
                                          CI_W(wave), 0, VX_CTX_QtCbf[2], (unsigned) cbfs[0], w, h, 2, 0, psLf, lane);
     }
     __threadfence_block();
@@ -4285,6 +4286,29 @@
   else wave_code_block<false>(org + b, 0, 0, rec + b, lev + b, tmp + (size_t) blockIdx.x * 2048, w, h, bd, qp, lane, sse, cbf, -1, nullptr, comp, CI_CUR, cbf_cb, lf, lf ? lfnst_mode(lfdir, w, h) : 0);
   if (lane == 0) { out[blockIdx.x * 2] = sse; out[blockIdx.x * 2 + 1] = (unsigned long long) cbf; }
 }
+extern "C" __global__ void __launch_bounds__(NT, VXD_WPE) vvcx_leaf_dq_batch_kernel(VxParams p, const uint16_t *ctx, int16_t *coef, uint8_t *nodes, int n, int w, int h, int comp,
+                                                                                    int cbf_cb, int zo, int lfnst, int tab, int *abs_out)
+{
+  if (VTX == 0) { L.par = p; L.lmcs_tab = 0; }
+  load_tables();
+  for (int i = VTX; i < NCTX; i += NT) { L.ctxs[CI_CUR].s0[i] = ctx[i]; L.ctxs[CI_CUR].s1[i] = ctx[NCTX + i]; }
+  __syncthreads();
+  n = uni(n); w = uni(w); h = uni(h); comp = uni(comp); tab = uni(tab);
+  const int wave = uni(VTX >> 6), lane = VTX & 63, P = w * h, total = imin(32, w) * imin(32, h);
+  if (tab == 2) dq_build_tables(comp ? 1 : 0);
+  const int room = tab == 2 ? (int) sizeof(WaveMem) : (int) (sizeof(WaveScratch) + sizeof(int32_t) * BUF);
+  const int ipw = imin(16, (room - (tab == 1 ? DQ_TAB_BYTES : 0)) / (240 + 2 * total));
+  const int cbf_ctx = VX_CTX_QtCbf[comp] + (comp == 2 ? uni(cbf_cb) : 0);
+  for (int i0 = wave * ipw; i0 < n && ipw > 0; i0 += NW * ipw) {
+    const int m = imin(ipw, n - i0);
+    int16_t *cf = coef + (size_t) i0 * P; uint8_t *nd = nodes + (size_t) i0 * 4 * total;
+    if (tab == 2) wave_depquant_batch<2>(room, m, cf, P, nd, 4 * total, wave, i0, CI_CUR, 0, cbf_ctx, 0u, w, h, comp, zo, lfnst, lane);
+    else if (tab == 1) wave_depquant_batch<1>(0, m, cf, P, nd, 4 * total, wave, i0, CI_CUR, 0, cbf_ctx, 0u, w, h, comp, zo, lfnst, lane);
+    else wave_depquant_batch<0>(room, m, cf, P, nd, 4 * total, wave, i0, CI_CUR, 0, cbf_ctx, 0u, w, h, comp, zo, lfnst, lane);
+  }
+  __syncthreads();
+  if ((int) VTX < n) abs_out[VTX] = L.dq_abs[VTX];
+}
 extern "C" __global__ void __launch_bounds__(NT, VXD_WPE) vvcx_leaf_ts_kernel(VxParams p, const uint16_t *ctx, const int16_t *resi, int16_t *lev, int16_t *resi_out, int32_t *tmp,
                                                                               int w, int h, int qp, int *out, unsigned long long *bits)
 {
diff --git a/reduce-complexity-for-intra-coding-of-vvc_amd/vvcx.py b/reduce-complexity-for-intra-coding-of-vvc_amd/vvcx.py
--- a/reduce-complexity-for-intra-coding-of-vvc_amd/vvcx.py
+++ b/reduce-complexity-for-intra-coding-of-vvc_amd/vvcx.py
@@ -571,6 +571,18 @@
     return lev.reshape(n, h, w), rec.reshape(n, h, w), sse, cbf
 
 
+def leaf_dq_batch(coef, w, h, bit_depth, qp, comp, cbf_cb, lam, s0, s1, zero_out=0, lfnst=0, tab=2, device=0, lib_path=None):
+    L = load_library(lib_path)
+    coef = np.ascontiguousarray(coef, np.int16).ravel()
+    s0 = np.ascontiguousarray(s0, np.uint16); s1 = np.ascontiguousarray(s1, np.uint16)
+    n = coef.size // (w * h)
+    lev = np.zeros(coef.size, np.int16); asum = np.zeros(n, np.int32)
+    L.vvcx_leaf_dq_batch.argtypes = [C.c_void_p] + [C.c_int] * 6 + [C.c_double, C.c_void_p, C.c_void_p] + [C.c_int] * 4 + [C.c_void_p] * 2 + [C.c_int]
+    _chk(L, L.vvcx_leaf_dq_batch(coef.ctypes.data, w, h, bit_depth, qp, comp, cbf_cb, lam, s0.ctypes.data, s1.ctypes.data, n, zero_out, lfnst, tab,
+                                 lev.ctypes.data, asum.ctypes.data, device))
+    return lev.reshape(n, h, w), asum
+
+
 def transform_skip_batch(resi, w, h, bit_depth, qp, lam, s0, s1, device=0, lib_path=None):
     L = load_library(lib_path)
     resi = np.ascontiguousarray(resi, np.int16).ravel()
```
